# thomasjaron/masking-bundle-adjusting-neural-radiance-fields

Measured on AMD Instinct MI355X. Metric: warped+encoded+MLP pixels/s/GPU; final PSNR vs ref (seed=3), higher is better.
Workload: dtype bf16x3; 1 GPU; c3: 64 patches x 256x256 px per GPU, L=16, MLP 66-256-256-256-256-3, bf16x3 recipe (split-bf16 hi+lo MFMA operands, fp32 accumulate; seed-3 parity), c2f [0,0.4] at progress 0.2; patches_per_gpu=64, parallelism=dp1 (patches), step_kernel=k_step2

## Files before the change

masking-bundle-adjusting-neural-radiance-fields_amd/csrc/marf_abi.hip:

```cpp
#include <hip/hip_runtime.h>

#include <algorithm>
#include <cmath>
#include <cstdarg>
#include <cstdio>
#include <cstring>
#include <mutex>
#include <string>

#include "../../include/marf.h"
#include "marf_args.h"
#include "marf_prof.h"

using namespace marf;

static thread_local std::string g_err;
static unsigned long long* g_stamps = nullptr;

static int fail(int code, const char* fmt, ...) {
    char buf[512];
    va_list ap;
    va_start(ap, fmt);
    vsnprintf(buf, sizeof(buf), fmt, ap);
    va_end(ap);
// ... 499 lines not shown
        mx = std::max(mx, (long long)p.Mp * p.Kp + (long long)p.Kp * p.Mt + p.Mp);
    }
    MarfProfScope ps("pack_weights", (hipStream_t)stream);
    if (!split_recipe(net->dtype))
        HIPCHK(marf_launch_pack(net->kdt, d_params, (char*)d_packed, a, mx, (hipStream_t)stream), "net_pack");
    if (net->s2.variant >= 0) {
        const Step2NetPlan& q = net->s2;
        Pack2Args b;
        memset(&b, 0, sizeof(b));
        b.nl = net->n_layers;
        b.L = net->L;
        b.nk0 = q.nk0;
        b.nta = q.nta;
        b.NKH = q.HM / 16;
        b.split = q.variant == 1 || q.variant == 3;
        b.fwd_f16 = q.variant == 3;
        b.slot_bytes = q.slot;
        b.n_stages = q.n_stages;
        b.r0 = q.r0;
        b.ns0 = q.ns0;
        for (int l = 0; l <= net->n_layers; ++l) b.dims[l] = net->dims[l];
        for (int l = 0; l < net->n_layers; ++l) {
            b.nrt[l] = q.nrt[l];
            b.nrtb[l] = q.nrtb[l];
            b.w_off[l] = net->w_off[l];
            b.b_off[l] = net->b_off[l];
            b.boff[l] = q.boff[l];
            b.Mp[l] = net->Mp[l];
        }
        b.nbias = q.nbias;
        char* pk = (char*)d_packed;
        HIPCHK(marf_launch_pack2(d_params, pk + q.prog_off, (float*)(pk + q.bias_off), (int*)(pk + q.kmap_off), b,
                                 (hipStream_t)stream),
               "net_pack step2");
    }
    return MARF_OK;
}

static void fill_netdev(const marf_net* n, const void* packed, NetDev& d) {
    memset(&d, 0, sizeof(d));
    d.n_layers = n->n_layers;
    d.L = n->L;
    d.D = n->D;
    for (int l = 0; l < n->n_layers; ++l) {
        d.Kp[l] = n->Kp[l];
        d.Mp[l] = n->Mp[l];
        d.Mt[l] = n->Mt[l];
        d.Wf[l] = (const char*)packed + n->wf_off[l];
        d.Wt[l] = (const char*)packed + n->wt_off[l];
        d.bias[l] = (const float*)((const char*)packed + n->bias_off[l]);
        d.diag[l] = n->diag[l];
    }
    d.skip = n->skip;
}


struct SavedPlan {
    size_t feat[MARF_MAX_LAYERS], mask[MARF_MAX_LAYERS], total;
};

static void plan_saved(const marf_net* n, long long S, SavedPlan& p) {
    size_t off = 0;
    for (int l = 0; l < n->n_layers; ++l) {
        p.feat[l] = off;
        off += rup((long long)S * n->Kp[l] * n->elem, 256);
    }
    p.mask[0] = 0;
    for (int l = 1; l < n->n_layers; ++l) {
        p.mask[l] = off;
        off += rup(S / n->TP * 4096, 256);
    }
    p.total = off;
}

struct WsPlan {
    size_t dz[MARF_MAX_LAYERS], glast, dH, part, bpart, total;
    int chunk, n_chunks, n_tiles;
    int chunk_last, n_chunks_last;
};

static void plan_ws(const marf_net* n, long long S, int n_tiles, WsPlan& p) {
    size_t off = 0;
    p.dz[0] = 0;
    for (int l = 1; l < n->n_layers; ++l) {
        p.dz[l] = off;
        off += rup((long long)S * n->Kp[l] * n->elem, 256);
    }
    p.glast = off;
    off += rup(S * 16, 256);
    p.dH = off;
    off += rup((long long)n_tiles * 9 * 4, 256);
    long long chunk = rup((S + 255) / 256, 64);
    if (chunk < 64) chunk = 64;
    p.chunk = (int)chunk;
    p.n_chunks = (int)((S + chunk - 1) / chunk);
    p.n_tiles = n_tiles;
    long long mxo = 0, mxm = 0;
    for (int l = 0; l < n->n_layers - 1; ++l) {
        mxo = std::max(mxo, (long long)n->Mp[l] * n->Kp[l]);
        mxm = std::max(mxm, (long long)n->Mp[l]);
    }
    long long cl = rup((S + 1023) / 1024, 64);
    if (cl < 64) cl = 64;
    p.chunk_last = (int)cl;
    p.n_chunks_last = (int)((S + cl - 1) / cl);
    long long part_elems = std::max((long long)p.n_chunks * mxo, (long long)p.n_chunks_last * 3 * n->Kp[n->n_layers - 1]);
    long long bpart_elems = std::max((long long)p.n_chunks * mxm, (long long)p.n_chunks_last * 3);
    p.part = off;
    off += rup(part_elems * 4, 256);
    p.bpart = off;
    off += rup(bpart_elems * 4, 256);
    p.total = off;
}

size_t marf_saved_bytes(const marf_net* net, const marf_geometry* geo) {
    GeoDev g;
    if (!net || make_geo(geo, g, MARF_TILE_PAD) != MARF_OK) return 0;
    SavedPlan p;
    plan_saved(net, (long long)g.B * g.Np_pad, p);
    return p.total;
}

size_t marf_workspace_bytes(const marf_net* net, const marf_geometry* geo) {
    GeoDev g;
    if (!net || make_geo(geo, g, MARF_TILE_PAD) != MARF_OK) return 0;
    long long S = (long long)g.B * g.Np_pad;
    WsPlan p;
    plan_ws(net, S, (int)(S / net->TP), p);
    return p.total;
}


int marf_forward(const marf_net* net, const marf_geometry* geo, const marf_c2f* c2f, const void* d_packed,
                 float* d_rgb, void* d_saved, void* stream) {
    if (!net || !d_packed || !d_rgb) return fail(MARF_ERR_INVALID, "forward: NULL argument");
    if (split_recipe(net->dtype))
        return fail(MARF_ERR_UNSUPPORTED, "forward: split-recipe nets run marf_step_forward / marf_render only");
    FwdArgs a;
    memset(&a, 0, sizeof(a));
    int rc = make_geo(geo, a.geo, MARF_TILE_PAD);
    if (rc) return rc;
    fill_netdev(net, d_packed, a.net);
    a.c2f = make_c2f(c2f);
    a.rgb = d_rgb;
    a.S = (long long)a.geo.B * a.geo.Np_pad;
    a.lda = net->lda;
    if (d_saved) {
        SavedPlan p;
        plan_saved(net, a.S, p);
        for (int l = 0; l < net->n_layers; ++l) a.feat[l] = (char*)d_saved + p.feat[l];
        for (int l = 1; l < net->n_layers; ++l) a.mask[l] = (uint64_t*)((char*)d_saved + p.mask[l]);
    }
    int n_tiles = (int)(a.S / net->TP);
    {
        MarfProfScope ps("mlp_fwd", (hipStream_t)stream);
        HIPCHK(marf_launch_mlp_fwd(a, net->kdt, net->TP, net->lds_fwd, n_tiles, (hipStream_t)stream), "forward");
    }
    return MARF_OK;
}

int marf_backward(const marf_net* net, const marf_geometry* geo, const marf_c2f* c2f, const void* d_packed,
                  const float* d_h_params, int lie_batch, const float* d_rgb_out, const float* d_drgb,
                  const void* d_saved, void* d_workspace, float* d_dparams, float* d_dh, float* d_dcoords,
                  void* stream) {
    if (!net || !d_packed || !d_rgb_out || !d_drgb || !d_saved || !d_workspace)
        return fail(MARF_ERR_INVALID, "backward: NULL argument");
    if (split_recipe(net->dtype))
        return fail(MARF_ERR_UNSUPPORTED, "backward: split-recipe nets run marf_step_backward only");
    hipStream_t s = (hipStream_t)stream;
    BwdArgs a;
    memset(&a, 0, sizeof(a));
    int rc = make_geo(geo, a.geo, MARF_TILE_PAD);
    if (rc) return rc;
    if (a.geo.mode == MARF_GEO_GRID && d_dh && !d_h_params)
        return fail(MARF_ERR_INVALID, "backward: d_dh requested without the warp parameters");
    fill_netdev(net, d_packed, a.net);
    a.c2f = make_c2f(c2f);
    a.rgb = d_rgb_out;
    a.d_rgb = d_drgb;
    a.S = (long long)a.geo.B * a.geo.Np_pad;
    a.lda = net->lda;
    const int n_tiles = (int)(a.S / net->TP);
    SavedPlan sp;
    plan_saved(net, a.S, sp);
    WsPlan wp;
    plan_ws(net, a.S, n_tiles, wp);
    char* ws = (char*)d_workspace;
    const char* sv = (const char*)d_saved;
    for (int l = 1; l < net->n_layers; ++l) {
        a.mask[l] = (const uint64_t*)(sv + sp.mask[l]);
        a.dz[l] = ws + wp.dz[l];
    }
    a.glast = (float*)(ws + wp.glast);
    a.dH_partial = (float*)(ws + wp.dH);
    a.d_coords = d_dcoords;
    if (a.geo.mode == MARF_GEO_COORDS && !d_dcoords) {
        a.d_coords = nullptr;
    }
    {
        MarfProfScope ps("mlp_bwd_dgrad", s);
        HIPCHK(marf_launch_mlp_bwd(a, net->kdt, net->TP, net->lds_bwd, n_tiles, s), "backward dgrad");
    }

    if (d_dparams) {
        float* part = (float*)(ws + wp.part);
        float* bpart = (float*)(ws + wp.bpart);
        const int nl = net->n_layers;
        for (int l = 0; l < nl - 1; ++l) {
            {
                MarfProfScope ps(l == 0 ? "wgrad_l0" : "wgrad_hidden", s);
                HIPCHK(marf_launch_wgrad(net->kdt, ws + wp.dz[l + 1], net->Kp[l + 1], sv + sp.feat[l], net->Kp[l],
                                         a.S, net->Mp[l], net->Kp[l], wp.chunk, wp.n_chunks, part, bpart, s),
                       "backward wgrad");
            }
            {
                MarfProfScope ps("wgrad_reduce", s);
                HIPCHK(marf_launch_wgrad_reduce(part, bpart, wp.n_chunks, net->Mp[l], net->Kp[l], net->dims[l + 1],
                                                net->kin[l], d_dparams + net->w_off[l], d_dparams + net->b_off[l], s),
                       "backward wgrad reduce");
            }
        }
        const int l = nl - 1;
        {
            MarfProfScope ps("wgrad_last", s);
            HIPCHK(marf_launch_wgrad_last(net->kdt, a.glast, sv + sp.feat[l], a.S, net->Kp[l], net->Kp[l],
                                          wp.chunk_last, wp.n_chunks_last, part, bpart, s),
                   "backward wgrad last");
        }
        HIPCHK(marf_launch_wgrad_reduce(part, bpart, wp.n_chunks_last, 3, net->Kp[l], 3, net->dims[l],
                                        d_dparams + net->w_off[l], d_dparams + net->b_off[l], s),
               "backward wgrad last reduce");
    }
    if (a.geo.mode == MARF_GEO_GRID && d_dh) {
        MarfProfScope ps("warp_bwd", s);
        HIPCHK(marf_launch_reduce_dH(a.dH_partial, a.geo.Np_pad / net->TP, a.geo.B, d_h_params, nullptr, d_dh,
                                     lie_batch > 0 ? lie_batch : a.geo.B, s),
               "backward warp");
    }
    return MARF_OK;
}


struct StepPlan {
    size_t feat[MARF_MAX_LAYERS], dz[MARF_MAX_LAYERS], mask[MARF_MAX_LAYERS];
    size_t wlast, blast, dH, loss, c2f, part, bpart, total;
    int n_tiles, chunk, n_chunks;
};

static void plan_step(const marf_net* n, long long S, StepPlan& p) {
    size_t off = 0;
    const int nl = n->n_layers;
    p.n_tiles = (int)(S / n->sTP);
    for (int l = 0; l < nl - 1; ++l) {
        p.feat[l] = off;
        off += rup((long long)S * n->Kp[l] * n->elem, 256);
    }
    p.dz[0] = p.mask[0] = 0;
    for (int l = 1; l < nl; ++l) {
        p.dz[l] = off;
        off += rup((long long)S * n->Kp[l] * n->elem, 256);
        p.mask[l] = off;
        off += rup(S / n->sTP * n->sNW * 1024, 256);
    }
    p.wlast = off;
    off += rup((long long)p.n_tiles * 3 * n->Kp[nl - 1] * 4, 256);
    p.blast = off;
    off += rup((long long)p.n_tiles * 3 * 4, 256);
    p.dH = off;
    off += rup((long long)p.n_tiles * 9 * 4, 256);
    p.loss = off;
    off += rup((long long)p.n_tiles * 2 * 8, 256);
    p.c2f = off;
    off += 256;
    long long chunk = rup((S + 255) / 256, 64);
    if (chunk < 64) chunk = 64;
    p.chunk = (int)chunk;
    p.n_chunks = (int)((S + chunk - 1) / chunk);
    long long mxo = 0, mxm = 0;
    for (int l = 0; l < nl - 1; ++l) {
        mxo = std::max(mxo, (long long)n->Mp[l] * n->Kp[l]);
        mxm = std::max(mxm, (long long)n->Mp[l]);
    }
    p.part = off;
    off += rup(std::max((long long)p.n_chunks * mxo, 256LL * (3 * n->Kp[nl - 1] + 3)) * 4, 256);
    p.bpart = off;
    off += rup((long long)p.n_chunks * mxm * 4, 256);
    p.total = off;
}


#define MARF_PIPE_MAXP 64
struct PipePlan {
    int on;
    int G, R, P;
    int piece;
    int wg_last;
    int n_parts;
};

struct Step2BufPlan {
    size_t feat[MARF_MAX_LAYERS], dz[MARF_MAX_LAYERS];
    size_t dH, loss, blast, wlast, dummy, c2f, kmap, part, bpart, total;
    size_t partl[MARF_MAX_LAYERS], bpartl[MARF_MAX_LAYERS];
    int grid, n_tiles;
    int nblk;
    long long S;
    PipePlan pipe;
    bool fused_res;
};

static bool step2_fused_wgrad_possible(const marf_net* n) {
    static const bool env_off = [] {
        const char* e = getenv("MARF_WGRAD_FUSED");
        return e && e[0] == '0';
    }();
    if (env_off) return false;
    for (int l = 1; l < n->n_layers - 1; ++l)
        if (n->Mp[l] != 256 || n->Kp[l] != 256) return false;
    return true;
}

static int device_cus() {
    static int cus[64] = {0};
    int dev = 0;
    if (hipGetDevice(&dev) != hipSuccess || dev < 0 || dev >= 64) return 256;
    if (!cus[dev]) {
        int c = 0;
        if (hipDeviceGetAttribute(&c, hipDeviceAttributeMultiprocessorCount, dev) != hipSuccess || c <= 0) c = 256;
        cus[dev] = c;
    }
    return cus[dev];
}

static bool use_step2(const marf_net* n) { return n->s2.variant >= 0; }

static long long wgrad_chunk(long long S) {
    long long chunk = rup((S + 255) / 256, 64);
    return chunk < 64 ? 64 : chunk;
}

static bool l0_recompute(const marf_net* n, const GeoDev& g, long long S) {
    const char* e = getenv("MARF_F0_RECOMPUTE");
    if (e && e[0] == '0') return false;
    if ((n->s2.variant != 1 && n->s2.variant != 3) || g.mode != MARF_GEO_GRID) return false;
    const long long chunk = wgrad_chunk(S);
    return marf_wgrad_l0_recompute_ok(n->Mp[0], n->Kp[1], n->s2.ldf0, S, (int)chunk, (int)((S + chunk - 1) / chunk),
                                      g.Np_pad);
}


static void plan_pipe(const marf_net* n, const GeoDev& g, long long S, int n_tiles, PipePlan& pp) {
    memset(&pp, 0, sizeof(pp));
    const Step2NetPlan& q = n->s2;
    const int mode = n->pipe_mode;
    if (mode == 0 || q.variant < 0 || q.variant == 3 || g.mode != MARF_GEO_GRID) return;
    const int cus = device_cus();
    int R = n->pipe_wg > 0 ? n->pipe_wg : std::max(1, cus * 7 / 64);
    R = std::max(1, std::min(R, cus / 2));
    const int G = cus - R;
    if (mode < 0 && n_tiles < 16 * cus) return;
    int piece = n->pipe_piece;
    if (piece <= 0) {
        const int k = std::max(1, (int)std::lround((double)n_tiles / (8.0 * q.NS * G)));
        piece = k * q.NS * G;
    }
    piece = (int)rup(piece, q.NS);
    int P = (n_tiles + piece - 1) / piece;
    if (P < 2) {
        if (mode != 1) return;
        piece = (int)rup((n_tiles + 1) / 2, q.NS);
        P = (n_tiles + piece - 1) / piece;
        if (P < 2) return;
    }
    if (P > MARF_PIPE_MAXP) return;
    const int nl = n->n_layers;
    for (int l = 1; l < nl - 1; ++l)
        if (!marf_wgrad_range_ok(n->kdt, n->Mp[l], n->Kp[l + 1], n->Kp[l], n->Kp[l])) return;
    if (!marf_wgrad_range_ok(n->kdt, n->Mp[0], n->Kp[1], q.ldf0, q.ldf0)) return;
    if (l0_recompute(n, g, S)) {
        const long long mx = rup((long long)piece * q.TPX / R + 32, 32);
        if (!marf_wgrad_l0_recompute_ok(n->Mp[0], n->Kp[1], q.ldf0, S, (int)mx, P * cus, g.Np_pad)) return;
    }
    pp.on = 1;
    pp.G = G;
    pp.R = R;
    pp.P = P;
    pp.piece = piece;
    pp.wg_last = cus;
    pp.n_parts = (P - 1) * R + cus;
}

struct PipeStreams {
    hipStream_t s2;
    hipEvent_t ev[MARF_PIPE_MAXP + 1];
    std::mutex use;
};
static int pipe_streams(PipeStreams** out) {
    static std::mutex mu;
    static PipeStreams ps[64];
    int dev = 0;
    HIPCHK(hipGetDevice(&dev), "pipeline: hipGetDevice");
    if (dev < 0 || dev >= 64) return fail(MARF_ERR_UNSUPPORTED, "pipeline: device %d", dev);
    std::lock_guard<std::mutex> lk(mu);
    PipeStreams& p = ps[dev];
    if (!p.s2) {
        HIPCHK(hipStreamCreateWithFlags(&p.s2, hipStreamNonBlocking), "pipeline: stream");
        for (int i = 0; i <= MARF_PIPE_MAXP; ++i)
            HIPCHK(hipEventCreateWithFlags(&p.ev[i], hipEventDisableTiming), "pipeline: event");
    }
    *out = &p;
    return MARF_OK;
}

static void plan_step2_bufs(const marf_net* n, const GeoDev& g, Step2BufPlan& p, bool render = false) {
    const Step2NetPlan& q = n->s2;
    const int nl = n->n_layers;
    const long long Ssave = render ? 0 : 1;
    p.S = (long long)g.B * g.Np_pad;
    p.n_tiles = (int)(p.S / q.TPX);
    int cap = device_cus();
    if (const char* e = getenv("MARF_STEP2_GRID")) cap = std::max(1, atoi(e));
    p.grid = std::max(1, std::min(p.n_tiles, cap));
    memset(&p.pipe, 0, sizeof(p.pipe));
    p.fused_res = false;
    if (!render) plan_pipe(n, g, p.S, p.n_tiles, p.pipe);
    if (p.pipe.on) p.grid = p.pipe.G;
    p.nblk = p.pipe.on ? p.pipe.P * p.pipe.G : p.grid;
    size_t off = 0;
    const long long Sfeat = p.S + (q.variant == 3 ? q.TPX : 0);
    for (int l = 0; l < nl - 1; ++l) {
        p.feat[l] = off;
        off += rup(Ssave * Sfeat * (l == 0 ? q.ldf0 : n->Kp[l]) * 2, 256);
    }
    p.dz[0] = 0;
    const long long Ssink = p.S + q.TPX;
    for (int l = 1; l < nl; ++l) {
        p.dz[l] = off;
        off += rup(Ssave * Ssink * n->Kp[l] * 2, 256);
    }
    p.dH = off;
    off += rup(Ssave * Ssink / q.PX * 9 * 4, 256);
    p.loss = off;
    off += rup((long long)p.nblk * 2 * 8, 256);
    p.blast = off;
    off += rup((long long)p.nblk * 3 * 4, 256);
    p.wlast = off;
    off += rup((long long)p.nblk * 3 * q.Kl * 4, 256);
    p.dummy = off;
    off += rup((long long)p.grid * q.NW * 4096, 256);
    p.c2f = off;
    off += 256;
    p.kmap = off;
    off += rup((long long)n->D * 4, 256);
    long long chunk = rup((p.S + 255) / 256, 64);
    if (chunk < 64) chunk = 64;
    const long long n_chunks = (p.S + chunk - 1) / chunk;
    long long mxo = 0, mxm = 0;
    for (int l = 0; l < nl - 1; ++l) {
        mxo = std::max(mxo, (long long)n->Mp[l] * (l == 0 ? q.ldf0 : n->Kp[l]));
        mxm = std::max(mxm, (long long)n->Mp[l]);
    }
    if (p.pipe.on) {
        const long long np = p.pipe.n_parts;
        for (int l = 0; l < nl - 1; ++l) {
            p.partl[l] = off;
            off += rup(np * n->Mp[l] * (l == 0 ? q.ldf0 : n->Kp[l]) * 4, 256);
            p.bpartl[l] = off;
            off += rup(np * n->Mp[l] * 4, 256);
        }
        p.part = off;
        off += rup(256LL * (3 * q.Kl + 3) * 4, 256);
        p.bpart = 0;
    } else {
        p.part = off;
        off += rup(Ssave * std::max(n_chunks * mxo, 256LL * (3 * q.Kl + 3)) * 4, 256);
        p.bpart = off;
        off += rup(Ssave * n_chunks * mxm * 4, 256);
        p.fused_res = !render && step2_fused_wgrad_possible(n);
        p.partl[0] = p.part;
        p.bpartl[0] = p.bpart;
        for (int l = 1; l < nl - 1; ++l) {
            p.partl[l] = p.part;
            p.bpartl[l] = p.bpart;
            if (!p.fused_res) continue;
            p.partl[l] = off;
            off += rup(Ssave * n_chunks * n->Mp[l] * n->Kp[l] * 4, 256);
            p.bpartl[l] = off;
            off += rup(Ssave * n_chunks * n->Mp[l] * 4, 256);
        }
    }
    p.total = off;
}

static int wgrad_piece(const marf_net* net, const GeoDev& g, const Step2BufPlan& p, char* sv, int j, hipStream_t s2) {
    const Step2NetPlan& q = net->s2;
    const PipePlan& pp = p.pipe;
    const int nl = net->n_layers;
    const long long TPX = q.TPX;
    const long long t0 = (long long)j * pp.piece, t1 = std::min<long long>(p.n_tiles, t0 + pp.piece);
    WgRange r;
    r.s_lo = t0 * TPX;
    r.s_len = (t1 - t0) * TPX;
    r.n = j == pp.P - 1 ? pp.wg_last : pp.R;
    r.part0 = j * pp.R;
    const bool f0 = l0_recompute(net, g, p.S);
    for (int l = 0; l < nl - 1; ++l) {
        const int K = l == 0 ? q.ldf0 : net->Kp[l];
        float* part = (float*)(sv + p.partl[l]);
        float* bpart = (float*)(sv + p.bpartl[l]);
        MarfProfScope ps(l == 0 ? "wgrad_l0" : "wgrad_hidden", s2);
        if (l == 0 && f0)
            HIPCHK(marf_launch_wgrad_l0_recompute(sv + p.dz[1], net->Kp[1], g, (const float*)(sv + p.c2f), net->L, q.nk0w,
                                                  q.ldf0, p.S, net->Mp[0], 32, r.n, part, bpart, s2, &r),
                   "step_forward pipelined wgrad_l0");
        else
            HIPCHK(marf_launch_wgrad(1, sv + p.dz[l + 1], net->Kp[l + 1], sv + p.feat[l], K, p.S, net->Mp[l], K, 32, r.n,
                                     part, bpart, s2, &r, true),
                   "step_forward pipelined wgrad");
    }
    return MARF_OK;
}

static hipError_t launch_s2(const marf_net* n, const Step2Args& a, int grid, hipStream_t s) {
    const Step2NetPlan& q = n->s2;
    bool full = (q.variant == 1 || q.variant == 3) && q.nk0 >= 1 && q.r0 == std::max(1, std::min(8, 16 / q.nk0)) && q.Kl == 256;
    for (int l = 0; l < n->n_layers - 1; ++l) full = full && n->Mp[l] == 256;
    if (const char* e = getenv("MARF_STEP2_GENERIC")) full = full && e[0] != '1';
    return marf_launch_step2(a, q.variant, grid, s, full ? q.nk0 : 0, q.dz);
}

static int step2_forward(const marf_net* net, const marf_geometry* geo, const marf_c2f* c2f, const void* d_packed,
                         const float* d_gt, const float* d_mask, const float* d_denom_override, float* d_rgb,
                         float* d_loss_out, void* d_saved, hipStream_t s, bool render = false) {
    const Step2NetPlan& q = net->s2;
    Step2Args a;
    memset(&a, 0, sizeof(a));
    int rc = make_geo(geo, a.geo, q.TPX);
    if (rc) return rc;
    Step2BufPlan p;
    plan_step2_bufs(net, a.geo, p, render);
    char* sv = (char*)d_saved;
    const char* pk = (const char*)d_packed;
    const int nl = net->n_layers;
    a.nl = nl;
    a.L = net->L;
    a.nk0 = q.nk0;
    a.nta = q.nta;
    a.r0 = q.r0;
    C2fDev cf = make_c2f(c2f);
    a.c2f_on = cf.on;
    a.prog = pk + q.prog_off;
    a.n_stages = q.n_stages;
    a.n_fwd = q.n_fwd;
    a.S = p.S;
    if (render) {
        a.fwd_only = 1;
        a.n_stages = a.n_fwd;
        a.pro_fallback = a.geo.mode == MARF_GEO_COORDS ? a.geo.coords : a.geo.Hm;
    }
    a.bias = (const float*)(pk + q.bias_off);
    a.nbias = q.nbias;
    a.feat0_recompute = !render && l0_recompute(net, a.geo, p.S) ? 1 : 0;
    a.gt = d_gt;
    a.mask = d_mask;
    a.rgb = d_rgb;
    for (int l = 0; l < nl; ++l) {
        S2Layer& y = a.layers[l];
        y.nrt = q.nrt[l];
        y.nrtb = q.nrtb[l];
        y.boff = q.boff[l];
        y.ldf = l == 0 ? q.ldf0 : net->Kp[l];
        y.ldz = net->Kp[l];
        y.feat = l < nl - 1 && !render ? (u16*)(sv + p.feat[l]) : nullptr;
        y.dz = l >= 1 && !render ? (u16*)(sv + p.dz[l]) : nullptr;
    }
    a.dH_partial = (float*)(sv + p.dH);
    a.loss_partial = (double*)(sv + p.loss);
    a.blast_partial = (float*)(sv + p.blast);
    a.wlast_partial = (float*)(sv + p.wlast);
    a.Kl = q.Kl;
    a.c2f_w = (const float*)(sv + p.c2f);
    a.dummy = (float*)(sv + p.dummy);
    a.stamps = g_stamps;
    a.n_tiles = p.n_tiles;
    const int TPX = q.TPX;
    int off = q.nslot * q.slot;
    a.lds_pro = off;
    off += q.variant == 3 ? 1024 + 2 * 4 * TPX * 4 : 2 * (4 * TPX + 64) * 4;
    a.lds_bias = off;
    off += (int)rup(q.nbias * 4, 16);
    a.lds_c2f = off;
    off += 128;
    a.lds_layers = off;
    off += (int)sizeof(S2Layer) * MARF_MAX_LAYERS;
    a.lds_wave = off;
    a.lds_wave_bytes = (int)rup(2048 + q.NS * q.MAXR * q.NMW * 256 + 12 * q.Kl, 16);
    off += q.NW * a.lds_wave_bytes;
    a.lds_total = off;
    if (off > 160 * 1024) return fail(MARF_ERR_UNSUPPORTED, "step2: LDS plan %d B exceeds 160 KB", off);
    HIPCHK(marf_launch_c2f_weights(cf, net->L, (float*)(sv + p.c2f), s, (const int*)(pk + q.kmap_off),
                                   (int*)(sv + p.kmap), net->D),
           "step_forward c2f / kmap");
    if (render) {
        MarfProfScope ps("mlp_fwd", s);
        HIPCHK(launch_s2(net, a, p.grid, s), "render step2");
        return MARF_OK;
    }
    double* const loss0 = a.loss_partial;
    if (!p.pipe.on) {
        MarfProfScope ps("mlp_step", s);
        HIPCHK(launch_s2(net, a, p.grid, s), "step_forward step2");
    } else {
        const PipePlan& pp = p.pipe;
        PipeStreams* st = nullptr;
        rc = pipe_streams(&st);
        if (rc) return rc;
        std::lock_guard<std::mutex> hold(st->use);
        float* const blast0 = a.blast_partial;
        float* const wlast0 = a.wlast_partial;
        for (int j = 0; j < pp.P; ++j) {
            a.tile0 = j * pp.piece;
            a.n_tiles = std::min(p.n_tiles, (j + 1) * pp.piece);
            a.loss_partial = loss0 + (size_t)j * pp.G * 2;
            a.blast_partial = blast0 + (size_t)j * pp.G * 3;
            a.wlast_partial = wlast0 + (size_t)j * pp.G * 3 * q.Kl;
            {
                MarfProfScope ps("mlp_step", s);
                HIPCHK(launch_s2(net, a, pp.G, s), "step_forward step2 piece");
            }
            HIPCHK(hipEventRecord(st->ev[j], s), "pipeline: record");
            HIPCHK(hipStreamWaitEvent(st->s2, st->ev[j], 0), "pipeline: wait");
            rc = wgrad_piece(net, a.geo, p, sv, j, st->s2);
            if (rc) return rc;
        }
        HIPCHK(hipEventRecord(st->ev[MARF_PIPE_MAXP], st->s2), "pipeline: record");
        HIPCHK(hipStreamWaitEvent(s, st->ev[MARF_PIPE_MAXP], 0), "pipeline: join");
    }
    {
        MarfProfScope ps("loss_final", s);
        HIPCHK(marf_launch_loss_final(loss0, p.nblk, d_loss_out, d_denom_override, s), "step_forward loss");
    }
    return MARF_OK;
}

static int mark_layer(const void* const* ev, int l, hipStream_t s) {
    if (ev && ev[l]) HIPCHK(hipEventRecord((hipEvent_t)ev[l], s), "step_backward: layer event");
    return MARF_OK;
}

static int step2_backward(const marf_net* net, const marf_geometry* geo, const void* d_saved,
                          const float* d_h_params, int lie_batch, const float* d_gout, const float* d_loss_out,
                          float* d_dparams, float* d_dh, hipStream_t s, const void* const* ev) {
    const Step2NetPlan& q = net->s2;
    GeoDev g;
    int rc = make_geo(geo, g, q.TPX);
    if (rc) return rc;
    Step2BufPlan p;
    plan_step2_bufs(net, g, p);
    const char* sv = (const char*)d_saved;
    float* part = (float*)(sv + p.part);
    float* bpart = (float*)(sv + p.bpart);
    const float* denom = d_loss_out + 1;
    const int nl = net->n_layers;
    const int sdt = q.variant == 3 ? 2 : 1;
    const float post = q.variant == 3 ? 1.0f / 1024.0f : 1.0f;
    if (d_dparams && !p.pipe.on && p.fused_res) {
        const long long chunk = wgrad_chunk(p.S);
        const int n_chunks = (int)((p.S + chunk - 1) / chunk);
        const int* kmap = (const int*)(sv + p.kmap);
        const bool f0 = l0_recompute(net, g, p.S);
        WgFusedLayer Lf[MARF_MAX_LAYERS];
        memset(Lf, 0, sizeof(Lf));
        int nf = 0;
        {
            const int l = nl - 1;
            WgFusedLayer& x = Lf[nf++];
            x.kind = 3;
            x.partial = (float*)(sv + p.wlast);
            x.bpartial = (float*)(sv + p.blast);
            x.n_parts = p.nblk;
            x.M = 3;
            x.K = q.Kl;
            x.Mo = 3;
            x.Ko = net->dims[l];
            x.dW = d_dparams + net->w_off[l];
            x.db = d_dparams + net->b_off[l];
        }
        for (int l = nl - 2; l >= 0; --l) {
            WgFusedLayer& x = Lf[nf++];
            x.kind = l > 0 ? 0 : (f0 ? 1 : 2);
            x.dz = sv + p.dz[l + 1];
            x.ldz = net->Kp[l + 1];
            x.feat = (l == 0 && f0) ? nullptr : sv + p.feat[l];
            x.ldf = x.K = l == 0 ? q.ldf0 : net->Kp[l];
            x.M = net->Mp[l];
            x.partial = (float*)(sv + p.partl[l]);
            x.bpartial = (float*)(sv + p.bpartl[l]);
            x.n_parts = n_chunks;
            x.Mo = net->dims[l + 1];
            x.Ko = net->dims[l];
            x.dW = d_dparams + net->w_off[l];
            x.db = d_dparams + net->b_off[l];
            x.kmap = l == 0 ? kmap : nullptr;
        }
        if (marf_wgrad_fused_ok(Lf, nf, p.S, (int)chunk, n_chunks, g.Np_pad)) {
            PipeStreams* st = nullptr;
            rc = pipe_streams(&st);
            if (rc) return rc;
            {
                std::lock_guard<std::mutex> hold(st->use);
                const char* dse = getenv("MARF_DH_SIDE");
                float* dh_side = (dse && dse[0] == '0') ? nullptr : d_dh;
                if (dh_side) {
                    HIPCHK(hipEventRecord(st->ev[2], s), "step_backward: fork");
                    HIPCHK(hipStreamWaitEvent(st->s2, st->ev[2], 0), "step_backward: fork");
                }
                {
                    MarfProfScope ps("wgrad_fused", s);
                    HIPCHK(marf_launch_wgrad_fused(Lf, nf, p.S, (int)chunk, n_chunks, g, (const float*)(sv + p.c2f),
                                                   net->L, q.nk0w, d_gout, denom, s, st->s2, st->ev[0], st->ev[1], sdt, post),
                           "step_backward fused weight gradients");
                }
                if (dh_side) {
                    MarfProfScope ps("warp_bwd_side", st->s2);
                    HIPCHK(marf_launch_reduce_dH((const float*)(sv + p.dH), g.Np_pad / q.PX, g.B, d_h_params, nullptr,
                                                 dh_side, lie_batch > 0 ? lie_batch : g.B, st->s2, d_gout, denom),
                           "step_backward warp");
                    HIPCHK(hipEventRecord(st->ev[3], st->s2), "step_backward: join");
                }
                for (int l = nl - 1; l >= 0; --l) {
                    rc = mark_layer(ev, l, s);
                    if (rc) return rc;
                }
                if (dh_side) {
                    HIPCHK(hipStreamWaitEvent(s, st->ev[3], 0), "step_backward: join");
                    d_dh = nullptr;
                }
            }
            d_dparams = nullptr;
        }
    }
    if (d_dparams) {
        const int l = nl - 1;
        MarfProfScope ps("wgrad_last_reduce", s);
        HIPCHK(marf_launch_wgrad_reduce((const float*)(sv + p.wlast), (const float*)(sv + p.blast), p.nblk, 3, q.Kl, 3,
                                        net->dims[l], d_dparams + net->w_off[l], d_dparams + net->b_off[l], s, d_gout,
                                        denom, part),
               "step_backward last reduce");
        rc = mark_layer(ev, l, s);
        if (rc) return rc;
    }
    if (d_dparams && p.pipe.on) {
        const int* kmap = (const int*)(sv + p.kmap);
        for (int l = nl - 2; l >= 0; --l) {
            const int K = l == 0 ? q.ldf0 : net->Kp[l];
            MarfProfScope ps("wgrad_reduce", s);
            HIPCHK(marf_launch_wgrad_reduce((const float*)(sv + p.partl[l]), (const float*)(sv + p.bpartl[l]),
                                            p.pipe.n_parts, net->Mp[l], K, net->dims[l + 1], net->dims[l],
                                            d_dparams + net->w_off[l], d_dparams + net->b_off[l], s, d_gout, denom,
                                            nullptr, l == 0 ? kmap : nullptr),
                   "step_backward wgrad reduce (pipelined)");
            rc = mark_layer(ev, l, s);
            if (rc) return rc;
        }
    } else if (d_dparams) {
        const long long chunk = wgrad_chunk(p.S);
        const int n_chunks = (int)((p.S + chunk - 1) / chunk);
        const int* kmap = (const int*)(sv + p.kmap);
        const bool f0 = l0_recompute(net, g, p.S);
        for (int l = nl - 2; l >= 0; --l) {
            const int K = l == 0 ? q.ldf0 : net->Kp[l];
            {
                MarfProfScope ps(l == 0 ? "wgrad_l0" : "wgrad_hidden", s);
                if (l == 0 && f0)
                    HIPCHK(marf_launch_wgrad_l0_recompute(sv + p.dz[1], net->Kp[1], g, (const float*)(sv + p.c2f), net->L,
                                                          q.nk0w, q.ldf0, p.S, net->Mp[0], (int)chunk, n_chunks, part, bpart, s,
                                                          nullptr, sdt),
                           "step_backward wgrad_l0 (feat_0 recomputed)");
                else
                    HIPCHK(marf_launch_wgrad(sdt, sv + p.dz[l + 1], net->Kp[l + 1], sv + p.feat[l], K, p.S, net->Mp[l], K,
                                             (int)chunk, n_chunks, part, bpart, s, nullptr, true),
                           "step_backward wgrad");
            }
            {
                MarfProfScope ps("wgrad_reduce", s);
                HIPCHK(marf_launch_wgrad_reduce(part, bpart, n_chunks, net->Mp[l], K, net->dims[l + 1], net->dims[l],
                                                d_dparams + net->w_off[l], d_dparams + net->b_off[l], s, d_gout, denom,
                                                nullptr, l == 0 ? kmap : nullptr, post),
                       "step_backward wgrad reduce");
            }
            rc = mark_layer(ev, l, s);
            if (rc) return rc;
        }
    }
    if (d_dh) {
        MarfProfScope ps("warp_bwd", s);
        HIPCHK(marf_launch_reduce_dH((const float*)(sv + p.dH), g.Np_pad / q.PX, g.B, d_h_params, nullptr, d_dh,
                                     lie_batch > 0 ? lie_batch : g.B, s, d_gout, denom),
               "step_backward warp");
    }
    return MARF_OK;
}

size_t marf_render_workspace_bytes(const marf_net* net, const marf_geometry* geo) {
    if (!net || !geo || !use_step2(net)) return 0;
    GeoDev g;
    if (make_geo(geo, g, net->s2.TPX) != MARF_OK) return 0;
    Step2BufPlan p;
    plan_step2_bufs(net, g, p, true);
    return p.total;
}

int marf_render(const marf_net* net, const marf_geometry* geo, const marf_c2f* c2f, const void* d_packed, float* d_rgb,
                void* d_ws, void* stream) {
    if (!net || !geo || !d_packed || !d_rgb) return fail(MARF_ERR_INVALID, "render: NULL argument");
    if (!use_step2(net)) return marf_forward(net, geo, c2f, d_packed, d_rgb, nullptr, stream);
    if (!d_ws) return fail(MARF_ERR_INVALID, "render: workspace (marf_render_workspace_bytes) missing");
    if (geo->mode == MARF_GEO_GRID || geo->mode == MARF_GEO_CANVAS) {
        if (!geo->d_H) return fail(MARF_ERR_INVALID, "render: grid geometry needs d_H");
    } else if (geo->mode == MARF_GEO_COORDS) {
        if (geo->Np <= 0 || !geo->d_coords) return fail(MARF_ERR_INVALID, "render: coords geometry needs points");
    }
    return step2_forward(net, geo, c2f, d_packed, nullptr, nullptr, nullptr, d_rgb, nullptr, d_ws,
                         (hipStream_t)stream, true);
}

size_t marf_step_saved_bytes(const marf_net* net, const marf_geometry* geo) {
    GeoDev g;
    if (!net || !geo || geo->mode == MARF_GEO_COORDS) return 0;
    if (use_step2(net)) {
        if (make_geo(geo, g, net->s2.TPX) != MARF_OK) return 0;
        Step2BufPlan p2;
        plan_step2_bufs(net, g, p2);
        return p2.total;
    }
    if (make_geo(geo, g, MARF_TILE_PAD) != MARF_OK) return 0;
    StepPlan p;
    plan_step(net, (long long)g.B * g.Np_pad, p);
    return p.total;
}

int marf_step_forward(const marf_net* net, const marf_geometry* geo, const marf_c2f* c2f, const void* d_packed,
                      const float* d_gt, const float* d_mask, const float* d_denom_override, float* d_rgb,
                      float* d_loss_out, void* d_saved, void* stream) {
    if (!net || !d_packed || !d_gt || !d_loss_out || !d_saved) return fail(MARF_ERR_INVALID, "step_forward: NULL argument");
    if (!geo || geo->mode == MARF_GEO_COORDS) return fail(MARF_ERR_INVALID, "step_forward: needs a pixel-grid geometry");
    hipStream_t s = (hipStream_t)stream;
    if (use_step2(net))
        return step2_forward(net, geo, c2f, d_packed, d_gt, d_mask, d_denom_override, d_rgb, d_loss_out, d_saved, s);
    StepArgs a;
    memset(&a, 0, sizeof(a));
    int rc = make_geo(geo, a.geo, MARF_TILE_PAD);
    if (rc) return rc;
    fill_netdev(net, d_packed, a.net);
    a.c2f = make_c2f(c2f);
    a.rgb = d_rgb;
    a.gt = d_gt;
    a.mask = d_mask;
    a.S = (long long)a.geo.B * a.geo.Np_pad;
    a.lda = net->lda;
    StepPlan p;
    plan_step(net, a.S, p);
    char* sv = (char*)d_saved;
    const int nl = net->n_layers;
    for (int l = 0; l < nl - 1; ++l) a.feat[l] = sv + p.feat[l];
    for (int l = 1; l < nl; ++l) {
        a.dz[l] = sv + p.dz[l];
        a.mask_bits[l] = (uint64_t*)(sv + p.mask[l]);
    }
    a.wlast_partial = (float*)(sv + p.wlast);
    a.blast_partial = (float*)(sv + p.blast);
    a.dH_partial = (float*)(sv + p.dH);
    a.loss_partial = (double*)(sv + p.loss);
    a.c2f_w = (const float*)(sv + p.c2f);
    a.stamps = g_stamps;
    if (net->L > 0) HIPCHK(marf_launch_c2f_weights(a.c2f, net->L, (float*)(sv + p.c2f), s), "step_forward c2f");
    {
        MarfProfScope ps("mlp_step", s);
        HIPCHK(marf_launch_mlp_step(a, net->kdt, net->sTP, net->sNW, net->lds_step, p.n_tiles, s), "step_forward");
    }
    {
        MarfProfScope ps("loss_final", s);
        HIPCHK(marf_launch_loss_final(a.loss_partial, p.n_tiles, d_loss_out, d_denom_override, s), "step_forward loss");
    }
    return MARF_OK;
}

int marf_step_backward(const marf_net* net, const marf_geometry* geo, const void* d_saved, const float* d_h_params,
                       int lie_batch, const float* d_gout, const float* d_loss_out, float* d_dparams, float* d_dh,
                       void* stream) {
    return marf_step_backward_ev(net, geo, d_saved, d_h_params, lie_batch, d_gout, d_loss_out, d_dparams, d_dh, nullptr,
                                 stream);
}

int marf_step_backward_ev(const marf_net* net, const marf_geometry* geo, const void* d_saved, const float* d_h_params,
                          int lie_batch, const float* d_gout, const float* d_loss_out, float* d_dparams, float* d_dh,
                          void* const* layer_events, void* stream) {
    const void* const* ev = (const void* const*)layer_events;
    if (!net || !d_saved || !d_gout || !d_loss_out) return fail(MARF_ERR_INVALID, "step_backward: NULL argument");
    if (!geo || geo->mode == MARF_GEO_COORDS) return fail(MARF_ERR_INVALID, "step_backward: needs a pixel-grid geometry");
    if (d_dh && !d_h_params) return fail(MARF_ERR_INVALID, "step_backward: d_dh requested without the warp parameters");
    hipStream_t s = (hipStream_t)stream;
    if (use_step2(net))
        return step2_backward(net, geo, d_saved, d_h_params, lie_batch, d_gout, d_loss_out, d_dparams, d_dh, s, ev);
    GeoDev g;
    int rc = make_geo(geo, g, MARF_TILE_PAD);
    if (rc) return rc;
    const long long S = (long long)g.B * g.Np_pad;
    StepPlan p;
    plan_step(net, S, p);
    const char* sv = (const char*)d_saved;
    float* part = (float*)(sv + p.part);
    float* bpart = (float*)(sv + p.bpart);
    const float* denom = d_loss_out + 1;
    const int nl = net->n_layers;
    if (d_dparams) {
        {
            const int l = nl - 1;
            MarfProfScope ps("wgrad_last_reduce", s);
            HIPCHK(marf_launch_wgrad_reduce((const float*)(sv + p.wlast), (const float*)(sv + p.blast), p.n_tiles, 3,
                                            net->Kp[l], 3, net->dims[l], d_dparams + net->w_off[l],
                                            d_dparams + net->b_off[l], s, d_gout, denom, part),
                   "step_backward last reduce");
            rc = mark_layer(ev, l, s);
            if (rc) return rc;
        }
        for (int l = nl - 2; l >= 0; --l) {
            {
                MarfProfScope ps(l == 0 ? "wgrad_l0" : "wgrad_hidden", s);
                HIPCHK(marf_launch_wgrad(net->kdt, sv + p.dz[l + 1], net->Kp[l + 1], sv + p.feat[l], net->Kp[l], S,
                                         net->Mp[l], net->Kp[l], p.chunk, p.n_chunks, part, bpart, s),
                       "step_backward wgrad");
            }
            {
                MarfProfScope ps("wgrad_reduce", s);
                HIPCHK(marf_launch_wgrad_reduce(part, bpart, p.n_chunks, net->Mp[l], net->Kp[l], net->dims[l + 1],
                                                net->kin[l], d_dparams + net->w_off[l], d_dparams + net->b_off[l], s,
                                                d_gout, denom),
                       "step_backward wgrad reduce");
            }
            rc = mark_layer(ev, l, s);
            if (rc) return rc;
        }
    }
    if (d_dh) {
        MarfProfScope ps("warp_bwd", s);
        HIPCHK(marf_launch_reduce_dH((const float*)(sv + p.dH), g.Np_pad / net->sTP, g.B, d_h_params, nullptr, d_dh,
                                     lie_batch > 0 ? lie_batch : g.B, s, d_gout, denom),
               "step_backward warp");
    }
    return MARF_OK;
}


size_t marf_mse_workspace_bytes(void) { return 1024 * 2 * sizeof(double); }

int marf_masked_mse(const float* d_pred, const float* d_gt, const float* d_mask, int B, int Np,
                    const float* d_denom_override, float* d_out, void* d_ws, void* stream) {
    if (B <= 0 || Np <= 0 || !d_pred || !d_gt || !d_out || !d_ws) return fail(MARF_ERR_INVALID, "masked_mse: bad args");
    MarfProfScope ps("loss_fwd", (hipStream_t)stream);
    HIPCHK(marf_launch_mse(d_pred, d_gt, d_mask, B, Np, (double*)d_ws, d_out, d_denom_override, (hipStream_t)stream),
           "masked_mse");
    return MARF_OK;
}

int marf_masked_mse_backward(const float* d_pred, const float* d_gt, const float* d_mask, int B, int Np,
                             const float* d_denom, const float* d_gout, float* d_dpred, void* stream) {
    if (B <= 0 || Np <= 0 || !d_pred || !d_gt || !d_denom || !d_gout || !d_dpred)
        return fail(MARF_ERR_INVALID, "masked_mse_backward: bad args");
    MarfProfScope ps("loss_bwd", (hipStream_t)stream);
    HIPCHK(marf_launch_mse_bwd(d_pred, d_gt, d_mask, B, Np, d_denom, d_gout, d_dpred, (hipStream_t)stream),
           "masked_mse_backward");
    return MARF_OK;
}

int marf_edge_map(const float* d_img, int n_img, int H, int W, double* d_out, void* stream) {
    if (n_img < 0 || H <= 0 || W <= 0 || (n_img > 0 && (!d_img || !d_out))) return fail(MARF_ERR_INVALID, "edge_map: bad args");
    if (n_img > 65535) return fail(MARF_ERR_INVALID, "edge_map: more than 65535 channel images");
    if (n_img == 0) return MARF_OK;
    MarfProfScope ps("edge_map", (hipStream_t)stream);
    HIPCHK(marf_launch_edge_map(d_img, d_out, n_img, H, W, (hipStream_t)stream), "edge_map");
    return MARF_OK;
}

int marf_erode_rect(const float* d_img, int n_img, int H, int W, int kh, int kw, float* d_out, void* stream) {
    if (n_img < 0 || H <= 0 || W <= 0 || kh <= 0 || kw <= 0 || (n_img > 0 && (!d_img || !d_out)))
        return fail(MARF_ERR_INVALID, "erode_rect: bad args");
    if (n_img > 65535) return fail(MARF_ERR_INVALID, "erode_rect: more than 65535 channel images");
    if (d_img == d_out) return fail(MARF_ERR_INVALID, "erode_rect: in-place erosion is not supported");
    if (n_img == 0) return MARF_OK;
    HIPCHK(marf_launch_erode_rect(d_img, d_out, n_img, H, W, kh, kw, (hipStream_t)stream), "erode_rect");
    return MARF_OK;
}

}

static void adam_scalars(double lr, double beta1, double beta2, long long step, float& step_size, float& bc2_sqrt) {
    const double bc1 = 1.0 - std::pow(beta1, (double)step);
    const double bc2 = 1.0 - std::pow(beta2, (double)step);
    step_size = (float)(lr / bc1);
    bc2_sqrt = (float)std::sqrt(bc2);
}

extern "C" {

int marf_adam_step(float* d_p, const float* d_g, float* d_m, float* d_v, long long n, double lr, double beta1,
                   double beta2, double eps, long long step, const float* d_grad_scale, void* stream) {
    if (n < 0 || step < 1 || (n > 0 && (!d_p || !d_g || !d_m || !d_v))) return fail(MARF_ERR_INVALID, "adam: bad args");
    float step_size, bc2_sqrt;
    adam_scalars(lr, beta1, beta2, step, step_size, bc2_sqrt);
    MarfProfScope ps("adam", (hipStream_t)stream);
    HIPCHK(marf_launch_adam(d_p, d_g, d_m, d_v, n, (float)(1.0 - beta1), (float)beta2, (float)(1.0 - beta2),
                            step_size, bc2_sqrt, (float)eps, d_grad_scale, (hipStream_t)stream),
           "adam");
    return MARF_OK;
}

int marf_adam_schedule(double lr, double beta1, double beta2, long long first_step, long long count, float* h_out) {
    if (first_step < 1 || count < 0 || (count > 0 && !h_out)) return fail(MARF_ERR_INVALID, "adam_schedule: bad args");
    for (long long i = 0; i < count; ++i) adam_scalars(lr, beta1, beta2, first_step + i, h_out[2 * i], h_out[2 * i + 1]);
    return MARF_OK;
}

int marf_adam_step_sched(float* d_p, const float* d_g, float* d_m, float* d_v, long long n, double beta1, double beta2,
                         double eps, const float* d_sched, const int* d_index, const float* d_grad_scale, void* stream) {
    if (n < 0 || (n > 0 && (!d_p || !d_g || !d_m || !d_v || !d_sched || !d_index)))
        return fail(MARF_ERR_INVALID, "adam_step_sched: bad args");
    MarfProfScope ps("adam", (hipStream_t)stream);
    HIPCHK(marf_launch_adam_sched(d_p, d_g, d_m, d_v, n, (float)(1.0 - beta1), (float)beta2, (float)(1.0 - beta2),
                                  d_sched, d_index, (float)eps, d_grad_scale, (hipStream_t)stream),
           "adam_step_sched");
    return MARF_OK;
}

}
```

masking-bundle-adjusting-neural-radiance-fields_amd/csrc/marf_args.h:

```cpp
#pragma once
#include "marf_common.h"

namespace marf {

struct C2fDev {
    const float* progress;
    float start, span;
    int on;
};

struct FwdArgs {
    NetDev net;
    GeoDev geo;
    C2fDev c2f;
    float* rgb;
    void* feat[MARF_MAX_LAYERS];
    uint64_t* mask[MARF_MAX_LAYERS];
    long long S;
    int lda;
};

struct BwdArgs {
    NetDev net;
    GeoDev geo;
    C2fDev c2f;
    const float* rgb;
    const float* d_rgb;
    const uint64_t* mask[MARF_MAX_LAYERS];
    void* dz[MARF_MAX_LAYERS];
    float* glast;
    float* dH_partial;
    float* d_coords;
    long long S;
    int lda;
};

struct StepArgs {
    NetDev net;
    GeoDev geo;
    C2fDev c2f;
    float* rgb;
    const float* gt;
    const float* mask;
    void* feat[MARF_MAX_LAYERS];
    uint64_t* mask_bits[MARF_MAX_LAYERS];
    void* dz[MARF_MAX_LAYERS];
    float* wlast_partial;
    float* blast_partial;
    float* dH_partial;
    double* loss_partial;
    const float* c2f_w;
    unsigned long long* stamps;
    long long S;
    int lda;
};

struct PackLayer {
    int M, K;
    int Mp, Kp, Mt;
    long long w_off, b_off;
    long long wf_off, wt_off, bias_off;
    unsigned diag;
};

struct PackArgs {
    int n_layers;
    PackLayer ly[MARF_MAX_LAYERS];
};

struct S2Layer {
    int nrt;
    int nrtb;
    int boff;
    int ldf;
    int ldz;
    int pad;
    u16* feat;
    u16* dz;
};

struct Step2Args {
    GeoDev geo;
    int nl, L, nk0, nta, c2f_on;
    int r0;
    const char* prog;
    int n_stages;
    int n_fwd;
    long long S;
    const float* bias;
    int nbias;
    const float* gt;
    const float* mask;
    float* rgb;
    S2Layer layers[MARF_MAX_LAYERS];
    float* dH_partial;
    double* loss_partial;
    float* blast_partial;
    float* wlast_partial;
    int Kl;
    const float* c2f_w;
    float* dummy;
    unsigned long long* stamps;
    int tile0, n_tiles;
    int fwd_only;
    int feat0_recompute;
    const float* pro_fallback;
    int lds_pro, lds_bias, lds_c2f, lds_layers, lds_wave, lds_wave_bytes, lds_total;
};

struct Pack2Args {
    int nl, L, nk0, nta, NKH, split, slot_bytes, n_stages;
    int fwd_f16;
    int r0, ns0;
    int dims[MARF_MAX_LAYERS + 1];
    int nrt[MARF_MAX_LAYERS], nrtb[MARF_MAX_LAYERS];
    long long w_off[MARF_MAX_LAYERS], b_off[MARF_MAX_LAYERS];
    int boff[MARF_MAX_LAYERS];
    int Mp[MARF_MAX_LAYERS];
    int nbias;
};

hipError_t ensure_dynamic_lds(const void* kernel, size_t lds);

}

hipError_t marf_launch_sl3(const float* h, float* H, int B, int batch_hint, hipStream_t s);
hipError_t marf_launch_se2_embed(const float* p, float* h, int B, hipStream_t s);
hipError_t marf_launch_se2_embed_bwd(const float* dh, float* dp, int B, hipStream_t s);
hipError_t marf_launch_sl3_bwd(const float* h, const float* dH, float* dh, int B, int batch_hint, hipStream_t s);
hipError_t marf_launch_reduce_dH(const float* partial, int tiles_per_patch, int B, const float* h, float* dH_out,
                                 float* dh, int batch_hint, hipStream_t s, const float* gscale = nullptr,
                                 const float* denom = nullptr);
hipError_t marf_launch_mlp_fwd(const marf::FwdArgs& a, int dtype, int TP, size_t lds, int n_tiles, hipStream_t s);
hipError_t marf_launch_mlp_bwd(const marf::BwdArgs& a, int dtype, int TP, size_t lds, int n_tiles, hipStream_t s);
struct WgRange {
    long long s_lo, s_len;
    int n, part0;
};
bool marf_wgrad_range_ok(int dtype, int M, int ldz, int K, int ldf);
bool marf_wgrad_l0_recompute_ok(int M, int ldz, int ldf0, long long S, int chunk, int n_chunks, long long Np_pad);
hipError_t marf_launch_wgrad_l0_recompute(const void* dz, int ldz, const GeoDev& geo, const float* c2f_w, int L,
                                          int nk0, int K0, long long S, int M, int chunk, int n_chunks, float* partial,
                                          float* bpartial, hipStream_t s, const WgRange* rng = nullptr, int dtype = 1);
hipError_t marf_launch_wgrad(int dtype, const void* dz, int ldz, const void* feat, int ldf, long long S, int M, int K,
                             int chunk, int n_chunks, float* partial, float* bpartial, hipStream_t s,
                             const WgRange* rng = nullptr, bool t16 = false);
struct WgFusedLayer {
    int kind;
    const void* dz;
    const void* feat;
    int ldz, ldf, M, K;
    float* partial;
    float* bpartial;
    int n_parts;
    int Mo, Ko;
    float* dW;
    float* db;
    const int* kmap;
};
bool marf_wgrad_fused_ok(const WgFusedLayer* layers, int n_layers, long long S, int chunk, int n_chunks,
                         long long Np_pad);
hipError_t marf_launch_wgrad_fused(const WgFusedLayer* layers, int n_layers, long long S, int chunk, int n_chunks,
                                   const GeoDev& f0_geo, const float* c2f_w, int L, int nk0, const float* gscale,
                                   const float* denom, hipStream_t s, hipStream_t s2, hipEvent_t fork, hipEvent_t join,
                                   int dtype = 1, float post = 1.f);
hipError_t marf_launch_wgrad_last(int dtype, const float* glast, const void* feat, long long S, int ldf, int K,
                                  int chunk, int n_chunks, float* partial, float* bpartial, hipStream_t s);
hipError_t marf_launch_wgrad_reduce(const float* partial, const float* bpartial, int n_chunks, int M, int K, int Mo,
                                    int Ko, float* dW, float* db, hipStream_t s, const float* gscale = nullptr,
                                    const float* denom = nullptr, float* scratch = nullptr,
                                    const int* kmap = nullptr, float post = 1.f);
hipError_t marf_launch_mlp_step(const marf::StepArgs& a, int dtype, int TP, int NW, size_t lds, int n_tiles, hipStream_t s);
hipError_t marf_launch_c2f_weights(const marf::C2fDev& c, int L, float* out, hipStream_t s,
                                   const int* csrc = nullptr, int* cdst = nullptr, int cn = 0);
hipError_t marf_launch_loss_final(const double* part, int n, float* out, const float* denom_override, hipStream_t s);
hipError_t marf_launch_step2(const marf::Step2Args& a, int variant, int grid, hipStream_t s, int full_nk0, bool dz = false);
hipError_t marf_launch_pack2(const float* params, void* prog, float* bias_out, int* kmap, const marf::Pack2Args& a,
                             hipStream_t s);
hipError_t marf_launch_edge_map(const float* in, double* out, int n_img, int H, int W, hipStream_t s);
hipError_t marf_launch_erode_rect(const float* in, float* out, int n_img, int H, int W, int kh, int kw, hipStream_t s);
hipError_t marf_launch_mse(const float* pred, const float* gt, const float* mask, int B, int Np, double* part,
                           float* out, const float* denom_override, hipStream_t s);
hipError_t marf_launch_mse_bwd(const float* pred, const float* gt, const float* mask, int B, int Np,
                               const float* denom, const float* gout, float* d_pred, hipStream_t s);
hipError_t marf_launch_adam(float* p, const float* g, float* m, float* v, long long n, float w1, float b2,
                            float one_minus_b2, float step_size, float bc2_sqrt, float eps, const float* grad_scale,
                            hipStream_t s);
hipError_t marf_launch_adam_sched(float* p, const float* g, float* m, float* v, long long n, float w1, float b2,
                                  float one_minus_b2, const float* sched, const int* index, float eps,
                                  const float* grad_scale, hipStream_t s);
hipError_t marf_launch_pack(int dtype, const float* params, char* packed, const marf::PackArgs& a,
                            long long max_elems, hipStream_t s);
hipError_t marf_launch_pixel_grid(const GeoDev& g, float* xy, int n, hipStream_t s);
hipError_t marf_launch_warp_points(const float* xy, const float* Hm, float* uv, int B, int n, int xy_shared,
                                   hipStream_t s);
hipError_t marf_launch_posenc(const float* coord, long long n, int L, const float* progress, float start, float span,
                              int c2f_on, float* enc, hipStream_t s);
hipError_t marf_launch_warp_points_bwd(const float* xy, const float* Hm, const float* G, float* dxy, float* dH, int B,
                                       int n, int xy_shared, hipStream_t s);
hipError_t marf_launch_posenc_bwd(const float* coord, const float* G, long long n, int L, const float* progress,
                                  float start, float span, int c2f_on, float* dcoord, hipStream_t s);
hipError_t marf_launch_prologue_probe(const GeoDev& g, const marf::C2fDev& c, int L, const float* gt,
                                      const float* mask, float* out, int grid, hipStream_t s);
```

masking-bundle-adjusting-neural-radiance-fields_amd/csrc/marf_step2.hip:

```cpp
#include <type_traits>

#include "marf_args.h"

namespace marf {


MARF_DEV void s2_glds4(const void* src, unsigned lds) {
    unsigned keep;
    asm volatile("s_mov_b32 %0, m0\n\ts_mov_b32 m0, %2\n\ts_nop 0\n\tglobal_load_lds_dword %1, off\n\ts_mov_b32 m0, %0"
                 : "=&s"(keep)
                 : "v"(src), "s"(lds)
                 : "memory");
}
typedef uint32_t s2_u32x2 __attribute__((ext_vector_type(2)));
typedef uint32_t s2_u32x4 __attribute__((ext_vector_type(4)));
MARF_DEV void s2_st8(void* dst, uint32_t a, uint32_t b) {
    const s2_u32x2 v = {a, b};
    asm volatile("global_store_dwordx2 %0, %1, off\n\ts_nop 1" ::"v"(dst), "v"(v) : "memory");
}
MARF_DEV void s2_st16(void* dst, uint4 u) {
    const s2_u32x4 v = {u.x, u.y, u.z, u.w};
    asm volatile("global_store_dwordx4 %0, %1, off\n\ts_nop 1" ::"v"(dst), "v"(v) : "memory");
}
template <int OFF>
MARF_DEV void s2_st16o(void* base, uint4 u) {
    const s2_u32x4 v = {u.x, u.y, u.z, u.w};
    asm volatile("global_store_dwordx4 %0, %1, off offset:%2\n\ts_nop 1" ::"v"(base), "v"(v), "n"(OFF) : "memory");
}
MARF_DEV void s2_st12(void* dst, float a, float b, float c) {
    typedef float f32x3 __attribute__((ext_vector_type(3)));
    f32x3 v = {a, b, c};
    asm volatile("global_store_dwordx3 %0, %1, off\n\ts_nop 1" ::"v"(dst), "v"(v) : "memory");
}
MARF_DEV void s2_st4(void* dst, float a) {
    asm volatile("global_store_dword %0, %1, off\n\ts_nop 1" ::"v"(dst), "v"(a) : "memory");
}
template <int N>
MARF_DEV void s2_wait_vm() {
    asm volatile("s_waitcnt vmcnt(%0)" ::"n"(N) : "memory");
}

MARF_DEV i16x4 s2_tr16(const u16* p) {
    return __builtin_amdgcn_ds_read_tr16_b64_v4i16((__attribute__((address_space(3))) i16x4*)(p));
}

template <int... I, class F>
MARF_DEV void s2_sfor_impl(std::integer_sequence<int, I...>, F&& f) {
    (f(std::integral_constant<int, I>()), ...);
}
template <int N, class F>
MARF_DEV void s2_sfor(F&& f) {
    s2_sfor_impl(std::make_integer_sequence<int, N>(), f);
}

MARF_DEV uint32_t s2_pk(float a, float b) {
    typedef float f32x2 __attribute__((ext_vector_type(2)));
    typedef __bf16 bf16x2 __attribute__((ext_vector_type(2)));
    return __builtin_bit_cast(uint32_t, __builtin_convertvector(((f32x2){a, b}), bf16x2));
}
MARF_DEV float s2_lo16(uint32_t w) { return __uint_as_float(w << 16); }
MARF_DEV float s2_hi16(uint32_t w) { return __uint_as_float(w & 0xffff0000u); }

union S2Frag {
    bf16x8 f;
    f16x8 h;
    uint4 u;
    uint32_t w[4];
};

MARF_DEV uint32_t s2_pkh(float a, float b) {
    typedef float f32x2 __attribute__((ext_vector_type(2)));
    typedef _Float16 f16x2 __attribute__((ext_vector_type(2)));
    return __builtin_bit_cast(uint32_t, __builtin_convertvector(((f32x2){a, b}), f16x2));
}

template <bool LO>
MARF_DEV void s2_split8(const float* x, S2Frag& hi, S2Frag& lo) {
    hi.u = make_uint4(s2_pk(x[0], x[1]), s2_pk(x[2], x[3]), s2_pk(x[4], x[5]), s2_pk(x[6], x[7]));
    if constexpr (LO) {
        const uint32_t w[4] = {hi.u.x, hi.u.y, hi.u.z, hi.u.w};
        float r[8];
#pragma unroll
        for (int q = 0; q < 4; ++q) {
            r[2 * q] = x[2 * q] - s2_lo16(w[q]);
            r[2 * q + 1] = x[2 * q + 1] - s2_hi16(w[q]);
        }
        lo.u = make_uint4(s2_pk(r[0], r[1]), s2_pk(r[2], r[3]), s2_pk(r[4], r[5]), s2_pk(r[6], r[7]));
    }
}


#ifdef MARF_STAMPS
#define S2T_BEGIN(k) const unsigned long long _t##k = __builtin_amdgcn_s_memtime()
#define S2T_END(k) tacc[k] += __builtin_amdgcn_s_memtime() - _t##k
#else
#define S2T_BEGIN(k) \
    do {         \
    } while (0)
#define S2T_END(k) \
    do {       \
    } while (0)
#endif

template <int HM, bool SPLIT, int NW, int MAXR, bool DZ = false>
struct S2Cfg {
    static constexpr int NKH = HM / 16;
    static constexpr int NRT = HM / 32;
    static constexpr int SLOT = NKH * 1024 * (SPLIT ? 2 : 1);
    static constexpr int LO = NKH * 1024;
    static constexpr int PER_DMA = SLOT / (NW * 1024);
    static constexpr int NSLOT = 3, D = 2;
    static constexpr int NS = SPLIT && !DZ ? 2 : 1;
    static constexpr int NK0 = 9;
    static constexpr int NTA = 5;
    static constexpr int TPX = 32 * NW;
    static constexpr int NMW = NRT / 2;
    static constexpr int MSET = MAXR * NMW * 64;
    static_assert(PER_DMA * NW * 1024 == SLOT, "slot size");
};

template <int HM, bool SPLIT, int NW, int MAXR, int NK0F, int NTAF, bool DZ, bool HF = false>
__device__ __attribute__((always_inline)) inline void k_step2_body(const Step2Args& a) {
    typedef S2Cfg<HM, SPLIT, NW, MAXR, DZ> C;
    constexpr bool SDZ = SPLIT && DZ;
    constexpr int NKH = C::NKH, NRT = C::NRT, NS = C::NS;
    constexpr bool FIX = NK0F > 0;
    static_assert(NK0F <= C::NK0, "layer-0 k-steps");
    static_assert(!HF || (SPLIT && !DZ && NK0F > 0 && NS == 2), "fp16x2: split dgrad, two sets, compile-time layer 0");
#ifndef MARF_STEP2_J2
#define MARF_STEP2_J2 1
#endif
    constexpr bool J2 = MARF_STEP2_J2 && NS == 2 && SPLIT && !SDZ && FIX;
    constexpr float kGS = 1024.f;
    constexpr int R0Q = NKH / (FIX ? NK0F : NKH);
    constexpr int R0F = R0Q < 1 ? 1 : (R0Q > NRT ? NRT : R0Q);
    extern __shared__ __attribute__((aligned(16))) char smem[];
    const int lane = threadIdx.x & 63;
    const int wave = __builtin_amdgcn_readfirstlane(threadIdx.x >> 6);
    const int h = lane >> 5, pxl = lane & 31;
    const int nl = a.nl, L = a.L;

    const unsigned lds0 = (unsigned)(uintptr_t)(__attribute__((address_space(3))) char*)smem;
    float* bias_l = reinterpret_cast<float*>(smem + a.lds_bias);
    float* c2f_l = reinterpret_cast<float*>(smem + a.lds_c2f);
    S2Layer* lyr = reinterpret_cast<S2Layer*>(smem + a.lds_layers);
    auto ly_int = [&](int l, int field) -> int {
        return __builtin_amdgcn_readfirstlane(reinterpret_cast<const int*>(lyr + l)[field]);
    };
    auto ly_ptr = [&](int l, int which) -> u16* {
        const uint32_t* q = reinterpret_cast<const uint32_t*>(lyr + l) + 6 + 2 * which;
        const uint64_t lo = (uint32_t)__builtin_amdgcn_readfirstlane(q[0]);
        const uint64_t hi = (uint32_t)__builtin_amdgcn_readfirstlane(q[1]);
        return reinterpret_cast<u16*>(lo | (hi << 32));
    };
    char* wpriv = smem + a.lds_wave + wave * a.lds_wave_bytes;
    u16* trs = reinterpret_cast<u16*>(wpriv);
    u16* gts = reinterpret_cast<u16*>(wpriv + 1024);
    uint32_t* mkl = reinterpret_cast<uint32_t*>(wpriv + 2048);
    float* wla = reinterpret_cast<float*>(wpriv + 2048 + NS * C::MSET * 4);
    float* dmy = a.dummy + (((size_t)blockIdx.x * NW + wave) * 2 * 64 + lane) * 2;
#ifdef MARF_STAMPS
    unsigned long long tacc[16] = {};
#endif

    for (int e = threadIdx.x; e < a.nbias; e += NW * 64) bias_l[e] = a.bias[e];
    if ((int)threadIdx.x < 32) c2f_l[threadIdx.x] = (int)threadIdx.x < L ? a.c2f_w[threadIdx.x] : 0.f;
    for (int e = threadIdx.x; e < nl * (int)(sizeof(S2Layer) / 4); e += NW * 64)
        reinterpret_cast<uint32_t*>(lyr)[e] = reinterpret_cast<const uint32_t*>(a.layers)[e];
    for (int e = lane; e < 512; e += 64) reinterpret_cast<uint32_t*>(gts)[e] = 0u;
    for (int e = lane; e < 3 * a.Kl; e += 64) wla[e] = 0.f;

    const int tpp = a.geo.Np_pad / C::TPX;
    const int Np = a.geo.Np;
    const int tbase = a.tile0 + (int)blockIdx.x;
    int my_tiles = 0;
    if (tbase < a.n_tiles) my_tiles = (a.n_tiles - 1 - tbase) / (int)gridDim.x + 1;
    const int nF = a.n_fwd, nB = a.n_stages - a.n_fwd;
    const int total = HF ? ((my_tiles + NS - 1) / NS) * (nF + nB)
                         : (my_tiles / NS) * (NS * nF + nB) + (my_tiles % NS ? (my_tiles % NS) * nF + nB : 0);

    auto pro_buf = [&](int pb) -> float* { return reinterpret_cast<float*>(smem + a.lds_pro + pb * (4 * C::TPX + 64) * 4); };
    auto issue_pro = [&](int tile, int pb) {
        const int b = tile / tpp, q0 = (tile - b * tpp) * C::TPX;
        const unsigned base = lds0 + a.lds_pro + pb * (4 * C::TPX + 64) * 4;
#pragma unroll
        for (int i = 0; i < 2; ++i) {
            const int f = ((wave * 2 + i) * 64) + lane;
            const int ch = f / C::TPX, q = f - ch * C::TPX;
            const int p = min(q0 + q, Np - 1);
            const float* src = !a.gt ? a.pro_fallback
                               : ch < 3 ? a.gt + ((size_t)b * 3 + ch) * Np + p
                                        : (a.mask ? a.mask + (size_t)b * Np + p : a.gt + (size_t)b * 3 * Np + p);
            s2_glds4(src, __builtin_amdgcn_readfirstlane(base + (wave * 2 + i) * 256));
        }
        s2_glds4(a.geo.Hm ? a.geo.Hm + 9 * (size_t)b + (lane < 9 ? lane : 0) : a.pro_fallback,
                 __builtin_amdgcn_readfirstlane(base + 4 * C::TPX * 4));
    };

    auto hf_tile = [&](int ti) -> int { return tbase + min(ti, my_tiles - 1) * (int)gridDim.x; };
    auto proH = [&](int par, int set) -> const float* {
        return reinterpret_cast<const float*>(smem + a.lds_pro + (par * 2 + set) * 256);
    };
    auto proT = [&](int set) -> const float* {
        return reinterpret_cast<const float*>(smem + a.lds_pro + 1024 + set * C::TPX * 16);
    };
    auto issue_h = [&](int ti, int par) {
#pragma unroll
        for (int set = 0; set < 2; ++set) {
            const int b = hf_tile(ti + set) / tpp;
            s2_glds4(a.geo.Hm ? a.geo.Hm + 9 * (size_t)b + (lane < 9 ? lane : 0) : a.pro_fallback,
                     __builtin_amdgcn_readfirstlane(lds0 + a.lds_pro + (par * 2 + set) * 256));
        }
    };
    auto issue_tgt = [&](int ti) {
#pragma unroll
        for (int set = 0; set < 2; ++set) {
            const int tile = hf_tile(ti + set);
            const int b = tile / tpp, q0 = (tile - b * tpp) * C::TPX;
            const unsigned base = lds0 + a.lds_pro + 1024 + set * C::TPX * 16;
#pragma unroll
            for (int i = 0; i < 2; ++i) {
                const int f = ((wave * 2 + i) * 64) + lane;
                const int ch = f / C::TPX, q = f - ch * C::TPX;
                const int p = min(q0 + q, Np - 1);
                const float* src = !a.gt ? a.pro_fallback
                                   : ch < 3 ? a.gt + ((size_t)b * 3 + ch) * Np + p
                                            : (a.mask ? a.mask + (size_t)b * Np + p : a.gt + (size_t)b * 3 * Np + p);
                s2_glds4(src, __builtin_amdgcn_readfirstlane(base + (wave * 2 + i) * 256));
            }
        }
    };

    int c_stage = 0;
    int dma_stage = 0;
    int dg_i = 0, dg_n = 0, dg_ns = 0, dg_t = 0;
    auto grp_init = [&](int t) {
        dg_t = t;
        dg_ns = HF ? 1 : min(NS, my_tiles - t);
        dg_n = dg_ns * nF + nB;
        dg_i = 0;
    };
    grp_init(0);
    auto dma_next = [&]() -> int {
        const int i = dg_i;
        const int prog = i < nF ? i : (i < dg_ns * nF ? i - nF : i - (dg_ns - 1) * nF);
        if (++dg_i == dg_n) grp_init(dg_t + NS);
        return prog;
    };
    unsigned dma_m0 = 0;
    const char* dma_va0 = nullptr;
    const char* dma_va1 = nullptr;
    auto dma_arm = [&]() {
        const int ps = dma_stage < total ? dma_next() : 0;
        dma_m0 = __builtin_amdgcn_readfirstlane(lds0 + (dma_stage % C::NSLOT) * C::SLOT + wave * C::PER_DMA * 1024);
        dma_va0 = a.prog + (size_t)ps * C::SLOT + wave * C::PER_DMA * 1024 + lane * 16;
        if constexpr (C::PER_DMA > 4) dma_va1 = dma_va0 + 4096;
        ++dma_stage;
    };
    auto dma_piece = [&](auto jc) {
        constexpr int j = decltype(jc)::value;
        static_assert(j < C::PER_DMA && C::PER_DMA <= 8, "piece index");
        const char* va = j < 4 ? dma_va0 : dma_va1;
        const unsigned m = dma_m0 + (j < 4 ? 0u : 4096u);
        unsigned keep;
        asm volatile("s_mov_b32 %0, m0\n\ts_mov_b32 m0, %2\n\ts_nop 0\n\tglobal_load_lds_dwordx4 %1, off offset:%3\n\ts_mov_b32 m0, %0"
                     : "=&s"(keep)
                     : "v"(va), "s"(m), "n"((j & 3) * 1024)
                     : "memory");
    };
    auto dma_burst = [&]() { s2_sfor<C::PER_DMA>([&](auto jc) { dma_piece(jc); }); };
    int st_cur = 0, st_prev = 0;
    auto wait_ring = [&]() {
        const int y = st_prev + st_cur;
        constexpr int PD = C::PER_DMA;
        if (y >= 8) s2_wait_vm<PD + 8>();
        else if (y >= 6) s2_wait_vm<PD + 6>();
        else if (y >= 4) s2_wait_vm<PD + 4>();
        else if (y >= 2) s2_wait_vm<PD + 2>();
        else s2_wait_vm<PD>();
    };
    auto stage_begin = [&](bool burst) -> const char* {
        S2T_BEGIN(0);
        S2T_BEGIN(12);
        wait_ring();
#ifdef MARF_STAMPS
        asm volatile("s_waitcnt lgkmcnt(0)" ::: "memory");
#endif
        S2T_END(12);
        st_prev = st_cur;
        st_cur = 0;
        asm volatile("s_waitcnt lgkmcnt(0)" ::: "memory");
        __builtin_amdgcn_s_barrier();
        asm volatile("" ::: "memory");
        S2T_END(0);
        S2T_BEGIN(1);
        dma_arm();
        if (burst) dma_burst();
        S2T_END(1);
        const char* slot = smem + (c_stage % C::NSLOT) * C::SLOT;
        ++c_stage;
        return slot;
    };

    if (my_tiles > 0) {
        if constexpr (HF) {
            issue_h(0, 0);
            issue_tgt(0);
        } else {
            issue_pro(tbase, 0);
        }
        dma_arm();
        dma_burst();
        dma_arm();
        dma_burst();
    }
    s2_wait_vm<0>();
    __syncthreads();

    double lsq = 0.0, lms = 0.0;
    float bl0 = 0.f, bl1 = 0.f, bl2 = 0.f;

    uint32_t mpend = 0u;

    S2Frag Bh[NKH], Bl[NKH], Oh[NKH], Ol[NKH];

    auto store_rt = [&](u16* row0, auto rtc, const S2Frag& f0, const S2Frag& f1) {
        constexpr int rt = decltype(rtc)::value;
        auto contig = [&](const S2Frag& f) -> uint4 {
            const auto xz = __builtin_amdgcn_permlane32_swap(f.u.x, f.u.z, false, false);
            const auto yw = __builtin_amdgcn_permlane32_swap(f.u.y, f.u.w, false, false);
            return make_uint4(xz[0], yw[0], xz[1], yw[1]);
        };
        u16* blk = row0 + 1024 * rt;
        s2_st16o<0>(blk, contig(f0));
        s2_st16o<1024>(blk, contig(f1));
        st_cur += 2;
    };

    auto nohook = [&](auto, auto) {};
    auto piece_at = [&](auto ksc, auto nk_tag, auto pieces_tag) {
        constexpr int ks = decltype(ksc)::value;
        constexpr int NK = decltype(nk_tag)::value;
        if constexpr (decltype(pieces_tag)::value) {
            static_assert(NK % C::PER_DMA == 0, "pieces per k-step");
            constexpr int per = NK / C::PER_DMA;
            if constexpr (ks % per == per - 1) dma_piece(std::integral_constant<int, ks / per>());
        }
    };
    typedef std::integral_constant<bool, true> PcOn;
    typedef std::integral_constant<bool, false> PcOff;
    auto mf = [&](f32x16& acc, const uint4& x, const S2Frag& y) {
        if constexpr (HF)
            acc = __builtin_amdgcn_mfma_f32_32x32x16_f16(__builtin_bit_cast(f16x8, x), y.h, acc, 0, 0, 0);
        else
            acc = __builtin_amdgcn_mfma_f32_32x32x16_bf16(__builtin_bit_cast(bf16x8, x), y.f, acc, 0, 0, 0);
    };
    auto gemm = [&](f32x16& acc, const char* slot, const S2Frag* Bhi, const S2Frag* Blo, int nk, auto mode_tag,
                    auto nk_tag, auto&& hook, auto pieces_tag) {
        constexpr int MODE = decltype(mode_tag)::value;
        constexpr int NK = decltype(nk_tag)::value;
        typedef std::integral_constant<int, 0> P0;
        typedef std::integral_constant<int, 1> P1;
        const uint4* ah = reinterpret_cast<const uint4*>(slot + lane * 16);
        const uint4* al = reinterpret_cast<const uint4*>(slot + C::LO + lane * 16);
        constexpr int P = NK < 4 ? NK : 4;
        uint4 A0[4], A1[4];
#pragma unroll
        for (int u = 0; u < P; ++u) {
            A0[u] = ah[u * 64];
            if constexpr (MODE != 0) A1[u] = al[u * 64];
        }
        s2_sfor<NK>([&](auto ksc) {
            constexpr int ks = decltype(ksc)::value;
            constexpr int u = ks & 3;
            constexpr bool refill = ks + P < NK;
            const bool live = NK != C::NK0 || ks < nk;
            auto piece = [&]() { piece_at(ksc, nk_tag, pieces_tag); };
            __builtin_amdgcn_sched_barrier(0);
            if constexpr (MODE == 0) {
                if (live) {
                    mf(acc, A0[u], Bhi[ks]);
                    hook(ksc, P0());
                    hook(ksc, P1());
                }
                if constexpr (refill) A0[u] = ah[(ks + P) * 64];
                if (live) piece();
            } else if constexpr (MODE == 2) {
                if (live) {
                    mf(acc, A0[u], Bhi[ks]);
                    hook(ksc, P0());
                }
                if constexpr (refill) A0[u] = ah[(ks + P) * 64];
                __builtin_amdgcn_sched_barrier(0);
                if (live) {
                    mf(acc, A1[u], Bhi[ks]);
                    hook(ksc, P1());
                }
                if constexpr (refill) A1[u] = al[(ks + P) * 64];
                if (live) piece();
            } else {
                if (live) {
                    mf(acc, A0[u], Bhi[ks]);
                    hook(ksc, P0());
                }
                __builtin_amdgcn_sched_barrier(0);
                if (live) {
                    mf(acc, A0[u], Blo[ks]);
                    hook(ksc, P1());
                }
                if constexpr (refill) A0[u] = ah[(ks + P) * 64];
                __builtin_amdgcn_sched_barrier(0);
                if (live) mf(acc, A1[u], Bhi[ks]);
                if constexpr (refill) A1[u] = al[(ks + P) * 64];
                if (live) piece();
            }
            __builtin_amdgcn_sched_barrier(0);
        });
    };
    typedef std::integral_constant<int, SPLIT ? 1 : 0> MFt;
    typedef std::integral_constant<int, SPLIT ? 2 : 0> MBt;
    typedef std::integral_constant<int, SDZ ? 1 : (SPLIT ? 2 : 0)> MDt;
    typedef std::integral_constant<int, NKH> NKHt;
    typedef std::integral_constant<int, C::NK0> NK0t;
    typedef std::conditional_t<FIX, std::integral_constant<int, FIX ? NK0F : 1>, NK0t> NK0x;
    const int nk0 = FIX ? NK0F : a.nk0, r0 = FIX ? R0F : a.r0;
    typedef std::integral_constant<int, 1> NK1t;

    auto bias_init = [&](int boff, int rt) -> f32x16 {
        f32x16 acc;
        const float* bb = bias_l + boff + rt * 32 + 4 * h;
#pragma unroll
        for (int q = 0; q < 4; ++q) {
            const float4 v = *reinterpret_cast<const float4*>(bb + 8 * q);
            acc[4 * q] = v.x;
            acc[4 * q + 1] = v.y;
            acc[4 * q + 2] = v.z;
            acc[4 * q + 3] = v.w;
        }
        return acc;
    };
    auto zero_out = [&](S2Frag& o0, S2Frag& o1, S2Frag& q0, S2Frag& q1) {
        o0.u = o1.u = q0.u = q1.u = make_uint4(0, 0, 0, 0);
    };
    struct EpSt {
        uint32_t bits, mw;
        float vp, xo;
        uint32_t hw[8], lw[8];
        float ta, tb;
    } ep;
    f32x16 acc0 = (f32x16){}, acc1 = (f32x16){};
    auto frelu = [&](const f32x16& pa, auto ec) {
        constexpr int e = decltype(ec)::value;
        float x;
        asm volatile("v_max_i32_e32 %0, 0, %1" : "=&v"(x) : "v"(pa[e]));
        if constexpr (e & 1) ep.xo = x;
        else ep.vp = x;
    };
    const uint32_t k_pair1 = 0x00010001u;
    auto mask_pair = [&](uint32_t w) {
        uint32_t t;
        asm volatile(
            "v_pk_min_u16 %1, %2, %3\n\t"
            "v_lshl_or_b32 %0, %0, 1, %1"
            : "+v"(ep.bits), "=&v"(t)
            : "v"(w), "s"(k_pair1));
    };
    auto fpack = [&](auto ec) {
        constexpr int e = decltype(ec)::value;
        if constexpr (e & 1) {
            if constexpr (SPLIT) {
                uint32_t w, wl, t0, t1;
                asm volatile(
                    "v_cvt_pk_bf16_f32 %0, %4, %5\n\t"
                    "v_lshlrev_b32_e32 %2, 16, %0\n\t"
                    "v_and_b32_e32 %3, 0xffff0000, %0\n\t"
                    "v_sub_f32_e32 %2, %4, %2\n\t"
                    "v_sub_f32_e32 %3, %5, %3\n\t"
                    "v_cvt_pk_bf16_f32 %1, %2, %3"
                    : "=&v"(w), "=&v"(wl), "=&v"(t0), "=&v"(t1)
                    : "v"(ep.vp), "v"(ep.xo));
                ep.hw[e >> 1] = w;
                ep.lw[e >> 1] = wl;
                mask_pair(w);
            } else {
                uint32_t w;
                asm volatile("v_cvt_pk_bf16_f32 %0, %1, %2" : "=v"(w) : "v"(ep.vp), "v"(ep.xo));
                ep.hw[e >> 1] = w;
                mask_pair(w);
            }
        }
    };
    auto fpackA = [&](auto ec) {
        constexpr int e = decltype(ec)::value;
        static_assert(e & 1, "odd step");
        uint32_t w;
        float t0, t1;
        asm volatile(
            "v_cvt_pk_bf16_f32 %0, %3, %4\n\t"
            "v_lshlrev_b32_e32 %1, 16, %0\n\t"
            "v_and_b32_e32 %2, 0xffff0000, %0"
            : "=&v"(w), "=&v"(t0), "=&v"(t1)
            : "v"(ep.vp), "v"(ep.xo));
        ep.hw[e >> 1] = w;
        ep.ta = t0;
        ep.tb = t1;
        mask_pair(w);
    };
    auto fpackB = [&](auto ec) {
        constexpr int e = decltype(ec)::value;
        static_assert(e & 1, "odd step");
        uint32_t wl;
        float r0, r1;
        asm volatile(
            "v_sub_f32_e32 %1, %3, %5\n\t"
            "v_sub_f32_e32 %2, %4, %6\n\t"
            "v_cvt_pk_bf16_f32 %0, %1, %2"
            : "=&v"(wl), "=&v"(r0), "=&v"(r1)
            : "v"(ep.vp), "v"(ep.xo), "v"(ep.ta), "v"(ep.tb));
        ep.lw[e >> 1] = wl;
    };
    auto fstep = [&](const f32x16& pa, auto ec) {
        frelu(pa, ec);
        fpack(ec);
    };
    auto fsteps_free = [&](const f32x16& pa, auto e0c) {
        constexpr int E0 = decltype(e0c)::value;
        static_assert((E0 & 1) == 0, "whole pairs");
        uint32_t w[8];
        s2_sfor<(16 - E0) / 2>([&](auto jc) {
            constexpr int q = E0 / 2 + decltype(jc)::value;
            const float x0 = __int_as_float(max(__float_as_int(pa[2 * q]), 0));
            const float x1 = __int_as_float(max(__float_as_int(pa[2 * q + 1]), 0));
            const uint32_t hw = s2_pk(x0, x1);
            w[q] = hw;
            ep.hw[q] = hw;
            if constexpr (SPLIT) ep.lw[q] = s2_pk(x0 - s2_lo16(hw), x1 - s2_hi16(hw));
        });
        s2_sfor<(16 - E0) / 2>([&](auto jc) { mask_pair(w[E0 / 2 + decltype(jc)::value]); });
    };
    auto ffinish = [&](int l, auto rtc, bool save, u16* srow, uint32_t* mks, bool last) {
        constexpr int rt = decltype(rtc)::value;
        Oh[2 * rt].u = make_uint4(ep.hw[0], ep.hw[1], ep.hw[2], ep.hw[3]);
        Oh[2 * rt + 1].u = make_uint4(ep.hw[4], ep.hw[5], ep.hw[6], ep.hw[7]);
        if constexpr (SPLIT) {
            Ol[2 * rt].u = make_uint4(ep.lw[0], ep.lw[1], ep.lw[2], ep.lw[3]);
            Ol[2 * rt + 1].u = make_uint4(ep.lw[4], ep.lw[5], ep.lw[6], ep.lw[7]);
        }
        if constexpr ((rt & 1) == 0) {
            mpend = ep.bits << 8;
            if (last) mks[(l * C::NMW + (rt >> 1)) * 64 + lane] = mpend;
        } else {
            mks[(l * C::NMW + (rt >> 1)) * 64 + lane] = mpend | ep.bits;
        }
        if (save) store_rt(srow, rtc, Oh[2 * rt], Oh[2 * rt + 1]);
    };
    auto bstep = [&](EpSt& es, const f32x16& pa, auto ec, auto rtc) {
        constexpr int e = decltype(ec)::value;
        constexpr int rt = decltype(rtc)::value;
        constexpr int bit = 16 * (e & 1) + 8 * (1 - (rt & 1)) + 7 - (e >> 1);
        float x;
        asm volatile(
            "v_bfe_i32 %0, %1, %3, 1\n\t"
            "v_and_b32_e32 %0, %0, %2"
            : "=&v"(x)
            : "v"(es.mw), "v"(pa[e]), "n"(bit));
        if constexpr (e & 1) {
            uint32_t w;
            if constexpr (HF)
                asm volatile("v_cvt_pk_f16_f32 %0, %1, %2" : "=v"(w) : "v"(es.vp), "v"(x));
            else
                asm volatile("v_cvt_pk_bf16_f32 %0, %1, %2" : "=v"(w) : "v"(es.vp), "v"(x));
            es.hw[e >> 1] = w;
            if constexpr (SDZ) es.lw[e >> 1] = s2_pk(es.vp - s2_lo16(w), x - s2_hi16(w));
        } else {
            es.vp = x;
        }
    };
    auto bsteps_free = [&](EpSt& es, const f32x16& pa, auto rtc) {
        constexpr int rt = decltype(rtc)::value;
        s2_sfor<8>([&](auto qc) {
            constexpr int q = decltype(qc)::value;
            constexpr int b0 = 16 * 0 + 8 * (1 - (rt & 1)) + 7 - q, b1 = 16 * 1 + 8 * (1 - (rt & 1)) + 7 - q;
            const float x0 = __int_as_float(__builtin_amdgcn_sbfe((int)es.mw, b0, 1) & __float_as_int(pa[2 * q]));
            const float x1 = __int_as_float(__builtin_amdgcn_sbfe((int)es.mw, b1, 1) & __float_as_int(pa[2 * q + 1]));
            es.hw[q] = HF ? s2_pkh(x0, x1) : s2_pk(x0, x1);
            if constexpr (SDZ) es.lw[q] = s2_pk(x0 - s2_lo16(es.hw[q]), x1 - s2_hi16(es.hw[q]));
        });
    };
    auto bfinish = [&](EpSt& es, S2Frag* O, auto rtc, u16* row0) {
        constexpr int rt = decltype(rtc)::value;
        O[2 * rt].u = make_uint4(es.hw[0], es.hw[1], es.hw[2], es.hw[3]);
        O[2 * rt + 1].u = make_uint4(es.hw[4], es.hw[5], es.hw[6], es.hw[7]);
        if constexpr (SDZ) {
            Ol[2 * rt].u = make_uint4(es.lw[0], es.lw[1], es.lw[2], es.lw[3]);
            Ol[2 * rt + 1].u = make_uint4(es.lw[4], es.lw[5], es.lw[6], es.lw[7]);
        }
        store_rt(row0, rtc, O[2 * rt], O[2 * rt + 1]);
    };
    auto gemm2 = [&](f32x16& c0, f32x16& c1, const char* slot, const S2Frag* B0, const S2Frag* B1, auto nk_tag,
                     auto&& hook, auto pieces_tag, auto f16_tag) {
        constexpr int NK = decltype(nk_tag)::value;
        constexpr bool F16 = decltype(f16_tag)::value;
        typedef std::integral_constant<int, 0> P0;
        typedef std::integral_constant<int, 1> P1;
        typedef std::integral_constant<int, 2> P2;
        typedef std::integral_constant<int, 3> P3;
        auto mma = [&](f32x16& c, const uint4& av, const S2Frag& b) {
            if constexpr (F16)
                c = __builtin_amdgcn_mfma_f32_32x32x16_f16(__builtin_bit_cast(f16x8, av), b.h, c, 0, 0, 0);
            else
                c = __builtin_amdgcn_mfma_f32_32x32x16_bf16(__builtin_bit_cast(bf16x8, av), b.f, c, 0, 0, 0);
        };
        const uint4* ah = reinterpret_cast<const uint4*>(slot + lane * 16);
        const uint4* al = reinterpret_cast<const uint4*>(slot + C::LO + lane * 16);
        constexpr int P = NK < 4 ? NK : 4;
        uint4 A0[4], A1[4];
#pragma unroll
        for (int u = 0; u < P; ++u) {
            A0[u] = ah[u * 64];
            A1[u] = al[u * 64];
        }
        s2_sfor<NK>([&](auto ksc) {
            constexpr int ks = decltype(ksc)::value;
            constexpr int u = ks & 3;
            constexpr bool refill = ks + P < NK;
            __builtin_amdgcn_sched_barrier(0);
            mma(c0, A0[u], B0[ks]);
            hook(ksc, P0());
            __builtin_amdgcn_sched_barrier(0);
            mma(c1, A0[u], B1[ks]);
            hook(ksc, P1());
            if constexpr (refill) A0[u] = ah[(ks + P) * 64];
            __builtin_amdgcn_sched_barrier(0);
            mma(c0, A1[u], B0[ks]);
            hook(ksc, P2());
            __builtin_amdgcn_sched_barrier(0);
            mma(c1, A1[u], B1[ks]);
            hook(ksc, P3());
            if constexpr (refill) A1[u] = al[(ks + P) * 64];
            piece_at(ksc, nk_tag, pieces_tag);
            __builtin_amdgcn_sched_barrier(0);
        });
    };
    typedef std::integral_constant<bool, true> F16t;
    typedef std::integral_constant<bool, false> BF16t;
    struct Ep2 {
        float x[4][2];
        uint32_t bw[8];
        uint32_t bits, mpend;
    };
    Ep2 e2[2];
    auto mask_pair_to = [&](uint32_t& bits, uint32_t w) {
        uint32_t t;
        asm volatile(
            "v_pk_min_u16 %1, %2, %3\n\t"
            "v_lshl_or_b32 %0, %0, 1, %1"
            : "+v"(bits), "=&v"(t)
            : "v"(w), "s"(k_pair1));
    };
    auto hop = [&](const f32x16& p0s, const f32x16& p1s, S2Frag* O0, S2Frag* O1, auto rtc, auto pic, auto jc, auto opc) {
        constexpr int rt = decltype(rtc)::value, PI = decltype(pic)::value, j = decltype(jc)::value;
        constexpr int op = decltype(opc)::value;
        if constexpr (PI < 16) {
            constexpr int sset = PI >> 3, q = PI & 7;
            const f32x16& pa = sset ? p1s : p0s;
            Ep2& es = e2[sset];
            if constexpr (op < 2) {
                float x;
                asm volatile("v_max_i32_e32 %0, 0, %1" : "=&v"(x) : "v"(pa[2 * q + op]));
                es.x[j][op] = x;
            } else if constexpr (op == 2) {
                uint32_t w, wb;
                asm volatile(
                    "v_cvt_pk_f16_f32 %0, %2, %3\n\t"
                    "v_cvt_pk_bf16_f32 %1, %2, %3"
                    : "=&v"(w), "=&v"(wb)
                    : "v"(es.x[j][0]), "v"(es.x[j][1]));
                (sset ? O1 : O0)[2 * rt + (q >> 2)].w[q & 3] = w;
                es.bw[q] = wb;
            } else {
                mask_pair_to(es.bits, es.bw[q]);
            }
        }
    };
    typedef std::integral_constant<int, 0> I0;
    typedef std::integral_constant<int, 1> I1;
    typedef std::integral_constant<int, 2> I2;
    typedef std::integral_constant<int, 3> I3;
    auto hook2 = [&](const f32x16& p0s, const f32x16& p1s, S2Frag* O0, S2Frag* O1, auto rtc, auto ksc, auto pc,
                     auto ppkc) {
        constexpr int ks = decltype(ksc)::value, p = decltype(pc)::value, PPK = decltype(ppkc)::value;
        typedef std::integral_constant<int, PPK * ks> Pa;
        typedef std::integral_constant<int, PPK * ks + 1> Pb;
        if constexpr (PPK == 1) {
            hop(p0s, p1s, O0, O1, rtc, Pa(), I0(), pc);
        } else if constexpr (PPK == 4) {
            s2_sfor<4>([&](auto jc) {
                hop(p0s, p1s, O0, O1, rtc, std::integral_constant<int, PPK * ks + decltype(jc)::value>(), jc, pc);
            });
        } else {
            static_assert(PPK == 2, "pairs per k-step");
            if constexpr (p == 0) {
                hop(p0s, p1s, O0, O1, rtc, Pa(), I0(), I0());
                hop(p0s, p1s, O0, O1, rtc, Pa(), I0(), I1());
            } else if constexpr (p == 1) {
                hop(p0s, p1s, O0, O1, rtc, Pa(), I0(), I2());
                hop(p0s, p1s, O0, O1, rtc, Pb(), I1(), I0());
            } else if constexpr (p == 2) {
                hop(p0s, p1s, O0, O1, rtc, Pb(), I1(), I1());
                hop(p0s, p1s, O0, O1, rtc, Pa(), I0(), I3());
            } else {
                hop(p0s, p1s, O0, O1, rtc, Pb(), I1(), I2());
                hop(p0s, p1s, O0, O1, rtc, Pb(), I1(), I3());
            }
        }
    };
    auto free_pairs = [&](const f32x16& p0s, const f32x16& p1s, S2Frag* O0, S2Frag* O1, auto rtc, auto pi0c) {
        constexpr int rt = decltype(rtc)::value, PI0 = decltype(pi0c)::value;
        if constexpr (PI0 < 16) {
            s2_sfor<16 - PI0>([&](auto jc) {
                constexpr int PI = PI0 + decltype(jc)::value, sset = PI >> 3, q = PI & 7;
                const f32x16& pa = sset ? p1s : p0s;
                const float x0 = __int_as_float(max(__float_as_int(pa[2 * q]), 0));
                const float x1 = __int_as_float(max(__float_as_int(pa[2 * q + 1]), 0));
                (sset ? O1 : O0)[2 * rt + (q >> 2)].w[q & 3] = s2_pkh(x0, x1);
                e2[sset].bw[q] = s2_pk(x0, x1);
            });
            s2_sfor<16 - PI0>([&](auto jc) {
                constexpr int PI = PI0 + decltype(jc)::value;
                mask_pair_to(e2[PI >> 3].bits, e2[PI >> 3].bw[PI & 7]);
            });
        }
    };
    auto ffinish2 = [&](int l, auto rtc, auto sc, bool save, u16* srow, bool last) {
        constexpr int rt = decltype(rtc)::value, sset = decltype(sc)::value;
        const S2Frag* O = sset ? Ol : Oh;
        Ep2& es = e2[sset];
        uint32_t* mks = mkl + sset * C::MSET;
        if constexpr ((rt & 1) == 0) {
            es.mpend = es.bits << 8;
            if (last) mks[(l * C::NMW + (rt >> 1)) * 64 + lane] = es.mpend;
        } else {
            mks[(l * C::NMW + (rt >> 1)) * 64 + lane] = es.mpend | es.bits;
        }
        if (save) store_rt(srow, rtc, O[2 * rt], O[2 * rt + 1]);
    };
    f32x16 hacc[4];

    const float pi_f = 3.14159265358979323846f;

    struct SetSt {
        S2Frag g;
        float X0, X1, X2;
        int tile;
    };
    SetSt ss[NS];

    S2T_BEGIN(7);
    for (int it = 0; it < my_tiles; it += NS) {
        const int nset = min(NS, my_tiles - it);
        if constexpr (HF) {
            S2T_BEGIN(4);
            const int gp = (it / NS) & 1;
            int tl[2];
            long long sl[2];
            bool real[2];
            float Xs[2][3];
            S2Frag F0[2][NK0F > 0 ? NK0F : 1];
            s2_sfor<2>([&](auto sc) {
                constexpr int sset = decltype(sc)::value;
                real[sset] = it + sset < my_tiles;
                const int tile = hf_tile(it + sset);
                tl[sset] = tile;
                const int b = tile / tpp;
                const int p0 = (tile - b * tpp) * C::TPX + 32 * wave;
                sl[sset] = real[sset] ? (long long)b * a.geo.Np_pad + p0 : a.S + 32 * wave;
                const float* hm = proH(gp, sset);
                float Hm[9];
#pragma unroll
                for (int e = 0; e < 9; ++e) Hm[e] = hm[e];
                const int p = p0 + pxl;
                float x, y, u, v, X[3];
                if (a.geo.mode == 1) {
                    const int pc = min(p, Np - 1);
                    u = x = a.geo.coords[2 * (size_t)pc];
                    v = y = a.geo.coords[2 * (size_t)pc + 1];
                    X[0] = u;
                    X[1] = v;
                    X[2] = 1.0f;
                } else {
                    const int r = p / a.geo.w, cc = p - r * a.geo.w;
                    x = grid_coord(a.geo.x0 + cc, a.geo.W, a.geo.norm_w);
                    y = grid_coord(a.geo.y0 + r, a.geo.H, a.geo.norm_h);
                    warp_point(Hm, x, y, u, v, X, a.geo.bmm_small);
                }
                Xs[sset][0] = X[0];
                Xs[sset][1] = X[1];
                Xs[sset][2] = X[2];
                const float cd = h ? v : u;
                const bool st0 = !a.fwd_only && !a.feat0_recompute;
                u16* row0 = st0 ? ly_ptr(0, 0) + (sl[sset] >> 5) * ly_int(0, 3) * 32 + pxl * 16 + 8 * h : nullptr;
                s2_sfor<NK0F>([&](auto gc) {
                    constexpr int g = decltype(gc)::value;
                    float f[8] = {0.f, 0.f, 0.f, 0.f, 0.f, 0.f, 0.f, 0.f};
                    if constexpr (g < NK0F - 1) {
#pragma unroll
                        for (int j = 0; j < 4; ++j) {
                            const int k = 4 * g + j;
                            float sn = 0.f, co = 0.f;
                            if (k < L) {
                                band_sincos<true>(cd, k, sn, co);
                                if (a.c2f_on) {
                                    const float w = c2f_l[k];
                                    sn = sn * w;
                                    co = co * w;
                                }
                            }
                            f[j] = sn;
                            f[4 + j] = co;
                        }
                    } else {
                        f[0] = cd;
                    }
                    F0[sset][g].u = make_uint4(s2_pkh(f[0], f[1]), s2_pkh(f[2], f[3]), s2_pkh(f[4], f[5]), s2_pkh(f[6], f[7]));
                    if (st0) s2_st16(row0 + 512 * g, F0[sset][g].u);
                });
                if (st0) {
                    st_cur += NK0F;
                    if (16 * NK0F < ly_int(0, 3)) {
                        s2_st16(row0 + 512 * NK0F, make_uint4(0, 0, 0, 0));
                        st_cur += 1;
                    }
                }
            });
            S2T_END(4);
            auto fwd2_layer = [&](int l, const S2Frag* B0, const S2Frag* B1, auto nk_tag, auto ppk_tag) {
                constexpr int NK = decltype(nk_tag)::value, PPK = decltype(ppk_tag)::value;
                typedef std::integral_constant<bool, NK == NKH> PcL;
                const bool save = l + 1 < nl - 1 && !a.fwd_only;
                u16* srow[2];
#pragma unroll
                for (int q = 0; q < 2; ++q)
                    srow[q] = save ? ly_ptr(l + 1, 0) + (sl[q] >> 5) * ly_int(l + 1, 3) * 32 + pxl * 16 + 8 * h : nullptr;
                const int boff = ly_int(l, 2);
                const char* slotb = nullptr;
                s2_sfor<NRT>([&](auto rtc) {
                    constexpr int rt = decltype(rtc)::value;
                    f32x16& c0 = hacc[(rt & 1) ? 2 : 0];
                    f32x16& c1 = hacc[(rt & 1) ? 3 : 1];
                    f32x16& q0 = hacc[(rt & 1) ? 0 : 2];
                    f32x16& q1 = hacc[(rt & 1) ? 1 : 3];
                    const int sub = l == 0 ? rt % R0F : 0;
                    S2T_BEGIN(15);
                    c0 = bias_init(boff, rt);
                    c1 = c0;
                    S2T_END(15);
                    if (sub == 0) slotb = stage_begin(l == 0);
                    const char* slot = slotb + sub * NK * 1024;
                    if (l == 0 && rt == 0 && it + NS < my_tiles) {
                        issue_h(it + NS, gp ^ 1);
                        st_cur += 2;
                    }
                    if constexpr (rt == 0) {
                        S2T_BEGIN(8);
                        gemm2(c0, c1, slot, B0, B1, nk_tag, nohook, PcL(), F16t());
                        S2T_END(8);
                    } else {
                        typedef std::integral_constant<int, rt - 1> RP;
                        e2[0].bits = 0;
                        e2[1].bits = 0;
                        S2T_BEGIN(8);
                        gemm2(c0, c1, slot, B0, B1, nk_tag, [&](auto ksc, auto pc) {
                            hook2(q0, q1, Oh, Ol, RP(), ksc, pc, ppk_tag);
                        }, PcL(), F16t());
                        S2T_END(8);
                        S2T_BEGIN(13);
                        free_pairs(q0, q1, Oh, Ol, RP(), std::integral_constant<int, PPK * NK>());
                        S2T_END(13);
                        S2T_BEGIN(10);
                        ffinish2(l, RP(), I0(), save, srow[0], false);
                        ffinish2(l, RP(), I1(), save, srow[1], false);
                        S2T_END(10);
                    }
                    if constexpr (rt == NRT - 1) {
                        S2T_BEGIN(13);
                        e2[0].bits = 0;
                        e2[1].bits = 0;
                        free_pairs(c0, c1, Oh, Ol, rtc, I0());
                        ffinish2(l, rtc, I0(), save, srow[0], true);
                        ffinish2(l, rtc, I1(), save, srow[1], true);
                        S2T_END(13);
                    }
                });
#pragma unroll
                for (int k = 0; k < NKH; ++k) {
                    Bh[k] = Oh[k];
                    Bl[k] = Ol[k];
                }
            };
            S2T_BEGIN(5);
// ... 116 lines not shown
            const int ti = it + si;
            const int tile = tbase + ti * (int)gridDim.x;
            const int pb = ti & 1;
            const int b = tile / tpp;
            const int p0 = (tile - b * tpp) * C::TPX + 32 * wave;
            const long long slot0 = (long long)b * a.geo.Np_pad + p0;
            const int p = p0 + pxl;
            const bool valid = p < Np;
            const float* pro = pro_buf(pb);
            uint32_t* mks = mkl + si * C::MSET;

            float Hm[9];
#pragma unroll
            for (int e = 0; e < 9; ++e) Hm[e] = pro[4 * C::TPX + e];
            float x, y, u, v, X[3];
            if (a.geo.mode == 1) {
                const int pc = min(p, Np - 1);
                u = x = a.geo.coords[2 * (size_t)pc];
                v = y = a.geo.coords[2 * (size_t)pc + 1];
                X[0] = u;
                X[1] = v;
                X[2] = 1.0f;
            } else {
                const int r = p / a.geo.w, cc = p - r * a.geo.w;
                x = grid_coord(a.geo.x0 + cc, a.geo.W, a.geo.norm_w);
                y = grid_coord(a.geo.y0 + r, a.geo.H, a.geo.norm_h);
                warp_point(Hm, x, y, u, v, X, a.geo.bmm_small);
            }
            const float cd = h ? v : u;
            S2Frag F0h[C::NK0], F0l[C::NK0];
            {
                const int ng = nk0 - 1;
#pragma unroll
                for (int g = 0; g < C::NK0 - 1; ++g) {
                    if (g < ng) {
                        float f[8];
#pragma unroll
                        for (int j = 0; j < 4; ++j) {
                            const int k = 4 * g + j;
                            float s = 0.f, co = 0.f;
                            if (k < L) {
                                band_sincos<true>(cd, k, s, co);
                                if (a.c2f_on) {
                                    const float w = c2f_l[k];
                                    s = s * w;
                                    co = co * w;
                                }
                            }
                            f[j] = s;
                            f[4 + j] = co;
                        }
                        s2_split8<SPLIT>(f, F0h[g], F0l[g]);
                    }
                }
                float f[8] = {cd, 0.f, 0.f, 0.f, 0.f, 0.f, 0.f, 0.f};
                S2Frag rh, rl;
                s2_split8<SPLIT>(f, rh, rl);
#pragma unroll
                for (int g = 0; g < C::NK0; ++g)
                    if (g == ng) {
                        F0h[g] = rh;
                        F0l[g] = rl;
                    }
                if (!a.fwd_only && !a.feat0_recompute) {
                    u16* row = ly_ptr(0, 0) + (slot0 >> 5) * ly_int(0, 3) * 32 + pxl * 16 + 8 * h;
#pragma unroll
                    for (int g = 0; g < C::NK0; ++g)
                        if (g < nk0) s2_st16(row + 512 * g, F0h[g].u);
                    st_cur += nk0;
                    if (16 * nk0 < ly_int(0, 3)) {
                        s2_st16(row + 512 * nk0, make_uint4(0, 0, 0, 0));
                        st_cur += 1;
                    }
                }
            }

            S2T_END(4);
            S2T_BEGIN(5);
            auto fwd_layer = [&](int l, const S2Frag* Bhi, const S2Frag* Blo, int nk, auto nk_tag, auto ms_tag) {
                constexpr int MS = decltype(ms_tag)::value;
                typedef std::integral_constant<bool, decltype(nk_tag)::value == NKH> PcL;
                constexpr bool SPLITPK = SPLIT && MS == 1 && decltype(nk_tag)::value == NKH;
                const int nrt = FIX ? NRT : ly_int(l, 0);
                const bool save = l + 1 < nl - 1 && !a.fwd_only;
                u16* srow = save ? ly_ptr(l + 1, 0) + (slot0 >> 5) * ly_int(l + 1, 3) * 32 + pxl * 16 + 8 * h : nullptr;
                const int boff = ly_int(l, 2);
                const char* slot0 = nullptr;
                s2_sfor<NRT>([&](auto rtc) {
                    constexpr int rt = decltype(rtc)::value;
                    f32x16& cur = (rt & 1) ? acc1 : acc0;
                    f32x16& prv = (rt & 1) ? acc0 : acc1;
                    if (rt < nrt) {
                        const int sub = l == 0 ? rt % r0 : 0;
                        S2T_BEGIN(15);
                        cur = bias_init(boff, rt);
                        S2T_END(15);
                        if (sub == 0) slot0 = stage_begin(l == 0);
                        const char* slot = slot0 + sub * nk0 * 1024;
                        if (l == 0 && rt == 0 && ti + 1 < my_tiles) issue_pro(tile + (int)gridDim.x, pb ^ 1);
                        if constexpr (rt == 0) {
                            S2T_BEGIN(8);
                            gemm(cur, slot, Bhi, Blo, nk, MFt(), nk_tag, nohook, PcL());
                            S2T_END(8);
                        } else {
                            ep.bits = 0;
                            S2T_BEGIN(8);
                            gemm(cur, slot, Bhi, Blo, nk, MFt(), nk_tag, [&](auto ksc, auto pc) {
                                constexpr int ks = decltype(ksc)::value, p = decltype(pc)::value;
                                if constexpr (SPLITPK) {
                                    if constexpr (p == 0) {
                                        if constexpr ((ks & 1) == 0 && ks >= 2) fpackB(std::integral_constant<int, ks - 1>());
                                        frelu(prv, ksc);
                                    } else if constexpr (ks & 1) {
                                        fpackA(ksc);
                                    }
                                } else {
                                    s2_sfor<MS>([&](auto jc) {
                                        constexpr int e = ks * MS + decltype(jc)::value;
                                        if constexpr (e < 16) {
                                            if constexpr (p == 0) frelu(prv, std::integral_constant<int, e>());
                                            else fpack(std::integral_constant<int, e>());
                                        }
                                    });
                                }
                            }, PcL());
                            S2T_END(8);
                            S2T_BEGIN(13);
                            if constexpr (SPLITPK) fpackB(std::integral_constant<int, 15>());
                            if constexpr (FIX && !SPLITPK) {
                                constexpr int E0 = MS * decltype(nk_tag)::value;
                                if constexpr (E0 < 16) fsteps_free(prv, std::integral_constant<int, E0>());
                            } else {
                                s2_sfor<16>([&](auto ec) {
                                    if (decltype(ec)::value >= MS * nk) fstep(prv, ec);
                                });
                            }
                            S2T_END(13);
                            S2T_BEGIN(10);
                            ffinish(l, std::integral_constant<int, rt - 1>(), save, srow, mks, false);
                            S2T_END(10);
                        }
                        if (rt == nrt - 1) {
                            S2T_BEGIN(13);
                            ep.bits = 0;
                            if constexpr (FIX) fsteps_free(cur, std::integral_constant<int, 0>());
                            else s2_sfor<16>([&](auto ec) { fstep(cur, ec); });
                            ffinish(l, rtc, save, srow, mks, true);
                            S2T_END(13);
                        }
                    } else {
                        zero_out(Oh[2 * rt], Oh[2 * rt + 1], Ol[2 * rt], Ol[2 * rt + 1]);
                    }
                });
#pragma unroll
                for (int k = 0; k < NKH; ++k) {
                    Bh[k] = Oh[k];
                    if constexpr (SPLIT) Bl[k] = Ol[k];
                }
            };
            S2T_BEGIN(14);
            fwd_layer(0, F0h, F0l, nk0, NK0x(), std::integral_constant<int, 2>());
            S2T_END(14);
            for (int l = 1; l < nl - 1; ++l) fwd_layer(l, Bh, Bl, NKH, NKHt(), std::integral_constant<int, 1>());

            S2T_END(5);
            S2T_BEGIN(6);
            float g[3] = {0.f, 0.f, 0.f};
            {
                f32x16 acc = bias_init(ly_int(nl - 1, 2), 0);
                const char* slot = stage_begin(false);
                gemm(acc, slot, Bh, Bl, NKH, MFt(), NKHt(), nohook, PcOn());
                float* o = (a.rgb && valid && h == 0) ? a.rgb + ((size_t)b * Np + p) * 3 : dmy;
                float yv[3] = {0.f, 0.f, 0.f};
                if (h == 0) {
                    const float m = valid ? (a.mask ? pro[3 * C::TPX + 32 * wave + pxl] : 1.0f) : 0.f;
                    double sq = 0.0;
                    float sqf = 0.f;
#pragma unroll
                    for (int c = 0; c < 3; ++c) {
                        const float z = acc[c];
                        const float yy = 1.0f / (1.0f + expf(-z));
                        yv[c] = yy;
                        const float t = valid ? pro[c * C::TPX + 32 * wave + pxl] : 0.f;
                        const float xx = (yy - t) * m;
                        sqf += xx * xx;
                        const float d = (2.0f * xx) * m;
                        g[c] = (d * (1.0f - yy)) * yy;
                    }
                    sq = (double)sqf;
                    lsq += sq;
                    lms += (double)m;
                    bl0 += g[0];
                    bl1 += g[1];
                    bl2 += g[2];
                }
                s2_st12(o, yv[0], yv[1], yv[2]);
                st_cur += 1;
            }
            if (a.fwd_only) {
                S2T_END(6);
                continue;
            }
            S2Frag Bg;
            {
                float f[8] = {0.f, 0.f, 0.f, 0.f, 0.f, 0.f, 0.f, 0.f};
                if (h == 0) {
#pragma unroll
                    for (int c = 0; c < 3; ++c) {
                        f[c] = g[c];
                        f[4 + c] = g[c] - s2_lo16(s2_pk(g[c], 0.f));
                    }
                }
                S2Frag dumm;
                s2_split8<false>(f, Bg, dumm);
            }
            {
                if (h == 0) {
                    const uint32_t w0 = Bg.u.x, w1 = Bg.u.y, w2 = Bg.u.z, w3 = Bg.u.w;
                    gts[0 * 32 + pxl] = (u16)(w0 & 0xffff);
                    gts[1 * 32 + pxl] = (u16)(w0 >> 16);
                    gts[2 * 32 + pxl] = (u16)(w1 & 0xffff);
                    gts[4 * 32 + pxl] = (u16)(w2 & 0xffff);
                    gts[5 * 32 + pxl] = (u16)(w2 >> 16);
                    gts[6 * 32 + pxl] = (u16)(w3 & 0xffff);
                }
                const bf16x8 ga = *reinterpret_cast<const bf16x8*>(gts + (lane & 15) * 32 + 8 * (lane >> 4));
                const int gq = lane >> 4, q = (lane & 15) >> 2, pp = lane & 3;
                const int nkl = FIX ? NKH : a.Kl / 16;
                const int Klw = FIX ? HM : a.Kl;
#pragma unroll
                for (int ks = 0; ks < NKH; ++ks) {
                    if (ks < nkl) {
                        *reinterpret_cast<uint4*>(trs + (pxl * 2 + h) * 8) = Bh[ks].u;
                        const u16* b0 = trs + (8 * gq + q) * 16 + (pp & 1) * 8 + 4 * (pp >> 1);
                        i16x4 vv[2] = {s2_tr16(b0), s2_tr16(b0 + 4 * 16)};
                        const f32x4 r4 = __builtin_amdgcn_mfma_f32_16x16x32_bf16(ga, *reinterpret_cast<bf16x8*>(vv), (f32x4){}, 0, 0, 0);
                        float lo[3];
#pragma unroll
                        for (int c = 0; c < 3; ++c) lo[c] = __shfl_down(r4[c], 16, 64);
                        if (lane < 16) {
#pragma unroll
                            for (int c = 0; c < 3; ++c) wla[c * Klw + 16 * ks + lane] += r4[c] + lo[c];
                        }
                    }
                }
            }
            {
                SetSt cs;
                cs.g = Bg;
                cs.X0 = X[0];
                cs.X1 = X[1];
                cs.X2 = X[2];
                cs.tile = tile;
                if (si == 0) ss[0] = cs;
                else ss[NS - 1] = cs;
            }
            S2T_END(6);
        }
        }
        if (a.fwd_only) continue;
        if (nset < NS) {
            SetSt cs;
            cs.g.u = make_uint4(0, 0, 0, 0);
            cs.X0 = cs.X1 = 0.f;
            cs.X2 = 1.f;
            cs.tile = -1;
            ss[NS - 1] = cs;
        }

        S2T_BEGIN(2);
        long long sl0[NS];
        s2_sfor<NS>([&](auto sc) {
            constexpr int s = decltype(sc)::value;
            const int tl = ss[s].tile;
            long long v;
            if (tl < 0) {
                v = a.S + 32 * wave;
            } else {
                const int bb = tl / tpp;
                v = (long long)bb * a.geo.Np_pad + (tl - bb * tpp) * C::TPX + 32 * wave;
            }
            sl0[s] = v;
        });
        S2Frag* const Dh[2] = {Bh, Bl};
        S2Frag* const Do[2] = {Oh, Ol};
        EpSt eb;
        auto mks_b = [&](int s) -> const uint32_t* { return mkl + s * C::MSET; };
        {
            const int lmask = nl - 2;
            const int nrt = FIX ? NRT : ly_int(nl - 1, 1);
            u16* brow[NS];
            s2_sfor<NS>([&](auto sc) {
                brow[decltype(sc)::value] = ly_ptr(nl - 1, 1) + (sl0[decltype(sc)::value] >> 5) * ly_int(nl - 1, 4) * 32 + pxl * 16 + 8 * h;
            });
            S2Frag gB[NS];
            s2_sfor<NS>([&](auto sc) { gB[decltype(sc)::value] = ss[decltype(sc)::value].g; });
            const char* slot = stage_begin(true);
            if constexpr (HF) {
                if (it + NS < my_tiles) {
                    issue_tgt(it + NS);
                    st_cur += 4;
                }
            }
            s2_sfor<NRT>([&](auto rtc) {
                constexpr int rt = decltype(rtc)::value;
                if (rt < nrt) {
                    s2_sfor<NS>([&](auto sc) {
                        constexpr int s = decltype(sc)::value, i = rt * NS + s;
                        constexpr int sp = (i + NS - 1) % NS, rp = (i - 1 + NS) / NS - 1;
                        f32x16& cur = (i & 1) ? acc1 : acc0;
                        f32x16& prv = (i & 1) ? acc0 : acc1;
                        cur = (f32x16){};
                        if constexpr (i == 0) {
                            gemm(cur, slot, &gB[s], &gB[s], 1, MBt(), NK1t(), nohook, PcOff());
                        } else {
                            eb.mw = mks_b(sp)[(lmask * C::NMW + (rp >> 1)) * 64 + lane];
                            if constexpr (FIX) {
                                gemm(cur, slot + rt * 1024, &gB[s], &gB[s], 1, MBt(), NK1t(), nohook, PcOff());
                                bsteps_free(eb, prv, std::integral_constant<int, rp>());
                            } else {
                                gemm(cur, slot + rt * 1024, &gB[s], &gB[s], 1, MBt(), NK1t(), [&](auto, auto pc) {
                                    s2_sfor<8>([&](auto ec) {
                                        bstep(eb, prv, std::integral_constant<int, 8 * decltype(pc)::value + decltype(ec)::value>(),
                                              std::integral_constant<int, rp>());
                                    });
                                }, PcOff());
                            }
                            S2T_BEGIN(11);
                            bfinish(eb, Do[sp], std::integral_constant<int, rp>(), brow[sp]);
                            S2T_END(11);
                        }
                        if (s == NS - 1 && rt == nrt - 1) {
                            eb.mw = mks_b(s)[(lmask * C::NMW + (rt >> 1)) * 64 + lane];
                            if constexpr (FIX) bsteps_free(eb, cur, rtc);
                            else s2_sfor<16>([&](auto ec) { bstep(eb, cur, ec, rtc); });
                            bfinish(eb, Do[s], rtc, brow[s]);
                        }
                    });
                } else {
                    s2_sfor<NS>([&](auto sc) {
                        constexpr int s = decltype(sc)::value;
                        Do[s][2 * rt].u = Do[s][2 * rt + 1].u = make_uint4(0, 0, 0, 0);
                    });
                    if constexpr (SDZ) Ol[2 * rt].u = Ol[2 * rt + 1].u = make_uint4(0, 0, 0, 0);
                }
            });
#pragma unroll
            for (int k = 0; k < NKH; ++k) {
                s2_sfor<NS>([&](auto sc) { Dh[decltype(sc)::value][k] = Do[decltype(sc)::value][k]; });
                if constexpr (SDZ) Bl[k] = Ol[k];
            }
        }
        for (int l = nl - 2; l >= 1; --l) {
            const int lmask = l - 1;
            const int nrt = FIX ? NRT : ly_int(l, 1);
            u16* brow[NS];
            s2_sfor<NS>([&](auto sc) {
                brow[decltype(sc)::value] = ly_ptr(l, 1) + (sl0[decltype(sc)::value] >> 5) * ly_int(l, 4) * 32 + pxl * 16 + 8 * h;
            });
            if constexpr (J2) {
                EpSt ebs[2];
                s2_sfor<NRT>([&](auto rtc) {
                    constexpr int rt = decltype(rtc)::value;
                    f32x16& c0 = hacc[(rt & 1) ? 2 : 0];
                    f32x16& c1 = hacc[(rt & 1) ? 3 : 1];
                    f32x16& q0 = hacc[(rt & 1) ? 0 : 2];
                    f32x16& q1 = hacc[(rt & 1) ? 1 : 3];
                    const char* slot = stage_begin(false);
                    c0 = (f32x16){};
                    c1 = (f32x16){};
                    if constexpr (rt == 0) {
                        S2T_BEGIN(9);
                        gemm2(c0, c1, slot, Dh[0], Dh[1], NKHt(), nohook, PcOn(), std::integral_constant<bool, HF>());
                        S2T_END(9);
                    } else {
                        typedef std::integral_constant<int, rt - 1> RP;
                        ebs[0].mw = mks_b(0)[(lmask * C::NMW + ((rt - 1) >> 1)) * 64 + lane];
                        ebs[1].mw = mks_b(1)[(lmask * C::NMW + ((rt - 1) >> 1)) * 64 + lane];
                        S2T_BEGIN(9);
                        gemm2(c0, c1, slot, Dh[0], Dh[1], NKHt(), [&](auto ksc, auto pc) {
                            constexpr int ks = decltype(ksc)::value, p = decltype(pc)::value;
                            if constexpr (p < 2) {
                                constexpr int sset = ks >> 3;
                                bstep(ebs[sset], sset ? q1 : q0, std::integral_constant<int, 2 * (ks & 7) + p>(), RP());
                            }
                        }, PcOn(), std::integral_constant<bool, HF>());
                        S2T_END(9);
                        S2T_BEGIN(11);
                        bfinish(ebs[0], Do[0], RP(), brow[0]);
                        bfinish(ebs[1], Do[1], RP(), brow[1]);
                        S2T_END(11);
                    }
                    if constexpr (rt == NRT - 1) {
                        ebs[0].mw = mks_b(0)[(lmask * C::NMW + (rt >> 1)) * 64 + lane];
                        ebs[1].mw = mks_b(1)[(lmask * C::NMW + (rt >> 1)) * 64 + lane];
                        bsteps_free(ebs[0], c0, rtc);
                        bsteps_free(ebs[1], c1, rtc);
                        bfinish(ebs[0], Do[0], rtc, brow[0]);
                        bfinish(ebs[1], Do[1], rtc, brow[1]);
                    }
                });
            } else
            s2_sfor<NRT>([&](auto rtc) {
                constexpr int rt = decltype(rtc)::value;
                if (rt < nrt) {
                    const char* slot = stage_begin(false);
                    s2_sfor<NS>([&](auto sc) {
                        constexpr int s = decltype(sc)::value, i = rt * NS + s;
                        constexpr int sp = (i + NS - 1) % NS, rp = (i - 1 + NS) / NS - 1;
                        f32x16& cur = (i & 1) ? acc1 : acc0;
                        f32x16& prv = (i & 1) ? acc0 : acc1;
                        cur = (f32x16){};
                        if constexpr (i == 0) {
                            S2T_BEGIN(9);
                            gemm(cur, slot, Dh[s], SDZ ? Bl : Dh[s], NKH, MDt(), NKHt(), nohook, std::integral_constant<bool, s == 0>());
                            S2T_END(9);
                        } else {
                            eb.mw = mks_b(sp)[(lmask * C::NMW + (rp >> 1)) * 64 + lane];
                            S2T_BEGIN(9);
                            gemm(cur, slot, Dh[s], SDZ ? Bl : Dh[s], NKH, MDt(), NKHt(), [&](auto ksc, auto pc) {
                                if constexpr (decltype(pc)::value == 0) bstep(eb, prv, ksc, std::integral_constant<int, rp>());
                            }, std::integral_constant<bool, s == 0>());
                            S2T_END(9);
                            S2T_BEGIN(11);
                            bfinish(eb, Do[sp], std::integral_constant<int, rp>(), brow[sp]);
                            S2T_END(11);
                        }
                        if (s == NS - 1 && rt == nrt - 1) {
                            eb.mw = mks_b(s)[(lmask * C::NMW + (rt >> 1)) * 64 + lane];
                            if constexpr (FIX) bsteps_free(eb, cur, rtc);
                            else s2_sfor<16>([&](auto ec) { bstep(eb, cur, ec, rtc); });
                            bfinish(eb, Do[s], rtc, brow[s]);
                        }
                    });
                } else {
                    s2_sfor<NS>([&](auto sc) {
                        constexpr int s = decltype(sc)::value;
                        Do[s][2 * rt].u = Do[s][2 * rt + 1].u = make_uint4(0, 0, 0, 0);
                    });
                    if constexpr (SDZ) Ol[2 * rt].u = Ol[2 * rt + 1].u = make_uint4(0, 0, 0, 0);
                }
            });
#pragma unroll
            for (int k = 0; k < NKH; ++k) {
                s2_sfor<NS>([&](auto sc) { Dh[decltype(sc)::value][k] = Do[decltype(sc)::value][k]; });
                if constexpr (SDZ) Bl[k] = Ol[k];
            }
        }
        float dc[NS], cds[NS];
        s2_sfor<NS>([&](auto sc) {
            constexpr int s = decltype(sc)::value;
            dc[s] = 0.f;
            const float dd = ss[s].X2 + 1e-8f;
            cds[s] = h ? ss[s].X1 / dd : ss[s].X0 / dd;
        });
        {
            const int nta = FIX ? NTAF : a.nta;
            auto adj_band = [&](float& d, const float cd, const f32x16& pa, int t, auto ic) {
                constexpr int i = decltype(ic)::value;
                const int k = 8 * t + i;
                if (k < L) {
                    float sn, co;
                    band_sincos<true>(cd, k, sn, co);
                    float gs = pa[2 * i], gc = pa[2 * i + 1];
                    if (a.c2f_on) {
                        const float w = c2f_l[k];
                        gs = gs * w;
                        gc = gc * w;
                    }
                    d += (gs * co - gc * sn) * ldexpf(pi_f, k);
                }
            };
            auto adj_raw = [&](float& d, const f32x16& pa, int t) {
#pragma unroll
                for (int r = 0; r < 16; ++r)
                    if (16 * t + r == 2 * L) d += pa[r];
            };
            s2_sfor<C::NTA>([&](auto tc) {
                constexpr int t = decltype(tc)::value;
                if (t < nta) {
                    const char* slot = stage_begin(false);
                    s2_sfor<NS>([&](auto sc) {
                        constexpr int s = decltype(sc)::value, i = t * NS + s;
                        constexpr int sp = (i + NS - 1) % NS, tp = (i - 1 + NS) / NS - 1;
                        f32x16& cur = (i & 1) ? acc1 : acc0;
                        f32x16& prv = (i & 1) ? acc0 : acc1;
                        cur = (f32x16){};
                        if constexpr (i == 0) {
                            S2T_BEGIN(9);
                            gemm(cur, slot, Dh[s], Dh[s], NKH, MBt(), NKHt(), nohook, std::integral_constant<bool, s == 0>());
                            S2T_END(9);
                        } else {
                            S2T_BEGIN(9);
                            gemm(cur, slot, Dh[s], Dh[s], NKH, MBt(), NKHt(), [&](auto ksc, auto pc) {
                                constexpr int ks = decltype(ksc)::value;
                                if constexpr ((ks & 1) == 0 && decltype(pc)::value == 0)
                                    adj_band(dc[sp], cds[sp], prv, tp, std::integral_constant<int, ks / 2>());
                            }, std::integral_constant<bool, s == 0>());
                            S2T_END(9);
                            adj_raw(dc[sp], prv, tp);
                        }
                        if (s == NS - 1 && t == nta - 1) {
                            s2_sfor<8>([&](auto ic) { adj_band(dc[s], cds[s], cur, t, ic); });
                            adj_raw(dc[s], cur, t);
                        }
                    });
                }
            });
        }
        S2T_END(2);
        if constexpr (HF) {
            s2_sfor<NS>([&](auto sc) { dc[decltype(sc)::value] *= 1.0f / kGS; });
        }
        S2T_BEGIN(3);
        {
            float mine[NS];
            float* dst[NS];
            s2_sfor<NS>([&](auto sc) {
                constexpr int s = decltype(sc)::value;
                const SetSt& cs = ss[s];
                const float dother = __shfl_xor(dc[s], 32, 64);
                const float du = h ? dother : dc[s], dv = h ? dc[s] : dother;
                bool valid = false;
                float x = 0.f, y = 0.f;
                if (cs.tile >= 0) {
                    const int bb = cs.tile / tpp;
                    const int p = (cs.tile - bb * tpp) * C::TPX + 32 * wave + pxl;
                    valid = p < Np;
                    const int r = p / a.geo.w, cc = p - r * a.geo.w;
                    x = grid_coord(a.geo.x0 + cc, a.geo.W, a.geo.norm_w);
                    y = grid_coord(a.geo.y0 + r, a.geo.H, a.geo.norm_h);
                }
                float h9[9];
#pragma unroll
                for (int e = 0; e < 9; ++e) h9[e] = 0.f;
                if (h == 0 && valid) {
                    const float dd = cs.X2 + 1e-8f;
                    const float dX0 = du / dd, dX1 = dv / dd;
                    const float dd2 = dd * dd;
                    const float dX2 = (-du * cs.X0) / dd2 + (-dv * cs.X1) / dd2;
                    const float hom[3] = {x, y, 1.f};
#pragma unroll
                    for (int cc = 0; cc < 3; ++cc) {
                        h9[0 + cc] = dX0 * hom[cc];
                        h9[3 + cc] = dX1 * hom[cc];
                        h9[6 + cc] = dX2 * hom[cc];
                    }
                }
                mine[s] = 0.f;
#pragma unroll
                for (int e = 0; e < 9; ++e) {
                    const float sm = wave_total63(h9[e]);
                    const float sb = __int_as_float(__builtin_amdgcn_readlane(__float_as_int(sm), 63));
                    if (lane == e) mine[s] = sb;
                }
                dst[s] = lane < 9 ? a.dH_partial + (size_t)(sl0[s] / 32) * 9 + lane : dmy;
            });
            s2_sfor<NS>([&](auto sc) { s2_st4(dst[decltype(sc)::value], mine[decltype(sc)::value]); });
            st_cur += NS;
        }
        S2T_END(3);
    }
    S2T_END(7);
#ifdef MARF_STAMPS
    if (a.stamps && threadIdx.x == 0)
        for (int k = 0; k < 16; ++k) a.stamps[(size_t)blockIdx.x * 16 + k] = tacc[k];
#endif

    s2_wait_vm<0>();
    __syncthreads();
    double* red = reinterpret_cast<double*>(smem);
    {
        const double s0 = wave_total63(lsq), s1 = wave_total63(lms);
        const float t0 = wave_total63(bl0), t1 = wave_total63(bl1), t2 = wave_total63(bl2);
        if (lane == 63) {
            red[wave * 5 + 0] = s0;
            red[wave * 5 + 1] = s1;
            red[wave * 5 + 2] = (double)t0;
            red[wave * 5 + 3] = (double)t1;
            red[wave * 5 + 4] = (double)t2;
        }
    }
    __syncthreads();
    if (threadIdx.x < 5) {
        double s = 0.0;
        float sf = 0.f;
        for (int w = 0; w < NW; ++w) {
            s += red[w * 5 + threadIdx.x];
            sf += (float)red[w * 5 + threadIdx.x];
        }
        if (threadIdx.x < 2) a.loss_partial[2 * (size_t)blockIdx.x + threadIdx.x] = s;
        else a.blast_partial[3 * (size_t)blockIdx.x + threadIdx.x - 2] = sf;
    }
    for (int e = threadIdx.x; e < 3 * a.Kl; e += NW * 64) {
        float s = 0.f;
        for (int w = 0; w < NW; ++w)
            s += reinterpret_cast<const float*>(smem + a.lds_wave + w * a.lds_wave_bytes + 2048 + NS * C::MSET * 4)[e];
        a.wlast_partial[(size_t)blockIdx.x * 3 * a.Kl + e] = s;
    }
}


MARF_DEV int s2_l0_fwd_feature(int ks, int hh, int j, int L, int nk0) {
    const int ng = nk0 - 1;
    if (ks == ng) return j == 0 ? hh : -1;
    const int k = 4 * ks + (j & 3);
    if (k >= L) return -1;
    const bool cosp = j >= 4;
    return 2 + 2 * hh * L + (cosp ? L : 0) + k;
}
MARF_DEV int s2_l0_adj_feature(int t, int rho, int L) {
    const int hh = (rho >> 2) & 1, r = (rho & 3) + 4 * (rho >> 3);
    const int sl = 16 * t + r;
    if (sl == 2 * L) return hh;
    if (sl >= 2 * L) return -1;
    const int k = sl >> 1;
    return 2 + 2 * hh * L + ((sl & 1) ? L : 0) + k;
}

template <int HM, bool SPLIT, int NW, int MAXR, int NK0F = 0, int NTAF = 0>
__global__ __launch_bounds__(NW * 64, NW / 4) void k_step2(Step2Args a) {
    k_step2_body<HM, SPLIT, NW, MAXR, NK0F, NTAF, false>(a);
}

template <int HM, bool SPLIT, int NW, int MAXR, int NK0F = 0, int NTAF = 0>
__global__ __launch_bounds__(NW * 64, NW / 4) void k_step2dz(Step2Args a) {
    k_step2_body<HM, SPLIT, NW, MAXR, NK0F, NTAF, true>(a);
}

template <int HM, int NW, int MAXR, int NK0F, int NTAF>
__global__ __launch_bounds__(NW * 64, NW / 4) void k_step2h(Step2Args a) {
    k_step2_body<HM, true, NW, MAXR, NK0F, NTAF, false, true>(a);
}

MARF_DEV int s2_kperm(int ks, int hh, int j) { return 16 * ks + 8 * (j >> 2) + 4 * hh + (j & 3); }

__global__ void k_pack2(const float* __restrict__ params, u16* __restrict__ prog, float* __restrict__ bias_out,
                        int* __restrict__ kmap, Pack2Args a) {
    const int per_slot = a.slot_bytes / 2;
// ... 162 lines not shown
```

masking-bundle-adjusting-neural-radiance-fields_amd/csrc/marf_wgrad.hip:

```cpp
#include "marf_args.h"

#include <algorithm>
#include <cstdlib>
#include <cstring>

namespace marf {

struct Feat0Src {
    GeoDev geo;
    const float* c2f_w;
    int L, nk0;
};

struct WgArgs {
    const void* dz;
    const void* feat;
    Feat0Src f0;
    long long S;
    int ldz, ldf;
    int M, K;
    int chunk;
    int n_chunks;
    int n_oblk_c;
    float* partial;
    float* bpartial;
    long long s_lo, s_len;
    int rng_n, part0;
    int t16;
};

template <int RT, int CT>
struct WgGeo {
    static constexpr int BM = 4 * RT * 32;
    static constexpr int BN = 2 * CT * 32;
};

MARF_DEV i16x4 tr_read(const u16* p) {
    return __builtin_amdgcn_ds_read_tr16_b64_v4i16((__attribute__((address_space(3))) i16x4*)(p));
}

MARF_DEV size_t t16_off(long long p, int f, int ld) {
    return ((size_t)(p >> 5) * (size_t)(ld >> 4) + (size_t)(f >> 4)) * 512 + (size_t)(p & 31) * 16 + (f & 15);
}
MARF_DEV int t16_lds(int r, int c, int nb) {
    const int b = c >> 4;
    return ((r >> 5) * nb + b) * 1024 + (r & 31) * 32 + (c & 15) * 2;
}

template <class P, int RT, int CT, int SP>
MARF_DEV void wgrad_body(const WgArgs& a, int chunk_id, int ob, char* smem) {
    typedef typename P::T T;
    constexpr int BM = WgGeo<RT, CT>::BM, BN = WgGeo<RT, CT>::BN;
    constexpr int PADE = sizeof(T) == 2 ? 32 : 4;
    constexpr int LDZ = BM + PADE, LDF = BN + PADE;
    constexpr int VEC = 16 / sizeof(T);
    constexpr int NVZ = SP * BM / VEC / 512;
    constexpr int NVF = SP * BN / VEC / 512;
    T* tz = reinterpret_cast<T*>(smem);
    T* tf = tz + SP * LDZ;
    const int lane = threadIdx.x & 63, wave = __builtin_amdgcn_readfirstlane(threadIdx.x >> 6);
    const int wr = wave >> 1, wc = wave & 1;
    const int m0 = (ob / a.n_oblk_c) * BM, k0 = (ob % a.n_oblk_c) * BN;
    const long long s_begin = (long long)chunk_id * a.chunk;
    const long long s_end = min(s_begin + a.chunk, a.S);
    const bool do_bias = a.bpartial && (ob % a.n_oblk_c) == 0;
    const T* dz = reinterpret_cast<const T*>(a.dz);
    const T* ft = reinterpret_cast<const T*>(a.feat);

    f32x16 acc[RT][CT];
#pragma unroll
    for (int i = 0; i < RT; ++i)
#pragma unroll
        for (int j = 0; j < CT; ++j) acc[i][j] = (f32x16){};
    float bsum = 0.f;

    uint4 rz[NVZ], rf[NVF];
    auto load_stage = [&](long long s0) {
#pragma unroll
        for (int q = 0; q < NVZ; ++q) {
            const int e = threadIdx.x + 512 * q;
            const int r = e / (BM / VEC), c = (e % (BM / VEC)) * VEC;
            rz[q] = make_uint4(0, 0, 0, 0);
            if (s0 + r < s_end && m0 + c < a.M)
                rz[q] = *reinterpret_cast<const uint4*>(dz + (a.t16 ? t16_off(s0 + r, m0 + c, a.ldz) : (size_t)((s0 + r) * a.ldz + m0 + c)));
        }
#pragma unroll
        for (int q = 0; q < NVF; ++q) {
            const int e = threadIdx.x + 512 * q;
            const int r = e / (BN / VEC), c = (e % (BN / VEC)) * VEC;
            rf[q] = make_uint4(0, 0, 0, 0);
            if (s0 + r < s_end && k0 + c < a.K)
                rf[q] = *reinterpret_cast<const uint4*>(ft + (a.t16 ? t16_off(s0 + r, k0 + c, a.ldf) : (size_t)((s0 + r) * a.ldf + k0 + c)));
        }
    };
    auto store_stage = [&]() {
#pragma unroll
        for (int q = 0; q < NVZ; ++q) {
            const int e = threadIdx.x + 512 * q;
            const int r = e / (BM / VEC), c = (e % (BM / VEC)) * VEC;
            *reinterpret_cast<uint4*>(tz + r * LDZ + c) = rz[q];
        }
#pragma unroll
        for (int q = 0; q < NVF; ++q) {
            const int e = threadIdx.x + 512 * q;
            const int r = e / (BN / VEC), c = (e % (BN / VEC)) * VEC;
            *reinterpret_cast<uint4*>(tf + r * LDF + c) = rf[q];
        }
    };

    if (s_begin < s_end) load_stage(s_begin);
    for (long long s0 = s_begin; s0 < s_end; s0 += SP) {
        __syncthreads();
        store_stage();
        __syncthreads();
        if (s0 + SP < s_end) load_stage(s0 + SP);

        if (do_bias) {
            constexpr int RSTEP = 512 / BM > 0 ? 512 / BM : 1;
            const int c = threadIdx.x % BM, r0 = threadIdx.x / BM;
            if (r0 < RSTEP)
                for (int r = r0; r < SP; r += RSTEP) bsum += P::tof(tz[r * LDZ + c]);
        }

        if constexpr (sizeof(T) == 2) {
            const int g = lane >> 4, gi = lane & 15, q = gi >> 2, p4 = gi & 3;
#pragma unroll
            for (int ks = 0; ks < SP; ks += 16) {
                const int r0 = ks + 8 * (g >> 1) + q;
                typename P::frag af[RT], bf[CT];
#pragma unroll
                for (int i = 0; i < RT; ++i) {
                    const int c0 = (wr * RT + i) * 32 + 16 * (g & 1) + 4 * p4;
                    const u16* base = reinterpret_cast<const u16*>(tz) + r0 * LDZ + c0;
                    i16x4 lo = tr_read(base), hi = tr_read(base + 4 * LDZ);
                    i16x4 v[2] = {lo, hi};
                    af[i] = *reinterpret_cast<typename P::frag*>(v);
                }
#pragma unroll
                for (int j = 0; j < CT; ++j) {
                    const int c0 = (wc * CT + j) * 32 + 16 * (g & 1) + 4 * p4;
                    const u16* base = reinterpret_cast<const u16*>(tf) + r0 * LDF + c0;
                    i16x4 lo = tr_read(base), hi = tr_read(base + 4 * LDF);
                    i16x4 v[2] = {lo, hi};
                    bf[j] = *reinterpret_cast<typename P::frag*>(v);
                }
#pragma unroll
                for (int i = 0; i < RT; ++i)
#pragma unroll
                    for (int j = 0; j < CT; ++j) acc[i][j] = P::mma32(af[i], bf[j], acc[i][j]);
            }
        } else {
            const int h = lane >> 5, rl = lane & 31;
            for (int ks = 0; ks < SP; ks += 2) {
                typename P::frag af[RT], bf[CT];
#pragma unroll
                for (int i = 0; i < RT; ++i) af[i] = tz[(ks + h) * LDZ + (wr * RT + i) * 32 + rl];
#pragma unroll
                for (int j = 0; j < CT; ++j) bf[j] = tf[(ks + h) * LDF + (wc * CT + j) * 32 + rl];
#pragma unroll
                for (int i = 0; i < RT; ++i)
#pragma unroll
                    for (int j = 0; j < CT; ++j) acc[i][j] = P::mma32(af[i], bf[j], acc[i][j]);
            }
        }
    }

    float* out = a.partial + (size_t)chunk_id * a.M * a.K;
#pragma unroll
    for (int i = 0; i < RT; ++i)
#pragma unroll
        for (int j = 0; j < CT; ++j) {
            const int k = k0 + (wc * CT + j) * 32 + (lane & 31);
#pragma unroll
            for (int r = 0; r < 16; ++r) {
                const int m = m0 + (wr * RT + i) * 32 + acc_row(lane, r);
                if (m < a.M && k < a.K) out[(size_t)m * a.K + k] = acc[i][j][r];
            }
        }
    if (do_bias) {
        __syncthreads();
        float* bs = reinterpret_cast<float*>(smem);
        bs[threadIdx.x] = bsum;
        __syncthreads();
        constexpr int RSTEP = 512 / BM > 0 ? 512 / BM : 1;
        if ((int)threadIdx.x < BM && m0 + (int)threadIdx.x < a.M) {
            float s = 0.f;
            for (int r = 0; r < RSTEP; ++r) s += bs[threadIdx.x + r * BM];
            a.bpartial[(size_t)chunk_id * a.M + m0 + threadIdx.x] = s;
        }
    }
}

template <class P, int RT, int CT, int SP>
__global__ __launch_bounds__(512, 1) void k_wgrad(WgArgs a) {
    extern __shared__ __attribute__((aligned(16))) char smem[];
    wgrad_body<P, RT, CT, SP>(a, blockIdx.x, blockIdx.y, smem);
}

MARF_DEV void glds16(const char* src, unsigned lds) {
    unsigned keep;
    asm volatile("s_mov_b32 %0, m0\n\ts_mov_b32 m0, %2\n\ts_nop 0\n\tglobal_load_lds_dwordx4 %1, off\n\ts_mov_b32 m0, %0"
                 : "=&s"(keep)
                 : "v"(src), "s"(lds)
                 : "memory");
}

constexpr int F0_PATCHES = 4;
constexpr int WG_SPH = 32, WG_NBUF_H = 4, WG_SP0 = 64, WG_NBUF_0 = 3, WG_NBUF_96 = 4;

MARF_DEV int swz(int r, int c) {
    return r * 512 + ((((c >> 3) ^ (4 * (r & 3)))) << 4) + (c & 7) * 2;
}


template <int N>
MARF_DEV void wait_vm() {
    asm volatile("s_waitcnt vmcnt(%0)" ::"n"(N) : "memory");
}

template <int KF>
MARF_DEV int foff(int r, int c) {
    if constexpr (KF == 256) return swz(r, c);
    else return r * (KF * 2) + c * 2;
}

template <class P, int NBUF, int SP, int KF, bool F0 = false, bool T16 = false>
MARF_DEV void wgrad_dma_body(const WgArgs& a, int chunk_id, int ob, char* smem) {
    static_assert(KF == 256 || KF == 96, "feat width");
    static_assert(!F0 || (KF == 96 && SP % 32 == 0), "feat_0 recompute: the 96-wide layer-0 stage, 32-row blocks");
    constexpr int WR = KF == 256 ? 4 : 8, WC = 8 / WR;
    constexpr int RT = 256 / 32 / WR, CT = KF / 32 / WC;
    constexpr int ZB = SP * 512;
    constexpr int FB = SP * KF * 2;
    constexpr int NGZ = ZB / 8192;
    constexpr int NGF = F0 ? 0 : (FB + 8191) / 8192;
    static_assert(NGZ * 8192 == ZB && FB % 1024 == 0 && NBUF >= 2 && NBUF <= 6, "stage shape");
    constexpr int PER_ST = NGZ + NGF;
    constexpr int STB = ZB + FB;
    const int lane = threadIdx.x & 63, wave = __builtin_amdgcn_readfirstlane(threadIdx.x >> 6);
    const int wr = wave / WC, wc = wave % WC;
    const int m0 = (ob / a.n_oblk_c) * 256, k0 = (ob % a.n_oblk_c) * KF;
    long long s_begin, s_end;
    int pidx;
    if (a.rng_n > 0) {
        const long long nst = a.s_len / SP;
        s_begin = a.s_lo + (long long)chunk_id * nst / a.rng_n * SP;
        s_end = a.s_lo + (long long)(chunk_id + 1) * nst / a.rng_n * SP;
        pidx = a.part0 + chunk_id;
    } else {
        s_begin = (long long)chunk_id * a.chunk;
        s_end = min(s_begin + a.chunk, a.S);
        pidx = chunk_id;
    }
    const int n_st = s_end > s_begin ? (int)((s_end - s_begin) / SP) : 0;
    const bool do_bias = a.bpartial != nullptr && k0 == 0;
    const char* dz = reinterpret_cast<const char*>(a.dz) + (size_t)m0 * 2;
    const char* ft = reinterpret_cast<const char*>(a.feat) + (size_t)k0 * 2;
    const size_t ldzb = (size_t)a.ldz * 2, ldfb = (size_t)a.ldf * 2;

    const unsigned lds0 = (unsigned)(uintptr_t)(__attribute__((address_space(3))) char*)smem;
    const unsigned junk = lds0 + NBUF * STB;
    float* f0_h = reinterpret_cast<float*>(smem + NBUF * STB);
    float* f0_w = f0_h + 9 * F0_PATCHES;
    float* f0_uv = f0_w + 32;
    int f0_b0 = 0, f0_p0 = 0;
    float f0_inv_w = 0.f;
    if constexpr (F0) {
        const GeoDev& gg = a.f0.geo;
        f0_b0 = (int)(s_begin / gg.Np_pad);
        f0_p0 = (int)(s_begin - (long long)f0_b0 * gg.Np_pad);
        f0_inv_w = 1.0f / (float)gg.w;
        for (int e = threadIdx.x; e < 9 * F0_PATCHES; e += 512) {
            const int bb = min(f0_b0 + e / 9, gg.B - 1);
            f0_h[e] = gg.Hm[9 * (size_t)bb + e % 9];
        }
        if (threadIdx.x < 32) f0_w[threadIdx.x] = (a.f0.c2f_w && (int)threadIdx.x < a.f0.L) ? a.f0.c2f_w[threadIdx.x] : 1.0f;
        wait_vm<0>();
        __syncthreads();
    }
    auto warp_rows = [&](int st, int r) {
        const GeoDev& gg = a.f0.geo;
        int p = f0_p0 + st * SP + r, bb = f0_b0;
        for (int i = 0; i < F0_PATCHES && p >= gg.Np_pad; ++i) {
            p -= gg.Np_pad;
            ++bb;
        }
        int rr = (int)((float)p * f0_inv_w);
        rr -= rr * gg.w > p;
        rr += (rr + 1) * gg.w <= p;
        const int cc = p - rr * gg.w;
        const float x = grid_coord(gg.x0 + cc, gg.W, gg.norm_w);
        const float y = grid_coord(gg.y0 + rr, gg.H, gg.norm_h);
        float u, v, X[3];
        warp_point(f0_h + 9 * min(bb - f0_b0, F0_PATCHES - 1), x, y, u, v, X, gg.bmm_small);
        f0_uv[((st % (NBUF + 1)) * SP + r) * 2] = u;
        f0_uv[((st % (NBUF + 1)) * SP + r) * 2 + 1] = v;
    };
    if constexpr (F0) {
        if ((int)threadIdx.x < SP * NBUF && (int)threadIdx.x / SP < n_st) warp_rows(threadIdx.x / SP, threadIdx.x % SP);
        __syncthreads();
    }
    auto compute_f0 = [&](int st, int buf_off) {
#pragma unroll
      for (int rb = 0; rb < SP; rb += 32) {
        const int r = rb + (threadIdx.x >> 4), sub = threadIdx.x & 15;
        const float u = f0_uv[((st % (NBUF + 1)) * SP + r) * 2], v = f0_uv[((st % (NBUF + 1)) * SP + r) * 2 + 1];
        char* row = smem + buf_off + r * (KF * 2);
        const int h = sub >> 3, k0 = 2 * (sub & 7);
        const float cd = h ? v : u;
        float sn[2] = {0.f, 0.f}, cs[2] = {0.f, 0.f};
#pragma unroll
        for (int i = 0; i < 2; ++i) {
            const int k = k0 + i;
            if (k < a.f0.L) {
                band_sincos<true>(cd, k, sn[i], cs[i]);
                if (a.f0.c2f_w) {
                    sn[i] = sn[i] * f0_w[k];
                    cs[i] = cs[i] * f0_w[k];
                }
            }
        }
        const int ng = a.f0.nk0 - 1;
        const int g = k0 >> 2, j = k0 & 3;
        if (g < ng) {
            *reinterpret_cast<uint32_t*>(row + 2 * (16 * g + 8 * h + j)) = P::pk2(sn[0], sn[1]);
            *reinterpret_cast<uint32_t*>(row + 2 * (16 * g + 8 * h + 4 + j)) = P::pk2(cs[0], cs[1]);
        }
        for (int c = 16 * ng + 2 * sub; c < KF; c += 32) {
            const int hc = (c - 16 * ng) >> 3;
            const float val = (c - 16 * ng) == 8 * hc && hc < 2 ? (hc ? v : u) : 0.f;
            *reinterpret_cast<uint32_t*>(row + 2 * c) = P::pk2(val, 0.f);
        }
      }
    };
    auto t16_lane = [&](int ld, int blk0, int nb, int seg) -> unsigned {
        const int tr = seg / nb, b = seg - tr * nb;
        return ((unsigned)tr * (unsigned)(ld >> 4) + (unsigned)(blk0 + b)) * 1024u + (unsigned)lane * 16u;
    };
    unsigned t16z[NGZ > 0 ? NGZ : 1], t16f[NGF > 0 ? NGF : 1];
    if constexpr (T16) {
#pragma unroll
        for (int q = 0; q < NGZ; ++q) t16z[q] = t16_lane(a.ldz, m0 >> 4, 16, q * 8 + wave);
#pragma unroll
        for (int q = 0; q < NGF; ++q) t16f[q] = t16_lane(a.ldf, k0 >> 4, KF >> 4, q * 8 + wave < (FB >> 10) ? q * 8 + wave : 0);
    }
    auto issue = [&](int st) {
        const unsigned buf = lds0 + (st % NBUF) * STB;
        const long long row0 = s_begin + (long long)st * SP;
        const char* z16 = reinterpret_cast<const char*>(a.dz) + (size_t)(row0 >> 5) * (size_t)(a.ldz >> 4) * 1024;
        const char* f16 = reinterpret_cast<const char*>(a.feat) + (size_t)(row0 >> 5) * (size_t)(a.ldf >> 4) * 1024;
#pragma unroll
        for (int q = 0; q < NGZ; ++q) {
            const int seg = q * 8 + wave;
            if constexpr (T16) {
                glds16(z16 + t16z[q], __builtin_amdgcn_readfirstlane(buf + seg * 1024));
                continue;
            }
            const int r = seg * 2 + (lane >> 5);
            const int c16 = (lane & 31) ^ (4 * (r & 3));
            glds16(dz + (size_t)(row0 + r) * ldzb + c16 * 16, __builtin_amdgcn_readfirstlane(buf + seg * 1024));
        }
#pragma unroll
        for (int q = 0; q < NGF; ++q) {
            const int seg = q * 8 + wave;
            if constexpr (T16) {
                const bool real = seg * 1024 < FB;
                glds16(f16 + t16f[q], __builtin_amdgcn_readfirstlane(real ? buf + ZB + seg * 1024 : junk));
            } else if constexpr (KF == 256) {
                const int r = seg * 2 + (lane >> 5);
                const int c16 = (lane & 31) ^ (4 * (r & 3));
                glds16(ft + (size_t)(row0 + r) * ldfb + c16 * 16, __builtin_amdgcn_readfirstlane(buf + ZB + seg * 1024));
            } else {
                const bool real = seg * 1024 < FB;
                const char* src = ft + (size_t)row0 * ldfb + (real ? seg * 1024 : 0) + lane * 16;
                glds16(src, __builtin_amdgcn_readfirstlane(real ? buf + ZB + seg * 1024 : junk));
            }
        }
        if constexpr (F0) compute_f0(st, (st % NBUF) * STB + ZB);
    };

    f32x16 acc[RT][CT];
#pragma unroll
    for (int i = 0; i < RT; ++i)
#pragma unroll
        for (int j = 0; j < CT; ++j) acc[i][j] = (f32x16){};
    float bsum = 0.f;

    for (int st = 0; st < NBUF - 1 && st < n_st; ++st) issue(st);
    const int g = lane >> 4, gi = lane & 15, q4 = gi >> 2, p4 = gi & 3;
    for (int st = 0; st < n_st; ++st) {
        const int ahead = min(NBUF - 2, n_st - 1 - st);
        if (ahead >= 4) wait_vm<4 * PER_ST>();
        else if (ahead == 3) wait_vm<3 * PER_ST>();
        else if (ahead == 2) wait_vm<2 * PER_ST>();
        else if (ahead == 1) wait_vm<PER_ST>();
        else wait_vm<0>();
        asm volatile("s_waitcnt lgkmcnt(0)" ::: "memory");
        __builtin_amdgcn_s_barrier();
        asm volatile("" ::: "memory");
        if (st + NBUF - 1 < n_st) issue(st + NBUF - 1);
        if constexpr (F0) {
            if (wave == 7 && lane < SP && st + NBUF < n_st) warp_rows(st + NBUF, lane);
        }

        const char* tz = smem + (st % NBUF) * STB;
        const char* tf = tz + ZB;
        if (do_bias) {
            const int c = threadIdx.x & 255;
#pragma unroll
            for (int r = 0; r < SP; r += 2) {
                const int rr = r + (threadIdx.x >> 8);
                bsum += P::tof(*reinterpret_cast<const u16*>(tz + (T16 ? t16_lds(rr, c, 16) : swz(rr, c))));
            }
        }
#pragma unroll
        for (int ks = 0; ks < SP; ks += 16) {
            const int r0 = ks + 8 * (g >> 1) + q4;
            typename P::frag af[RT], bf[CT];
#pragma unroll
            for (int i = 0; i < RT; ++i) {
                const int c = (wr * RT + i) * 32 + 16 * (g & 1) + 4 * p4;
                const u16* base = reinterpret_cast<const u16*>(tz + (T16 ? t16_lds(r0, c, 16) : swz(r0, c)));
                const u16* base4 = T16 ? reinterpret_cast<const u16*>(tz + t16_lds(r0 + 4, c, 16)) : base + 4 * 256;
                i16x4 v[2] = {tr_read(base), tr_read(base4)};
                af[i] = *reinterpret_cast<typename P::frag*>(v);
            }
#pragma unroll
            for (int j = 0; j < CT; ++j) {
                const int c = (wc * CT + j) * 32 + 16 * (g & 1) + 4 * p4;
                constexpr bool FT = T16 && !F0;
                const u16* base = reinterpret_cast<const u16*>(tf + (FT ? t16_lds(r0, c, KF >> 4) : foff<KF>(r0, c)));
                const u16* base4 = FT ? reinterpret_cast<const u16*>(tf + t16_lds(r0 + 4, c, KF >> 4)) : base + 4 * KF;
                i16x4 v[2] = {tr_read(base), tr_read(base4)};
                bf[j] = *reinterpret_cast<typename P::frag*>(v);
            }
#pragma unroll
            for (int i = 0; i < RT; ++i)
#pragma unroll
                for (int j = 0; j < CT; ++j) acc[i][j] = P::mma32(af[i], bf[j], acc[i][j]);
        }
    }

    float* out = a.partial + (size_t)pidx * a.M * a.K + (size_t)m0 * a.K + k0;
#pragma unroll
    for (int i = 0; i < RT; ++i)
#pragma unroll
        for (int j = 0; j < CT; ++j) {
            const int k = (wc * CT + j) * 32 + (lane & 31);
            if (KF != 256 && k0 + k >= a.K) continue;
#pragma unroll
            for (int r = 0; r < 16; ++r) out[(size_t)((wr * RT + i) * 32 + acc_row(lane, r)) * a.K + k] = acc[i][j][r];
        }
    if (do_bias) {
        __syncthreads();
        float* bs = reinterpret_cast<float*>(smem);
        bs[threadIdx.x] = bsum;
        __syncthreads();
        if (threadIdx.x < 256)
            a.bpartial[(size_t)pidx * a.M + m0 + threadIdx.x] = bs[threadIdx.x] + bs[threadIdx.x + 256];
    }
}

template <class P, int NBUF, int SP, int KF, bool F0 = false, bool T16 = false>
__global__ __launch_bounds__(512, 1) void k_wgrad_dma(WgArgs a) {
    extern __shared__ __attribute__((aligned(16))) char smem[];
    const int n_ob = (a.M / 256) * a.n_oblk_c;
    int chunk_id, ob;
    if (n_ob > 1 && a.n_chunks % 8 == 0) {
        const int grp = blockIdx.x / (8 * n_ob), rem = blockIdx.x % (8 * n_ob);
        chunk_id = grp * 8 + rem % 8;
        ob = rem / 8;
    } else {
        chunk_id = blockIdx.x % a.n_chunks;
        ob = blockIdx.x / a.n_chunks;
    }
    wgrad_dma_body<P, NBUF, SP, KF, F0, T16>(a, chunk_id, ob, smem);
}

template <class P>
__global__ __launch_bounds__(256) void k_wgrad_last(const float* __restrict__ glast, const void* feat_v, long long S,
                                                    int ldf, int K, int chunk, float* partial, float* bpartial) {
    typedef typename P::T T;
    constexpr int VEC = 16 / sizeof(T);
    __shared__ float red[3072];
    __shared__ float redb[256][3];
    const T* feat = reinterpret_cast<const T*>(feat_v);
    const int ngrp = K / VEC;
    const int lanes = 256 / ngrp;
    const int t = threadIdx.x;
    const int fg = t % ngrp, pl = t / ngrp;
    const bool active = pl < lanes;
    const long long s_begin = (long long)blockIdx.x * chunk;
    const long long s_end = min(s_begin + chunk, S);
    float acc[VEC][3];
#pragma unroll
    for (int v = 0; v < VEC; ++v) acc[v][0] = acc[v][1] = acc[v][2] = 0.f;
    float b0 = 0.f, b1 = 0.f, b2 = 0.f;
    if (active) {
        long long s = s_begin + pl;
#pragma unroll 4
        for (; s < s_end; s += lanes) {
            const float4 g = *reinterpret_cast<const float4*>(glast + s * 4);
            const uint4 raw = *reinterpret_cast<const uint4*>(feat + s * ldf + fg * VEC);
            const T* f = reinterpret_cast<const T*>(&raw);
#pragma unroll
            for (int v = 0; v < VEC; ++v) {
                const float x = P::tof(f[v]);
                acc[v][0] += g.x * x;
                acc[v][1] += g.y * x;
                acc[v][2] += g.z * x;
            }
            b0 += g.x;
            b1 += g.y;
            b2 += g.z;
        }
    }
    float* out = partial + (size_t)blockIdx.x * 3 * K;
    for (int lane_id = 0; lane_id < lanes; ++lane_id) {
        if (active && pl == lane_id) {
#pragma unroll
            for (int v = 0; v < VEC; ++v)
#pragma unroll
                for (int c = 0; c < 3; ++c) {
                    float* r = &red[(fg * VEC + v) * 3 + c];
                    *r = lane_id == 0 ? acc[v][c] : *r + acc[v][c];
                }
        }
        __syncthreads();
    }
    for (int e = t; e < K * 3; e += 256) out[(e % 3) * K + e / 3] = red[e];
    redb[t][0] = (active && fg == 0) ? b0 : 0.f;
    redb[t][1] = (active && fg == 0) ? b1 : 0.f;
    redb[t][2] = (active && fg == 0) ? b2 : 0.f;
    __syncthreads();
    if (t < 3) {
        float sb = 0.f;
        for (int i = 0; i < 256; ++i) sb += redb[i][t];
        bpartial[(size_t)blockIdx.x * 3 + t] = sb;
    }
}

__global__ __launch_bounds__(256) void k_fold_partials(const float* __restrict__ partial, const float* __restrict__ bpartial,
                                                       int n, int per, long long E, int Eb, float* __restrict__ out,
                                                       float* __restrict__ bout) {
    const long long e = blockIdx.x * 256LL + threadIdx.x;
    const int g = blockIdx.y;
    const int c0 = g * per, c1 = min(n, c0 + per);
    if (e < E) {
        float acc[4] = {0.f, 0.f, 0.f, 0.f};
        int c = c0;
#pragma unroll 2
        for (; c + 4 <= c1; c += 4)
#pragma unroll
            for (int u = 0; u < 4; ++u) acc[u] += partial[(size_t)(c + u) * E + e];
        for (int u = 0; c < c1; ++c, ++u) acc[u] += partial[(size_t)c * E + e];
        out[(size_t)g * E + e] = (acc[0] + acc[1]) + (acc[2] + acc[3]);
    } else if (e < E + Eb) {
        const int eb = (int)(e - E);
        float s = 0.f;
        for (int c = c0; c < c1; ++c) s += bpartial[(size_t)c * Eb + eb];
        bout[(size_t)g * Eb + eb] = s;
    }
}


constexpr int WF_MAXJ = 6;

struct WgLayersArgs {
    WgArgs a[WF_MAXJ];
    int n_chunks;
};

template <class P, int NBUF, int SP, int KF>
__global__ __launch_bounds__(512, 1) void k_wgrad_dma_layers(WgLayersArgs la) {
    extern __shared__ __attribute__((aligned(16))) char smem[];
    const int l = blockIdx.x / la.n_chunks, c = blockIdx.x - l * la.n_chunks;
    wgrad_dma_body<P, NBUF, SP, KF, false, true>(la.a[l], c, 0, smem);
}

struct WgRedJob {
    const float* partial;
    const float* bpartial;
    int n_chunks, M, K, Mo, Ko, blk0;
    float* dW;
    float* db;
    const int* kmap;
    float post;
};
struct WgRedArgs {
    WgRedJob job[WF_MAXJ];
    int n_jobs;
    const float* gscale;
    const float* denom;
};

MARF_DEV void wgrad_reduce_block(const float* __restrict__ partial, const float* __restrict__ bpartial, int n_chunks,
                                 int M, int K, int Mo, int Ko, float* __restrict__ dW, float* __restrict__ db,
                                 const float* __restrict__ gscale, const float* __restrict__ denom,
                                 const int* __restrict__ kmap, int blk, float (*red)[64], float post = 1.f) {
    const long long n = (long long)Mo * Ko;
    const long long e = blk * 64LL + (threadIdx.x & 63);
    const int g = threadIdx.x >> 6;
    const int c0 = (int)((long long)n_chunks * g / 4), c1 = (int)((long long)n_chunks * (g + 1) / 4);
    float s = 0.f;
    if (e < n + Mo) {
        const float* src;
        size_t stride;
        if (e < n) {
            const int m = (int)(e / Ko), k = (int)(e % Ko);
            src = partial + (size_t)m * K + (kmap ? kmap[k] : k);
            stride = (size_t)M * K;
        } else {
            src = bpartial + (e - n);
            stride = (size_t)M;
        }
        float acc[8] = {0.f, 0.f, 0.f, 0.f, 0.f, 0.f, 0.f, 0.f};
        int c = c0;
        for (; c + 8 <= c1; c += 8) {
#pragma unroll
            for (int u = 0; u < 8; ++u) acc[u] += src[(size_t)(c + u) * stride];
        }
        for (int u = 0; c < c1; ++c, ++u) acc[u] += src[(size_t)c * stride];
        s = ((acc[0] + acc[1]) + (acc[2] + acc[3])) + ((acc[4] + acc[5]) + (acc[6] + acc[7]));
    }
    red[g][threadIdx.x & 63] = s;
    __syncthreads();
    if (g == 0 && e < n + Mo) {
        float t = ((red[0][threadIdx.x] + red[1][threadIdx.x]) + red[2][threadIdx.x]) + red[3][threadIdx.x];
        if (gscale) t = t * (gscale[0] / denom[0]);
        if (post != 1.f) t = t * post;
        if (e < n) dW[e] = t;
        else db[e - n] = t;
    }
}

__global__ __launch_bounds__(256) void k_wgrad_reduce_layers(WgRedArgs r) {
    __shared__ float red[4][64];
    int j = 0;
    while (j < r.n_jobs - 1 && (int)blockIdx.x >= r.job[j + 1].blk0) ++j;
    const WgRedJob& q = r.job[j];
    wgrad_reduce_block(q.partial, q.bpartial, q.n_chunks, q.M, q.K, q.Mo, q.Ko, q.dW, q.db, r.gscale, r.denom, q.kmap,
                       (int)blockIdx.x - q.blk0, red, q.post);
}

__global__ __launch_bounds__(256) void k_wgrad_reduce(const float* __restrict__ partial,
                                                      const float* __restrict__ bpartial, int n_chunks, int M, int K,
                                                      int Mo, int Ko, float* __restrict__ dW, float* __restrict__ db,
                                                      const float* __restrict__ gscale, const float* __restrict__ denom,
                                                      const int* __restrict__ kmap, float post) {
    __shared__ float red[4][64];
    wgrad_reduce_block(partial, bpartial, n_chunks, M, K, Mo, Ko, dW, db, gscale, denom, kmap, blockIdx.x, red, post);
}

}

using namespace marf;

template <class P, int RT, int CT>
static hipError_t launch_wg(const WgArgs& a, int n_chunks, int n_oblk, hipStream_t s) {
    typedef typename P::T T;
    constexpr int SP = 64;
    constexpr int BM = WgGeo<RT, CT>::BM, BN = WgGeo<RT, CT>::BN;
    constexpr int PADE = sizeof(T) == 2 ? 32 : 4;
    size_t lds = (size_t)SP * (BM + PADE + BN + PADE) * sizeof(T);
    if (lds < 512 * sizeof(float)) lds = 512 * sizeof(float);
    {
        hipError_t e = ensure_dynamic_lds((const void*)k_wgrad<P, RT, CT, SP>, lds);
        if (e != hipSuccess) return e;
    }
    hipLaunchKernelGGL((k_wgrad<P, RT, CT, SP>), dim3(n_chunks, n_oblk), dim3(512), lds, s, a);
    return hipGetLastError();
}

static bool wgrad_dma_enabled() {
    const char* e = getenv("MARF_WGRAD_DMA");
    return !(e && e[0] == '0');
}

template <class P, int KF, bool F0 = false, bool T16 = false>
static hipError_t launch_wg_dma(WgArgs a, int n_chunks, hipStream_t s) {
    a.n_chunks = n_chunks;
    a.n_oblk_c = (a.K + KF - 1) / KF;
    constexpr int SP = F0 ? WG_SP0 : KF == 256 ? WG_SPH : 32;
    constexpr int NBUF = KF == 256 ? WG_NBUF_H : F0 ? WG_NBUF_0 : WG_NBUF_96;
    const size_t lds = (size_t)NBUF * SP * (512 + KF * 2) + (KF == 256 ? 0 : 1024) + (F0 ? (9 * F0_PATCHES + 32 + (NBUF + 1) * SP * 2) * 4 : 0);
    {
        hipError_t e = ensure_dynamic_lds((const void*)k_wgrad_dma<P, NBUF, SP, KF, F0, T16>, lds);
        if (e != hipSuccess) return e;
    }
    hipLaunchKernelGGL((k_wgrad_dma<P, NBUF, SP, KF, F0, T16>), dim3(n_chunks * (a.M / 256) * a.n_oblk_c), dim3(512), lds, s,
                       a);
    return hipGetLastError();
}

hipError_t marf_launch_wgrad(int dtype, const void* dz, int ldz, const void* feat, int ldf, long long S, int M, int K,
                             int chunk, int n_chunks, float* partial, float* bpartial, hipStream_t s,
                             const WgRange* rng, bool t16) {
    WgArgs a;
    memset(&a, 0, sizeof(a));
    a.t16 = t16 ? 1 : 0;
    if (rng) {
        a.s_lo = rng->s_lo;
        a.s_len = rng->s_len;
        a.rng_n = n_chunks = rng->n;
        a.part0 = rng->part0;
        chunk = 64;
    }
    a.dz = dz;
    a.feat = feat;
    a.S = S;
    a.ldz = ldz;
    a.ldf = ldf;
    a.M = M;
    a.K = K;
    a.chunk = chunk;
    a.partial = partial;
    a.bpartial = bpartial;
    int cfg;
    if (M >= 256 && K >= 192) cfg = 0;
    else if (M >= 256 && K > 64) cfg = 3;
    else if (M >= 256) cfg = 1;
    else cfg = 2;
    int BM = cfg == 2 ? 128 : 256, BN = cfg == 0 ? 256 : (cfg == 3 ? 128 : 64);
    int nr = (M + BM - 1) / BM, nc = (K + BN - 1) / BN;
    a.n_oblk_c = nc;
    const bool dma = M % 256 == 0 && ldz % 8 == 0 && ldz >= M && S % 32 == 0 && chunk % 32 == 0 &&
                     (long long)n_chunks * (M / 256) * ((K + 255) / 256) <= 0x7fffffff && wgrad_dma_enabled();
    const bool dma256 = dma && K % 256 == 0 && ldf % 8 == 0 && ldf >= K && S % WG_SPH == 0 && chunk % WG_SPH == 0,
               dma96 = dma && K == 96 && ldf == 96;
    if (rng && (dtype == 0 || !(dma256 || dma96))) return hipErrorInvalidValue;
    if (t16 && dtype == 0) return hipErrorInvalidValue;
    if (dtype == 1) {
        if (dma256) return t16 ? launch_wg_dma<PrecBF16, 256, false, true>(a, n_chunks, s) : launch_wg_dma<PrecBF16, 256>(a, n_chunks, s);
        if (dma96) return t16 ? launch_wg_dma<PrecBF16, 96, false, true>(a, n_chunks, s) : launch_wg_dma<PrecBF16, 96>(a, n_chunks, s);
        if (cfg == 0) return launch_wg<PrecBF16, 2, 4>(a, n_chunks, nr * nc, s);
        if (cfg == 3) return launch_wg<PrecBF16, 2, 2>(a, n_chunks, nr * nc, s);
        if (cfg == 1) return launch_wg<PrecBF16, 2, 1>(a, n_chunks, nr * nc, s);
        return launch_wg<PrecBF16, 1, 1>(a, n_chunks, nr * nc, s);
    }
    if (dtype == 2) {
        if (dma256) return t16 ? launch_wg_dma<PrecF16, 256, false, true>(a, n_chunks, s) : launch_wg_dma<PrecF16, 256>(a, n_chunks, s);
        if (dma96) return t16 ? launch_wg_dma<PrecF16, 96, false, true>(a, n_chunks, s) : launch_wg_dma<PrecF16, 96>(a, n_chunks, s);
        if (cfg == 0) return launch_wg<PrecF16, 2, 4>(a, n_chunks, nr * nc, s);
        if (cfg == 3) return launch_wg<PrecF16, 2, 2>(a, n_chunks, nr * nc, s);
        if (cfg == 1) return launch_wg<PrecF16, 2, 1>(a, n_chunks, nr * nc, s);
        return launch_wg<PrecF16, 1, 1>(a, n_chunks, nr * nc, s);
    }
    if (cfg == 0) return launch_wg<PrecF32, 2, 4>(a, n_chunks, nr * nc, s);
    if (cfg == 3) return launch_wg<PrecF32, 2, 2>(a, n_chunks, nr * nc, s);
    if (cfg == 1) return launch_wg<PrecF32, 2, 1>(a, n_chunks, nr * nc, s);
    return launch_wg<PrecF32, 1, 1>(a, n_chunks, nr * nc, s);
}

bool marf_wgrad_range_ok(int dtype, int M, int ldz, int K, int ldf) {
    if (dtype != 1 && dtype != 2) return false;
    if (!(M % 256 == 0 && ldz % 8 == 0 && ldz >= M && wgrad_dma_enabled())) return false;
    return (K % 256 == 0 && ldf % 8 == 0 && ldf >= K) || (K == 96 && ldf == 96);
}

bool marf_wgrad_l0_recompute_ok(int M, int ldz, int ldf0, long long S, int chunk, int n_chunks, long long Np_pad) {
    return M == 256 && ldz % 8 == 0 && ldz >= M && (ldf0 == 96 || ldf0 == 64) && S % WG_SP0 == 0 && chunk % WG_SP0 == 0 &&
           (long long)n_chunks <= 0x7fffffff && Np_pad < (1 << 24) && (chunk + Np_pad - 1) / Np_pad + 1 <= F0_PATCHES;
}

hipError_t marf_launch_wgrad_l0_recompute(const void* dz, int ldz, const GeoDev& geo, const float* c2f_w, int L,
                                          int nk0, int K0, long long S, int M, int chunk, int n_chunks, float* partial,
                                          float* bpartial, hipStream_t s, const WgRange* rng, int dtype) {
    WgArgs a;
    memset(&a, 0, sizeof(a));
    if (rng) {
        a.s_lo = rng->s_lo;
        a.s_len = rng->s_len;
        a.rng_n = n_chunks = rng->n;
        a.part0 = rng->part0;
    }
    a.dz = dz;
    a.feat = nullptr;
    a.f0.geo = geo;
    a.f0.c2f_w = c2f_w;
    a.f0.L = L;
    a.f0.nk0 = nk0;
    a.S = S;
    a.ldz = ldz;
    a.ldf = 96;
    a.M = M;
    a.K = K0;
    a.t16 = 1;
    a.chunk = chunk;
    a.partial = partial;
    a.bpartial = bpartial;
    if (dtype == 2) return launch_wg_dma<PrecF16, 96, true, true>(a, n_chunks, s);
    return launch_wg_dma<PrecBF16, 96, true, true>(a, n_chunks, s);
}

bool marf_wgrad_fused_ok(const WgFusedLayer* layers, int n_layers, long long S, int chunk, int n_chunks,
                         long long Np_pad) {
    if (!layers || n_layers < 1 || n_layers > WF_MAXJ || n_chunks < 1 || chunk < 64 || chunk % 64) return false;
    if (const char* e = getenv("MARF_WGRAD_FUSED")) {
        if (e[0] == '0') return false;
    }
    int n_l0 = 0;
    for (int i = 0; i < n_layers; ++i) {
        const WgFusedLayer& L = layers[i];
        if (L.Mo > L.M || L.Ko > L.K || !L.partial || !L.bpartial || !L.dW || !L.db) return false;
        switch (L.kind) {
            case 0:
                if (!(L.M == 256 && L.K == 256 && L.ldz % 8 == 0 && L.ldz >= L.M && L.ldf % 8 == 0 && L.ldf >= L.K &&
                      S % WG_SPH == 0 && chunk % WG_SPH == 0 && wgrad_dma_enabled()))
                    return false;
                break;
            case 1:
                if (!marf_wgrad_l0_recompute_ok(L.M, L.ldz, L.K, S, chunk, n_chunks, Np_pad)) return false;
                ++n_l0;
                break;
            case 2:
                ++n_l0;
                break;
            case 3:
                if (L.n_parts < 1 || L.n_parts > 1024) return false;
                break;
            default: return false;
        }
    }
    return n_l0 <= 1;
}

hipError_t marf_launch_wgrad_fused(const WgFusedLayer* layers, int n_layers, long long S, int chunk, int n_chunks,
                                   const GeoDev& f0_geo, const float* c2f_w, int L, int nk0, const float* gscale,
                                   const float* denom, hipStream_t s, hipStream_t s2, hipEvent_t fork,
                                   hipEvent_t join, int dtype, float post) {
    hipError_t e;
    const WgFusedLayer* l0 = nullptr;
    for (int i = 0; i < n_layers; ++i)
        if (layers[i].kind == 1 || layers[i].kind == 2) l0 = &layers[i];
    if (l0) {
        if ((e = hipEventRecord(fork, s)) != hipSuccess || (e = hipStreamWaitEvent(s2, fork, 0)) != hipSuccess) return e;
        if (l0->kind == 1)
            e = marf_launch_wgrad_l0_recompute(l0->dz, l0->ldz, f0_geo, c2f_w, L, nk0, l0->K, S, l0->M, chunk, n_chunks, l0->partial,
                                               l0->bpartial, s2, nullptr, dtype);
        else
            e = marf_launch_wgrad(dtype, l0->dz, l0->ldz, l0->feat, l0->ldf, S, l0->M, l0->K, chunk, n_chunks, l0->partial,
                                  l0->bpartial, s2, nullptr, true);
        if (e != hipSuccess) return e;
        if ((e = hipEventRecord(join, s2)) != hipSuccess) return e;
    }
    WgLayersArgs la;
    memset(&la, 0, sizeof(la));
    la.n_chunks = n_chunks;
    int nh = 0;
    for (int i = 0; i < n_layers; ++i) {
        const WgFusedLayer& Ly = layers[i];
        if (Ly.kind != 0) continue;
        WgArgs& a = la.a[nh++];
        a.dz = Ly.dz;
        a.feat = Ly.feat;
        a.S = S;
        a.ldz = Ly.ldz;
        a.ldf = Ly.ldf;
        a.M = Ly.M;
        a.K = Ly.K;
        a.chunk = chunk;
        a.n_chunks = n_chunks;
        a.n_oblk_c = 1;
        a.partial = Ly.partial;
        a.bpartial = Ly.bpartial;
        a.t16 = 1;
    }
    if (nh) {
        const size_t lds = (size_t)WG_NBUF_H * WG_SPH * (512 + 256 * 2);
        auto go = [&](auto prec) -> hipError_t {
            typedef decltype(prec) P;
            hipError_t er = ensure_dynamic_lds((const void*)k_wgrad_dma_layers<P, WG_NBUF_H, WG_SPH, 256>, lds);
            if (er != hipSuccess) return er;
            hipLaunchKernelGGL((k_wgrad_dma_layers<P, WG_NBUF_H, WG_SPH, 256>), dim3(nh * n_chunks), dim3(512), lds, s, la);
            return hipGetLastError();
        };
        e = dtype == 2 ? go(PrecF16()) : go(PrecBF16());
        if (e != hipSuccess) return e;
    }
    if (l0 && (e = hipStreamWaitEvent(s, join, 0)) != hipSuccess) return e;
    WgRedArgs r;
    memset(&r, 0, sizeof(r));
    r.n_jobs = n_layers;
    r.gscale = gscale;
    r.denom = denom;
    int blk = 0;
    for (int i = 0; i < n_layers; ++i) {
        const WgFusedLayer& Ly = layers[i];
        WgRedJob& q = r.job[i];
        q.partial = Ly.partial;
        q.bpartial = Ly.bpartial;
        q.n_chunks = Ly.kind == 3 ? Ly.n_parts : n_chunks;
        q.M = Ly.M;
        q.K = Ly.K;
        q.Mo = Ly.Mo;
        q.Ko = Ly.Ko;
        q.dW = Ly.dW;
        q.db = Ly.db;
        q.kmap = Ly.kmap;
        q.post = Ly.kind == 3 ? 1.f : post;
        q.blk0 = blk;
        blk += (int)(((long long)Ly.Mo * Ly.Ko + Ly.Mo + 63) / 64);
    }
    hipLaunchKernelGGL(k_wgrad_reduce_layers, dim3(blk), dim3(256), 0, s, r);
    return hipGetLastError();
}

hipError_t marf_launch_wgrad_last(int dtype, const float* glast, const void* feat, long long S, int ldf, int K, int chunk,
                                  int n_chunks, float* partial, float* bpartial, hipStream_t s) {
    if (dtype == 1)
        hipLaunchKernelGGL(k_wgrad_last<PrecBF16>, dim3(n_chunks), dim3(256), 0, s, glast, feat, S, ldf, K, chunk,
                           partial, bpartial);
    else if (dtype == 2)
        hipLaunchKernelGGL(k_wgrad_last<PrecF16>, dim3(n_chunks), dim3(256), 0, s, glast, feat, S, ldf, K, chunk,
                           partial, bpartial);
    else
        hipLaunchKernelGGL(k_wgrad_last<PrecF32>, dim3(n_chunks), dim3(256), 0, s, glast, feat, S, ldf, K, chunk,
                           partial, bpartial);
    return hipGetLastError();
}

hipError_t marf_launch_wgrad_reduce(const float* partial, const float* bpartial, int n_chunks, int M, int K, int Mo,
                                    int Ko, float* dW, float* db, hipStream_t s, const float* gscale,
                                    const float* denom, float* scratch, const int* kmap, float post) {
    if (n_chunks > 1024 && scratch) {
        const int per = (n_chunks + 255) / 256;
        const int G = (n_chunks + per - 1) / per;
        const long long E = (long long)M * K;
        float* out = scratch;
        float* bout = scratch + (size_t)G * E;
        dim3 grid((unsigned)((E + M + 255) / 256), G);
        hipLaunchKernelGGL(k_fold_partials, grid, dim3(256), 0, s, partial, bpartial, n_chunks, per, E, M, out, bout);
        hipError_t err = hipGetLastError();
        if (err != hipSuccess) return err;
        partial = out;
        bpartial = bout;
        n_chunks = G;
    }
    long long n = (long long)Mo * Ko + Mo;
    int blocks = (int)((n + 63) / 64);
    hipLaunchKernelGGL(k_wgrad_reduce, dim3(blocks), dim3(256), 0, s, partial, bpartial, n_chunks, M, K, Mo, Ko, dW, db,
                       gscale, denom, kmap, post);
    return hipGetLastError();
}
```

Measured before the change: 359.5 million pixels/s.

## Recompute last hidden-layer dz in wgrad instead of saving it

Rather than writing the last hidden layer's bf16 dz activations (S x 256) to global memory in the step kernel, it stores only the compact output gradient and mask bits per 32-pixel set plus a copy of the last-layer weights. The wgrad kernel then recomputes dz with an extra small MFMA per stage before the usual weight-gradient GEMM. This trades a large HBM write and read for extra MFMA work and LDS in the wgrad kernel. It is enabled by default when the network shape and variant conditions hold.

```diff
diff --git a/masking-bundle-adjusting-neural-radiance-fields_amd/csrc/marf_abi.hip b/masking-bundle-adjusting-neural-radiance-fields_amd/csrc/marf_abi.hip
--- a/masking-bundle-adjusting-neural-radiance-fields_amd/csrc/marf_abi.hip
+++ b/masking-bundle-adjusting-neural-radiance-fields_amd/csrc/marf_abi.hip
@@ -825,6 +825,8 @@
     size_t feat[MARF_MAX_LAYERS], dz[MARF_MAX_LAYERS];
     size_t dH, loss, blast, wlast, dummy, c2f, kmap, part, bpart, total;
     size_t partl[MARF_MAX_LAYERS], bpartl[MARF_MAX_LAYERS];
+    bool dzl;
+    size_t dzl_g, dzl_mk, dzl_w;
     int grid, n_tiles;
     int nblk;
     long long S;
@@ -869,6 +871,18 @@
     const long long chunk = wgrad_chunk(S);
     return marf_wgrad_l0_recompute_ok(n->Mp[0], n->Kp[1], n->s2.ldf0, S, (int)chunk, (int)((S + chunk - 1) / chunk),
                                       g.Np_pad);
+}
+
+static bool dzl_recompute(const marf_net* n, const GeoDev& g, long long S, bool pipe_on) {
+    const char* e = getenv("MARF_DZL_RECOMPUTE");
+    if (e && e[0] == '0') return false;
+    const int nl = n->n_layers;
+    if (n->s2.variant != 1 || n->s2.dz || pipe_on || g.mode != MARF_GEO_GRID || nl < 3 || n->s2.NMW != 4) return false;
+    for (int l = 0; l < nl - 1; ++l)
+        if (n->Mp[l] != 256 || (l > 0 && n->Kp[l] != 256)) return false;
+    const long long chunk = wgrad_chunk(S);
+    return marf_wgrad_dzl_ok(n->Mp[nl - 2], n->Kp[nl - 1], n->Kp[nl - 2], n->Kp[nl - 2], S, (int)chunk,
+                             (int)((S + chunk - 1) / chunk));
 }
 
 
@@ -957,9 +971,20 @@
     }
     p.dz[0] = 0;
     const long long Ssink = p.S + q.TPX;
+    p.dzl = !render && dzl_recompute(n, g, p.S, p.pipe.on != 0);
     for (int l = 1; l < nl; ++l) {
         p.dz[l] = off;
+        if (p.dzl && l == nl - 1) continue;
         off += rup(Ssave * Ssink * n->Kp[l] * 2, 256);
+    }
+    p.dzl_g = p.dzl_mk = p.dzl_w = 0;
+    if (p.dzl) {
+        p.dzl_g = off;
+        off += rup(Ssink / 32 * DZL_G_SET, 256);
+        p.dzl_mk = off;
+        off += rup(Ssink / 32 * DZL_MK_SET, 256);
+        p.dzl_w = off;
+        off += DZL_W_BYTES;
     }
     p.dH = off;
     off += rup(Ssave * Ssink / q.PX * 9 * 4, 256);
@@ -1084,6 +1109,11 @@
     a.bias = (const float*)(pk + q.bias_off);
     a.nbias = q.nbias;
     a.feat0_recompute = !render && l0_recompute(net, a.geo, p.S) ? 1 : 0;
+    if (p.dzl) {
+        a.dzl_g = sv + p.dzl_g;
+        a.dzl_mk = sv + p.dzl_mk;
+        a.dzl_w = sv + p.dzl_w;
+    }
     a.gt = d_gt;
     a.mask = d_mask;
     a.rgb = d_rgb;
@@ -1095,7 +1125,7 @@
         y.ldf = l == 0 ? q.ldf0 : net->Kp[l];
         y.ldz = net->Kp[l];
         y.feat = l < nl - 1 && !render ? (u16*)(sv + p.feat[l]) : nullptr;
-        y.dz = l >= 1 && !render ? (u16*)(sv + p.dz[l]) : nullptr;
+        y.dz = l >= 1 && !render && !(p.dzl && l == nl - 1) ? (u16*)(sv + p.dz[l]) : nullptr;
     }
     a.dH_partial = (float*)(sv + p.dH);
     a.loss_partial = (double*)(sv + p.loss);
@@ -1187,6 +1217,8 @@
     const int nl = net->n_layers;
     const int sdt = q.variant == 3 ? 2 : 1;
     const float post = q.variant == 3 ? 1.0f / 1024.0f : 1.0f;
+    WgDzlSrc dzl_src = {nullptr, nullptr, nullptr};
+    if (p.dzl) dzl_src = {sv + p.dzl_g, sv + p.dzl_mk, sv + p.dzl_w};
     if (d_dparams && !p.pipe.on && p.fused_res) {
         const long long chunk = wgrad_chunk(p.S);
         const int n_chunks = (int)((p.S + chunk - 1) / chunk);
@@ -1225,6 +1257,7 @@
             x.dW = d_dparams + net->w_off[l];
             x.db = d_dparams + net->b_off[l];
             x.kmap = l == 0 ? kmap : nullptr;
+            if (p.dzl && l == nl - 2) x.dzl = dzl_src;
         }
         if (marf_wgrad_fused_ok(Lf, nf, p.S, (int)chunk, n_chunks, g.Np_pad)) {
             PipeStreams* st = nullptr;
@@ -1302,7 +1335,8 @@
                            "step_backward wgrad_l0 (feat_0 recomputed)");
                 else
                     HIPCHK(marf_launch_wgrad(sdt, sv + p.dz[l + 1], net->Kp[l + 1], sv + p.feat[l], K, p.S, net->Mp[l], K,
-                                             (int)chunk, n_chunks, part, bpart, s, nullptr, true),
+                                             (int)chunk, n_chunks, part, bpart, s, nullptr, true,
+                                             p.dzl && l == nl - 2 ? &dzl_src : nullptr),
                            "step_backward wgrad");
             }
             {
diff --git a/masking-bundle-adjusting-neural-radiance-fields_amd/csrc/marf_args.h b/masking-bundle-adjusting-neural-radiance-fields_amd/csrc/marf_args.h
--- a/masking-bundle-adjusting-neural-radiance-fields_amd/csrc/marf_args.h
+++ b/masking-bundle-adjusting-neural-radiance-fields_amd/csrc/marf_args.h
@@ -67,6 +67,8 @@
     int n_layers;
     PackLayer ly[MARF_MAX_LAYERS];
 };
+
+constexpr int DZL_G_SET = 512, DZL_MK_SET = 1024, DZL_W_BYTES = 16384;
 
 struct S2Layer {
     int nrt;
@@ -105,6 +107,9 @@
     int fwd_only;
     int feat0_recompute;
     const float* pro_fallback;
+    char* dzl_g;
+    char* dzl_mk;
+    char* dzl_w;
     int lds_pro, lds_bias, lds_c2f, lds_layers, lds_wave, lds_wave_bytes, lds_total;
 };
 
@@ -138,13 +143,19 @@
     int n, part0;
 };
 bool marf_wgrad_range_ok(int dtype, int M, int ldz, int K, int ldf);
+struct WgDzlSrc {
+    const char* g;
+    const char* mk;
+    const char* w;
+};
+bool marf_wgrad_dzl_ok(int M, int ldz, int K, int ldf, long long S, int chunk, int n_chunks);
 bool marf_wgrad_l0_recompute_ok(int M, int ldz, int ldf0, long long S, int chunk, int n_chunks, long long Np_pad);
 hipError_t marf_launch_wgrad_l0_recompute(const void* dz, int ldz, const GeoDev& geo, const float* c2f_w, int L,
                                           int nk0, int K0, long long S, int M, int chunk, int n_chunks, float* partial,
                                           float* bpartial, hipStream_t s, const WgRange* rng = nullptr, int dtype = 1);
 hipError_t marf_launch_wgrad(int dtype, const void* dz, int ldz, const void* feat, int ldf, long long S, int M, int K,
                              int chunk, int n_chunks, float* partial, float* bpartial, hipStream_t s,
-                             const WgRange* rng = nullptr, bool t16 = false);
+                             const WgRange* rng = nullptr, bool t16 = false, const WgDzlSrc* dzl = nullptr);
 struct WgFusedLayer {
     int kind;
     const void* dz;
@@ -157,6 +168,7 @@
     float* dW;
     float* db;
     const int* kmap;
+    WgDzlSrc dzl;
 };
 bool marf_wgrad_fused_ok(const WgFusedLayer* layers, int n_layers, long long S, int chunk, int n_chunks,
                          long long Np_pad);
diff --git a/masking-bundle-adjusting-neural-radiance-fields_amd/csrc/marf_step2.hip b/masking-bundle-adjusting-neural-radiance-fields_amd/csrc/marf_step2.hip
--- a/masking-bundle-adjusting-neural-radiance-fields_amd/csrc/marf_step2.hip
+++ b/masking-bundle-adjusting-neural-radiance-fields_amd/csrc/marf_step2.hip
@@ -1,17 +1,11 @@
 #include <type_traits>
 
 #include "marf_args.h"
+#include "marf_step2_dev.h"
 
 namespace marf {
 
 
-MARF_DEV void s2_glds4(const void* src, unsigned lds) {
-    unsigned keep;
-    asm volatile("s_mov_b32 %0, m0\n\ts_mov_b32 m0, %2\n\ts_nop 0\n\tglobal_load_lds_dword %1, off\n\ts_mov_b32 m0, %0"
-                 : "=&s"(keep)
-                 : "v"(src), "s"(lds)
-                 : "memory");
-}
 typedef uint32_t s2_u32x2 __attribute__((ext_vector_type(2)));
 typedef uint32_t s2_u32x4 __attribute__((ext_vector_type(4)));
 MARF_DEV void s2_st8(void* dst, uint32_t a, uint32_t b) {
@@ -42,36 +36,6 @@
 
 MARF_DEV i16x4 s2_tr16(const u16* p) {
     return __builtin_amdgcn_ds_read_tr16_b64_v4i16((__attribute__((address_space(3))) i16x4*)(p));
-}
-
-template <int... I, class F>
-MARF_DEV void s2_sfor_impl(std::integer_sequence<int, I...>, F&& f) {
-    (f(std::integral_constant<int, I>()), ...);
-}
-template <int N, class F>
-MARF_DEV void s2_sfor(F&& f) {
-    s2_sfor_impl(std::make_integer_sequence<int, N>(), f);
-}
-
-MARF_DEV uint32_t s2_pk(float a, float b) {
-    typedef float f32x2 __attribute__((ext_vector_type(2)));
-    typedef __bf16 bf16x2 __attribute__((ext_vector_type(2)));
-    return __builtin_bit_cast(uint32_t, __builtin_convertvector(((f32x2){a, b}), bf16x2));
-}
-MARF_DEV float s2_lo16(uint32_t w) { return __uint_as_float(w << 16); }
-MARF_DEV float s2_hi16(uint32_t w) { return __uint_as_float(w & 0xffff0000u); }
-
-union S2Frag {
-    bf16x8 f;
-    f16x8 h;
-    uint4 u;
-    uint32_t w[4];
-};
-
-MARF_DEV uint32_t s2_pkh(float a, float b) {
-    typedef float f32x2 __attribute__((ext_vector_type(2)));
-    typedef _Float16 f16x2 __attribute__((ext_vector_type(2)));
-    return __builtin_bit_cast(uint32_t, __builtin_convertvector(((f32x2){a, b}), f16x2));
 }
 
 template <bool LO>
@@ -132,6 +96,7 @@
 #endif
     constexpr bool J2 = MARF_STEP2_J2 && NS == 2 && SPLIT && !SDZ && FIX;
     constexpr float kGS = 1024.f;
+    constexpr bool DZL_OK = SPLIT && !DZ && !HF && C::NMW == 4;
     constexpr int R0Q = NKH / (FIX ? NK0F : NKH);
     constexpr int R0F = R0Q < 1 ? 1 : (R0Q > NRT ? NRT : R0Q);
     extern __shared__ __attribute__((aligned(16))) char smem[];
@@ -169,6 +134,16 @@
         reinterpret_cast<uint32_t*>(lyr)[e] = reinterpret_cast<const uint32_t*>(a.layers)[e];
     for (int e = lane; e < 512; e += 64) reinterpret_cast<uint32_t*>(gts)[e] = 0u;
     for (int e = lane; e < 3 * a.Kl; e += 64) wla[e] = 0.f;
+    if constexpr (DZL_OK) {
+        if (a.dzl_w && blockIdx.x == 0) {
+            const uint4* src = reinterpret_cast<const uint4*>(a.prog + (size_t)a.n_fwd * C::SLOT);
+            uint4* dst = reinterpret_cast<uint4*>(a.dzl_w);
+            for (int e = threadIdx.x; e < 2 * NRT * 64; e += NW * 64) {
+                const int part = e / (NRT * 64);
+                dst[e] = src[part * (C::LO / 16) + (e - part * NRT * 64)];
+            }
+        }
+    }
 
     const int tpp = a.geo.Np_pad / C::TPX;
     const int Np = a.geo.Np;
@@ -326,14 +301,9 @@
 
     auto store_rt = [&](u16* row0, auto rtc, const S2Frag& f0, const S2Frag& f1) {
         constexpr int rt = decltype(rtc)::value;
-        auto contig = [&](const S2Frag& f) -> uint4 {
-            const auto xz = __builtin_amdgcn_permlane32_swap(f.u.x, f.u.z, false, false);
-            const auto yw = __builtin_amdgcn_permlane32_swap(f.u.y, f.u.w, false, false);
-            return make_uint4(xz[0], yw[0], xz[1], yw[1]);
-        };
         u16* blk = row0 + 1024 * rt;
-        s2_st16o<0>(blk, contig(f0));
-        s2_st16o<1024>(blk, contig(f1));
+        s2_st16o<0>(blk, s2_t16_contig(f0));
+        s2_st16o<1024>(blk, s2_t16_contig(f1));
         st_cur += 2;
     };
 
@@ -349,12 +319,7 @@
     };
     typedef std::integral_constant<bool, true> PcOn;
     typedef std::integral_constant<bool, false> PcOff;
-    auto mf = [&](f32x16& acc, const uint4& x, const S2Frag& y) {
-        if constexpr (HF)
-            acc = __builtin_amdgcn_mfma_f32_32x32x16_f16(__builtin_bit_cast(f16x8, x), y.h, acc, 0, 0, 0);
-        else
-            acc = __builtin_amdgcn_mfma_f32_32x32x16_bf16(__builtin_bit_cast(bf16x8, x), y.f, acc, 0, 0, 0);
-    };
+    auto mf = [&](f32x16& acc, const uint4& x, const S2Frag& y) { s2_mfma<HF>(acc, x, y); };
     auto gemm = [&](f32x16& acc, const char* slot, const S2Frag* Bhi, const S2Frag* Blo, int nk, auto mode_tag,
                     auto nk_tag, auto&& hook, auto pieces_tag) {
         constexpr int MODE = decltype(mode_tag)::value;
@@ -580,14 +545,13 @@
         constexpr int rt = decltype(rtc)::value;
         s2_sfor<8>([&](auto qc) {
             constexpr int q = decltype(qc)::value;
-            constexpr int b0 = 16 * 0 + 8 * (1 - (rt & 1)) + 7 - q, b1 = 16 * 1 + 8 * (1 - (rt & 1)) + 7 - q;
-            const float x0 = __int_as_float(__builtin_amdgcn_sbfe((int)es.mw, b0, 1) & __float_as_int(pa[2 * q]));
-            const float x1 = __int_as_float(__builtin_amdgcn_sbfe((int)es.mw, b1, 1) & __float_as_int(pa[2 * q + 1]));
+            float x0, x1;
+            s2_bmask_pair<rt & 1, q>(es.mw, pa, x0, x1);
             es.hw[q] = HF ? s2_pkh(x0, x1) : s2_pk(x0, x1);
             if constexpr (SDZ) es.lw[q] = s2_pk(x0 - s2_lo16(es.hw[q]), x1 - s2_hi16(es.hw[q]));
         });
     };
-    auto bfinish = [&](EpSt& es, S2Frag* O, auto rtc, u16* row0) {
+    auto bfinish = [&](EpSt& es, S2Frag* O, auto rtc, u16* row0, bool save = true) {
         constexpr int rt = decltype(rtc)::value;
         O[2 * rt].u = make_uint4(es.hw[0], es.hw[1], es.hw[2], es.hw[3]);
         O[2 * rt + 1].u = make_uint4(es.hw[4], es.hw[5], es.hw[6], es.hw[7]);
@@ -595,7 +559,7 @@
             Ol[2 * rt].u = make_uint4(es.lw[0], es.lw[1], es.lw[2], es.lw[3]);
             Ol[2 * rt + 1].u = make_uint4(es.lw[4], es.lw[5], es.lw[6], es.lw[7]);
         }
-        store_rt(row0, rtc, O[2 * rt], O[2 * rt + 1]);
+        if (save) store_rt(row0, rtc, O[2 * rt], O[2 * rt + 1]);
     };
     auto gemm2 = [&](f32x16& c0, f32x16& c1, const char* slot, const S2Frag* B0, const S2Frag* B1, auto nk_tag,
                      auto&& hook, auto pieces_tag, auto f16_tag) {
@@ -1318,6 +1282,20 @@
                     st_cur += 4;
                 }
             }
+            bool save_dz = true;
+            if constexpr (DZL_OK) {
+                if (a.dzl_g) {
+                    save_dz = false;
+                    s2_sfor<NS>([&](auto sc) {
+                        constexpr int s = decltype(sc)::value;
+                        const size_t set = (size_t)(sl0[s] >> 5);
+                        const uint32_t* mk = mks_b(s) + lmask * C::NMW * 64 + lane;
+                        s2_st16(a.dzl_mk + set * DZL_MK_SET + lane * 16, make_uint4(mk[0], mk[64], mk[128], mk[192]));
+                        if (h == 0) s2_st16(a.dzl_g + set * DZL_G_SET + pxl * 16, gB[s].u);
+                        st_cur += 2;
+                    });
+                }
+            }
             s2_sfor<NRT>([&](auto rtc) {
                 constexpr int rt = decltype(rtc)::value;
                 if (rt < nrt) {
@@ -1343,14 +1321,14 @@
                                 }, PcOff());
                             }
                             S2T_BEGIN(11);
-                            bfinish(eb, Do[sp], std::integral_constant<int, rp>(), brow[sp]);
+                            bfinish(eb, Do[sp], std::integral_constant<int, rp>(), brow[sp], save_dz);
                             S2T_END(11);
                         }
                         if (s == NS - 1 && rt == nrt - 1) {
                             eb.mw = mks_b(s)[(lmask * C::NMW + (rt >> 1)) * 64 + lane];
                             if constexpr (FIX) bsteps_free(eb, cur, rtc);
                             else s2_sfor<16>([&](auto ec) { bstep(eb, cur, ec, rtc); });
-                            bfinish(eb, Do[s], rtc, brow[s]);
+                            bfinish(eb, Do[s], rtc, brow[s], save_dz);
                         }
                     });
                 } else {
diff --git a/masking-bundle-adjusting-neural-radiance-fields_amd/csrc/marf_step2_dev.h b/masking-bundle-adjusting-neural-radiance-fields_amd/csrc/marf_step2_dev.h
--- /dev/null
+++ b/masking-bundle-adjusting-neural-radiance-fields_amd/csrc/marf_step2_dev.h
@@ -0,0 +1,68 @@
+#pragma once
+#include <type_traits>
+#include <utility>
+
+#include "marf_common.h"
+
+namespace marf {
+
+template <int... I, class F>
+MARF_DEV void s2_sfor_impl(std::integer_sequence<int, I...>, F&& f) {
+    (f(std::integral_constant<int, I>()), ...);
+}
+template <int N, class F>
+MARF_DEV void s2_sfor(F&& f) {
+    s2_sfor_impl(std::make_integer_sequence<int, N>(), f);
+}
+
+MARF_DEV void s2_glds4(const void* src, unsigned lds) {
+    unsigned keep;
+    asm volatile("s_mov_b32 %0, m0\n\ts_mov_b32 m0, %2\n\ts_nop 0\n\tglobal_load_lds_dword %1, off\n\ts_mov_b32 m0, %0"
+                 : "=&s"(keep)
+                 : "v"(src), "s"(lds)
+                 : "memory");
+}
+
+MARF_DEV uint32_t s2_pk(float a, float b) {
+    typedef float f32x2 __attribute__((ext_vector_type(2)));
+    typedef __bf16 bf16x2 __attribute__((ext_vector_type(2)));
+    return __builtin_bit_cast(uint32_t, __builtin_convertvector(((f32x2){a, b}), bf16x2));
+}
+MARF_DEV float s2_lo16(uint32_t w) { return __uint_as_float(w << 16); }
+MARF_DEV float s2_hi16(uint32_t w) { return __uint_as_float(w & 0xffff0000u); }
+
+union S2Frag {
+    bf16x8 f;
+    f16x8 h;
+    uint4 u;
+    uint32_t w[4];
+};
+
+MARF_DEV uint32_t s2_pkh(float a, float b) {
+    typedef float f32x2 __attribute__((ext_vector_type(2)));
+    typedef _Float16 f16x2 __attribute__((ext_vector_type(2)));
+    return __builtin_bit_cast(uint32_t, __builtin_convertvector(((f32x2){a, b}), f16x2));
+}
+
+template <bool HF>
+MARF_DEV void s2_mfma(f32x16& acc, const uint4& x, const S2Frag& y) {
+    if constexpr (HF)
+        acc = __builtin_amdgcn_mfma_f32_32x32x16_f16(__builtin_bit_cast(f16x8, x), y.h, acc, 0, 0, 0);
+    else
+        acc = __builtin_amdgcn_mfma_f32_32x32x16_bf16(__builtin_bit_cast(bf16x8, x), y.f, acc, 0, 0, 0);
+}
+
+template <int RTO, int Q>
+MARF_DEV void s2_bmask_pair(uint32_t mw, const f32x16& pa, float& x0, float& x1) {
+    constexpr int b0 = 16 * 0 + 8 * (1 - RTO) + 7 - Q, b1 = 16 * 1 + 8 * (1 - RTO) + 7 - Q;
+    x0 = __int_as_float(__builtin_amdgcn_sbfe((int)mw, b0, 1) & __float_as_int(pa[2 * Q]));
+    x1 = __int_as_float(__builtin_amdgcn_sbfe((int)mw, b1, 1) & __float_as_int(pa[2 * Q + 1]));
+}
+
+MARF_DEV uint4 s2_t16_contig(const S2Frag& f) {
+    const auto xz = __builtin_amdgcn_permlane32_swap(f.u.x, f.u.z, false, false);
+    const auto yw = __builtin_amdgcn_permlane32_swap(f.u.y, f.u.w, false, false);
+    return make_uint4(xz[0], yw[0], xz[1], yw[1]);
+}
+
+}
diff --git a/masking-bundle-adjusting-neural-radiance-fields_amd/csrc/marf_wgrad.hip b/masking-bundle-adjusting-neural-radiance-fields_amd/csrc/marf_wgrad.hip
--- a/masking-bundle-adjusting-neural-radiance-fields_amd/csrc/marf_wgrad.hip
+++ b/masking-bundle-adjusting-neural-radiance-fields_amd/csrc/marf_wgrad.hip
@@ -1,4 +1,5 @@
 #include "marf_args.h"
+#include "marf_step2_dev.h"
 
 #include <algorithm>
 #include <cstdlib>
@@ -27,6 +28,7 @@
     long long s_lo, s_len;
     int rng_n, part0;
     int t16;
+    WgDzlSrc dzl;
 };
 
 template <int RT, int CT>
@@ -224,9 +226,11 @@
     else return r * (KF * 2) + c * 2;
 }
 
-template <class P, int NBUF, int SP, int KF, bool F0 = false, bool T16 = false>
+template <class P, int NBUF, int SP, int KF, bool F0 = false, bool T16 = false, bool DZL = false>
 MARF_DEV void wgrad_dma_body(const WgArgs& a, int chunk_id, int ob, char* smem) {
     static_assert(KF == 256 || KF == 96, "feat width");
+    static_assert(!DZL || (T16 && !F0 && KF == 256 && SP == 32 && std::is_same<P, PrecBF16>::value),
+                  "dz recompute: the bf16 T16 hidden layer, one 32-pixel set per stage");
     static_assert(!F0 || (KF == 96 && SP % 32 == 0), "feat_0 recompute: the 96-wide layer-0 stage, 32-row blocks");
     constexpr int WR = KF == 256 ? 4 : 8, WC = 8 / WR;
     constexpr int RT = 256 / 32 / WR, CT = KF / 32 / WC;
@@ -260,6 +264,17 @@
 
     const unsigned lds0 = (unsigned)(uintptr_t)(__attribute__((address_space(3))) char*)smem;
     const unsigned junk = lds0 + NBUF * STB;
+    constexpr int DZL_SLOT = DZL_MK_SET + DZL_G_SET, DZL_SM0 = NBUF * STB;
+    const bool dzl = DZL && a.dzl.g != nullptr;
+    uint4 dzl_whi = make_uint4(0, 0, 0, 0), dzl_wlo = make_uint4(0, 0, 0, 0);
+    if constexpr (DZL) {
+        if (dzl) {
+            dzl_whi = *reinterpret_cast<const uint4*>(a.dzl.w + wave * 1024 + lane * 16);
+            dzl_wlo = *reinterpret_cast<const uint4*>(a.dzl.w + DZL_W_BYTES / 2 + wave * 1024 + lane * 16);
+            asm volatile("" ::"v"(dzl_whi.x), "v"(dzl_whi.y), "v"(dzl_whi.z), "v"(dzl_whi.w), "v"(dzl_wlo.x), "v"(dzl_wlo.y),
+                         "v"(dzl_wlo.z), "v"(dzl_wlo.w));
+        }
+    }
     float* f0_h = reinterpret_cast<float*>(smem + NBUF * STB);
     float* f0_w = f0_h + 9 * F0_PATCHES;
     float* f0_uv = f0_w + 32;
@@ -344,6 +359,47 @@
 #pragma unroll
         for (int q = 0; q < NGF; ++q) t16f[q] = t16_lane(a.ldf, k0 >> 4, KF >> 4, q * 8 + wave < (FB >> 10) ? q * 8 + wave : 0);
     }
+    auto issue_dzl_in = [&](int st) {
+        const bool real = st < n_st && wave < 6;
+        const size_t set = (size_t)(s_begin >> 5) + (st < n_st ? st : 0);
+        const char* src = wave < 4 ? a.dzl.mk + set * DZL_MK_SET + wave * 256 + lane * 4
+                                   : a.dzl.g + set * DZL_G_SET + (wave & 1) * 256 + lane * 4;
+        const unsigned dst = real ? lds0 + DZL_SM0 + (st % (NBUF + 1)) * DZL_SLOT + wave * 256
+                                  : lds0 + DZL_SM0 + (NBUF + 1) * DZL_SLOT;
+        s2_glds4(src, __builtin_amdgcn_readfirstlane(dst));
+    };
+    f32x16 dzl_c = (f32x16){};
+    uint32_t dzl_mw = 0u;
+    auto dzl_mma = [&](int st) {
+        const char* in = smem + DZL_SM0 + (st % (NBUF + 1)) * DZL_SLOT;
+        S2Frag gB;
+        gB.u = lane < 32 ? *reinterpret_cast<const uint4*>(in + DZL_MK_SET + lane * 16) : make_uint4(0, 0, 0, 0);
+        dzl_mw = *reinterpret_cast<const uint32_t*>(in + lane * 16 + (wave >> 1) * 4);
+        dzl_c = (f32x16){};
+        s2_mfma<false>(dzl_c, dzl_whi, gB);
+        s2_mfma<false>(dzl_c, dzl_wlo, gB);
+    };
+    auto dzl_store = [&](int st) {
+        const f32x16& c = dzl_c;
+        const uint32_t mw = dzl_mw;
+        uint32_t hw[8];
+        auto pack = [&](auto rto) {
+            s2_sfor<8>([&](auto qc) {
+                constexpr int q = decltype(qc)::value;
+                float x0, x1;
+                s2_bmask_pair<decltype(rto)::value, q>(mw, c, x0, x1);
+                hw[q] = s2_pk(x0, x1);
+            });
+        };
+        if (wave & 1) pack(std::integral_constant<int, 1>());
+        else pack(std::integral_constant<int, 0>());
+        S2Frag f0, f1;
+        f0.u = make_uint4(hw[0], hw[1], hw[2], hw[3]);
+        f1.u = make_uint4(hw[4], hw[5], hw[6], hw[7]);
+        char* out = smem + (st % NBUF) * STB + t16_lds(lane & 31, 32 * wave + 8 * (lane >> 5), 16);
+        *reinterpret_cast<uint4*>(out) = s2_t16_contig(f0);
+        *reinterpret_cast<uint4*>(out + 1024) = s2_t16_contig(f1);
+    };
     auto issue = [&](int st) {
         const unsigned buf = lds0 + (st % NBUF) * STB;
         const long long row0 = s_begin + (long long)st * SP;
@@ -351,6 +407,7 @@
         const char* f16 = reinterpret_cast<const char*>(a.feat) + (size_t)(row0 >> 5) * (size_t)(a.ldf >> 4) * 1024;
 #pragma unroll
         for (int q = 0; q < NGZ; ++q) {
+            if (dzl) break;
             const int seg = q * 8 + wave;
             if constexpr (T16) {
                 glds16(z16 + t16z[q], __builtin_amdgcn_readfirstlane(buf + seg * 1024));
@@ -377,6 +434,17 @@
             }
         }
         if constexpr (F0) compute_f0(st, (st % NBUF) * STB + ZB);
+        if constexpr (DZL) {
+            if (dzl) issue_dzl_in(st + 1);
+        }
+    };
+    auto ring_wait = [&](int ahead, auto per) {
+        constexpr int PER = decltype(per)::value;
+        if (ahead >= 4) wait_vm<4 * PER>();
+        else if (ahead == 3) wait_vm<3 * PER>();
+        else if (ahead == 2) wait_vm<2 * PER>();
+        else if (ahead == 1) wait_vm<PER>();
+        else wait_vm<0>();
     };
 
     f32x16 acc[RT][CT];
@@ -386,19 +454,31 @@
         for (int j = 0; j < CT; ++j) acc[i][j] = (f32x16){};
     float bsum = 0.f;
 
+    if constexpr (DZL) {
+        if (dzl && n_st > 0) issue_dzl_in(0);
+    }
     for (int st = 0; st < NBUF - 1 && st < n_st; ++st) issue(st);
     const int g = lane >> 4, gi = lane & 15, q4 = gi >> 2, p4 = gi & 3;
     for (int st = 0; st < n_st; ++st) {
         const int ahead = min(NBUF - 2, n_st - 1 - st);
-        if (ahead >= 4) wait_vm<4 * PER_ST>();
-        else if (ahead == 3) wait_vm<3 * PER_ST>();
-        else if (ahead == 2) wait_vm<2 * PER_ST>();
-        else if (ahead == 1) wait_vm<PER_ST>();
-        else wait_vm<0>();
+        if (dzl) ring_wait(ahead, std::integral_constant<int, NGF + 1>());
+        else ring_wait(ahead, std::integral_constant<int, PER_ST>());
         asm volatile("s_waitcnt lgkmcnt(0)" ::: "memory");
         __builtin_amdgcn_s_barrier();
         asm volatile("" ::: "memory");
         if (st + NBUF - 1 < n_st) issue(st + NBUF - 1);
+        if constexpr (DZL) {
+            if (dzl) {
+                if (st == 0) {
+                    dzl_mma(0);
+                    dzl_store(0);
+                    asm volatile("s_waitcnt lgkmcnt(0)" ::: "memory");
+                    __builtin_amdgcn_s_barrier();
+                    asm volatile("" ::: "memory");
+                }
+                if (st + 1 < n_st) dzl_mma(st + 1);
+            }
+        }
         if constexpr (F0) {
             if (wave == 7 && lane < SP && st + NBUF < n_st) warp_rows(st + NBUF, lane);
         }
@@ -439,6 +519,9 @@
 #pragma unroll
                 for (int j = 0; j < CT; ++j) acc[i][j] = P::mma32(af[i], bf[j], acc[i][j]);
         }
+        if constexpr (DZL) {
+            if (dzl && st + 1 < n_st) dzl_store(st + 1);
+        }
     }
 
     float* out = a.partial + (size_t)pidx * a.M * a.K + (size_t)m0 * a.K + k0;
@@ -461,7 +544,7 @@
     }
 }
 
-template <class P, int NBUF, int SP, int KF, bool F0 = false, bool T16 = false>
+template <class P, int NBUF, int SP, int KF, bool F0 = false, bool T16 = false, bool DZL = false>
 __global__ __launch_bounds__(512, 1) void k_wgrad_dma(WgArgs a) {
     extern __shared__ __attribute__((aligned(16))) char smem[];
     const int n_ob = (a.M / 256) * a.n_oblk_c;
@@ -474,7 +557,7 @@
         chunk_id = blockIdx.x % a.n_chunks;
         ob = blockIdx.x / a.n_chunks;
     }
-    wgrad_dma_body<P, NBUF, SP, KF, F0, T16>(a, chunk_id, ob, smem);
+    wgrad_dma_body<P, NBUF, SP, KF, F0, T16, DZL>(a, chunk_id, ob, smem);
 }
 
 template <class P>
@@ -571,11 +654,11 @@
     int n_chunks;
 };
 
-template <class P, int NBUF, int SP, int KF>
+template <class P, int NBUF, int SP, int KF, bool DZL = false>
 __global__ __launch_bounds__(512, 1) void k_wgrad_dma_layers(WgLayersArgs la) {
     extern __shared__ __attribute__((aligned(16))) char smem[];
     const int l = blockIdx.x / la.n_chunks, c = blockIdx.x - l * la.n_chunks;
-    wgrad_dma_body<P, NBUF, SP, KF, false, true>(la.a[l], c, 0, smem);
+    wgrad_dma_body<P, NBUF, SP, KF, false, true, DZL>(la.a[l], c, 0, smem);
 }
 
 struct WgRedJob {
@@ -677,28 +760,36 @@
     return !(e && e[0] == '0');
 }
 
-template <class P, int KF, bool F0 = false, bool T16 = false>
+constexpr size_t WG_DZL_LDS = (size_t)(WG_NBUF_H + 1) * (DZL_MK_SET + DZL_G_SET) + 256;
+
+template <class P, int KF, bool F0 = false, bool T16 = false, bool DZL = false>
 static hipError_t launch_wg_dma(WgArgs a, int n_chunks, hipStream_t s) {
     a.n_chunks = n_chunks;
     a.n_oblk_c = (a.K + KF - 1) / KF;
     constexpr int SP = F0 ? WG_SP0 : KF == 256 ? WG_SPH : 32;
     constexpr int NBUF = KF == 256 ? WG_NBUF_H : F0 ? WG_NBUF_0 : WG_NBUF_96;
-    const size_t lds = (size_t)NBUF * SP * (512 + KF * 2) + (KF == 256 ? 0 : 1024) + (F0 ? (9 * F0_PATCHES + 32 + (NBUF + 1) * SP * 2) * 4 : 0);
+    const size_t lds = (size_t)NBUF * SP * (512 + KF * 2) + (KF == 256 ? 0 : 1024) + (F0 ? (9 * F0_PATCHES + 32 + (NBUF + 1) * SP * 2) * 4 : 0) +
+                       (DZL ? WG_DZL_LDS : 0);
     {
-        hipError_t e = ensure_dynamic_lds((const void*)k_wgrad_dma<P, NBUF, SP, KF, F0, T16>, lds);
+        hipError_t e = ensure_dynamic_lds((const void*)k_wgrad_dma<P, NBUF, SP, KF, F0, T16, DZL>, lds);
         if (e != hipSuccess) return e;
     }
-    hipLaunchKernelGGL((k_wgrad_dma<P, NBUF, SP, KF, F0, T16>), dim3(n_chunks * (a.M / 256) * a.n_oblk_c), dim3(512), lds, s,
+    hipLaunchKernelGGL((k_wgrad_dma<P, NBUF, SP, KF, F0, T16, DZL>), dim3(n_chunks * (a.M / 256) * a.n_oblk_c), dim3(512), lds, s,
                        a);
     return hipGetLastError();
 }
 
 hipError_t marf_launch_wgrad(int dtype, const void* dz, int ldz, const void* feat, int ldf, long long S, int M, int K,
                              int chunk, int n_chunks, float* partial, float* bpartial, hipStream_t s,
-                             const WgRange* rng, bool t16) {
+                             const WgRange* rng, bool t16, const WgDzlSrc* dzl) {
     WgArgs a;
     memset(&a, 0, sizeof(a));
     a.t16 = t16 ? 1 : 0;
+    if (dzl && dzl->g) {
+        if (rng || dtype != 1 || !t16 || !dzl->mk || !dzl->w || !marf_wgrad_dzl_ok(M, ldz, K, ldf, S, chunk, n_chunks))
+            return hipErrorInvalidValue;
+        a.dzl = *dzl;
+    }
     if (rng) {
         a.s_lo = rng->s_lo;
         a.s_len = rng->s_len;
@@ -731,6 +822,7 @@
     if (rng && (dtype == 0 || !(dma256 || dma96))) return hipErrorInvalidValue;
     if (t16 && dtype == 0) return hipErrorInvalidValue;
     if (dtype == 1) {
+        if (a.dzl.g) return launch_wg_dma<PrecBF16, 256, false, true, true>(a, n_chunks, s);
         if (dma256) return t16 ? launch_wg_dma<PrecBF16, 256, false, true>(a, n_chunks, s) : launch_wg_dma<PrecBF16, 256>(a, n_chunks, s);
         if (dma96) return t16 ? launch_wg_dma<PrecBF16, 96, false, true>(a, n_chunks, s) : launch_wg_dma<PrecBF16, 96>(a, n_chunks, s);
         if (cfg == 0) return launch_wg<PrecBF16, 2, 4>(a, n_chunks, nr * nc, s);
@@ -756,6 +848,11 @@
     if (dtype != 1 && dtype != 2) return false;
     if (!(M % 256 == 0 && ldz % 8 == 0 && ldz >= M && wgrad_dma_enabled())) return false;
     return (K % 256 == 0 && ldf % 8 == 0 && ldf >= K) || (K == 96 && ldf == 96);
+}
+
+bool marf_wgrad_dzl_ok(int M, int ldz, int K, int ldf, long long S, int chunk, int n_chunks) {
+    return M == 256 && K == 256 && ldz == 256 && ldf % 8 == 0 && ldf >= K && S % WG_SPH == 0 && chunk % WG_SPH == 0 &&
+           n_chunks >= 1 && wgrad_dma_enabled();
 }
 
 bool marf_wgrad_l0_recompute_ok(int M, int ldz, int ldf0, long long S, int chunk, int n_chunks, long long Np_pad) {
@@ -848,6 +945,7 @@
     memset(&la, 0, sizeof(la));
     la.n_chunks = n_chunks;
     int nh = 0;
+    bool any_dzl = false;
     for (int i = 0; i < n_layers; ++i) {
         const WgFusedLayer& Ly = layers[i];
         if (Ly.kind != 0) continue;
@@ -865,17 +963,26 @@
         a.partial = Ly.partial;
         a.bpartial = Ly.bpartial;
         a.t16 = 1;
+        if (Ly.dzl.g) {
+            if (dtype != 1 || !Ly.dzl.mk || !Ly.dzl.w || !marf_wgrad_dzl_ok(Ly.M, Ly.ldz, Ly.K, Ly.ldf, S, chunk, n_chunks))
+                return hipErrorInvalidValue;
+            a.dzl = Ly.dzl;
+            any_dzl = true;
+        }
     }
     if (nh) {
         const size_t lds = (size_t)WG_NBUF_H * WG_SPH * (512 + 256 * 2);
-        auto go = [&](auto prec) -> hipError_t {
+        auto go = [&](auto prec, auto dzl_tag) -> hipError_t {
             typedef decltype(prec) P;
-            hipError_t er = ensure_dynamic_lds((const void*)k_wgrad_dma_layers<P, WG_NBUF_H, WG_SPH, 256>, lds);
+            constexpr bool DZL = decltype(dzl_tag)::value;
+            const size_t ldsx = lds + (DZL ? WG_DZL_LDS : 0);
+            hipError_t er = ensure_dynamic_lds((const void*)k_wgrad_dma_layers<P, WG_NBUF_H, WG_SPH, 256, DZL>, ldsx);
             if (er != hipSuccess) return er;
-            hipLaunchKernelGGL((k_wgrad_dma_layers<P, WG_NBUF_H, WG_SPH, 256>), dim3(nh * n_chunks), dim3(512), lds, s, la);
+            hipLaunchKernelGGL((k_wgrad_dma_layers<P, WG_NBUF_H, WG_SPH, 256, DZL>), dim3(nh * n_chunks), dim3(512), ldsx, s, la);
             return hipGetLastError();
         };
-        e = dtype == 2 ? go(PrecF16()) : go(PrecBF16());
+        e = dtype == 2 ? go(PrecF16(), std::false_type())
+                       : (any_dzl ? go(PrecBF16(), std::true_type()) : go(PrecBF16(), std::false_type()));
         if (e != hipSuccess) return e;
     }
     if (l0 && (e = hipStreamWaitEvent(s, join, 0)) != hipSuccess) return e;
```

After: 363.5 million pixels/s (median of 6 runs). 1.1% higher.
